# johnayoung/llm-consensus

Measured on AMD Instinct MI355X. Metric: consensus_aggregate_output_tokens_per_s, higher is better.
Workload: dtype bf16

## Files before the change

csrc/kernels/bindings.cpp:

```cpp
#include <hip/hip_runtime_api.h>
#include <pybind11/pybind11.h>

#include <pybind11/stl.h>

#include <stdexcept>
#include <string>
#include <vector>

namespace py = pybind11;
typedef uintptr_t ptr;

extern "C" {
int llmc_rmsnorm(const void*, const void*, void*, int, int, int, int, float, hipStream_t);
int llmc_embedding(const void*, const void*, void*, int, int, int, hipStream_t);
int llmc_lane_exchange_check(const void*, void*, int, hipStream_t);
int llmc_silu_mul_interleaved(const void*, void*, int, int, hipStream_t);
int llmc_gemv(int, const void*, int, const void*, float, const void*, void*, int, int, int, int, int, hipStream_t);
int llmc_gemv_p13(int, const void*, int, const void*, float, const void*, const void*, const void*, void*, int, int, int,
                  int, hipStream_t);
int llmc_gemv_qkv_rope_p13(int, const void*, int, const void*, float, const void*, const void*, const void*, int, int,
                           void*, int, void*, void*, const void*, const void*, const void*, const void*, int, int, int,
                           int, const void*, hipStream_t);
int llmc_wpack13(const void*, void*, void*, void*, int, int, hipStream_t);
int llmc_gemvm(int, const void*, int, const void*, float, const void*, void*, int, int, int, int, int, hipStream_t);
int llmc_moe_gemvm(int, const void*, int, const void*, float, const void*, const void*, int, int, void*, int, int, int,
                   int, hipStream_t);
int llmc_gemm(const void*, int, const void*, int, void*, int, int, int, int, int, hipStream_t);
int llmc_gemm_t128(const void*, int, const void*, int, void*, int, int, int, int, int, hipStream_t);
int llmc_gemm_narrow(const void*, int, const void*, int, void*, int, int, int, int, int, hipStream_t);
int llmc_gemm_kind(const void*, int, const void*, int, void*, int, int, int, int, int, int, hipStream_t);
int llmc_gemm_plan(int, int);
int llmc_rope_kv_write(const void*, int, void*, int, const void*, const void*, const void*, void*, void*, const void*,
                       int, int, int, int, int, const void*, hipStream_t);
int llmc_attn_decode_groups(int);
int llmc_qkv_attn_check(int, int, int, int);
int llmc_qkv_attn(const void*, const void*, float, const void*, int, void*, void*, void*, const void*, const void*,
                  const void*, const void*, const void*, int, const void*, void*, void*, void*, int, int, int, int, int,
                  int, int, int, float, void*, void*, void*, int, const void*, void*, int, const void* const*, void*,
                  int, int, size_t, hipStream_t);
int llmc_attn_oproj_check(int, int, int, int, int, int);
int llmc_attn_oproj_form(int, int, int, int, int, int, int, int);
int llmc_attn_oproj(const void*, const void*, const void*, const void*, int, const void*, const void*, void*, void*,
                    void*, void*, void*, void*, void*, int, int, int, int, int, int, int, int, float, int, void*,
                    int, const void* const*, void*, int, int, size_t, const void*, const void*, float, int, int,
                    void*, void*, void*, void*, hipStream_t);
int llmc_attn_decode(const void*, int, const void*, const void*, const void*, int, const void*, void*, void*, void*,
                     int, int, int, int, int, int, int, int, int, int, float, int, void*, int, hipStream_t);
int llmc_gemv_qkv_rope(int, const void*, int, const void*, float, const void*, int, int, void*, int, void*, void*,
                       const void*, const void*, const void*, const void*, int, int, int, int, int, const void*,
                       hipStream_t);
int llmc_attn_prefill(const void*, int, const void*, const void*, const void*, int, const void*, const void*,
                      const void*, void*, int, int, int, int, int, int, int, float, int, int, void*, void*, int,
                      int, int, hipStream_t);
int llmc_attn_prefill_form(int, int, int, int, int, int, int);
int llmc_attn_prefill_plan(int, int, int, int, int, int, int, int*);
int64_t llmc_attn_prefill_counters(int, int, int, int);
int llmc_sample(const void*, int64_t, int, int, const void*, const void*, const void*, const void*, const void*, void*,
                void*, void*, void*, void*, void*, const void*, int, int, void*, void*, int, int, hipStream_t);
int llmc_sample_parts();
int llmc_moe_route(const void*, int, int, int, void*, void*, hipStream_t);
int llmc_moe_down_combine(int, const void*, int, const void*, const void*, const void*, void*, int, int, int, int,
                          hipStream_t);
int llmc_moe_router(const void*, int, const void*, float, const void*, int, int, int, int, void*, void*, hipStream_t);
int llmc_moe_align(const void*, int, int, int, int, void*, void*, void*, void*, hipStream_t);
int llmc_moe_gemm(const void*, int, int, const void*, const void*, const void*, const void*, void*, int, int, int, int,
                  int, int, int, hipStream_t);
int llmc_moe_combine(const void*, const void*, const void*, void*, int, int, int, hipStream_t);
int llmc_moe_gemv(int, const void*, int, const void*, float, const void*, const void*, int, void*, int, int, int, int,
                  hipStream_t);
int llmc_moe_ep_localize(const void*, const void*, int, int, int, void*, void*, hipStream_t);
int llmc_moe_ep_dispatch(const void*, int, int, int, int, void*, void*, void*, void*, hipStream_t);
int llmc_gather_rows(const void*, int, const void*, int, int, int, void*, int, hipStream_t);
int llmc_moe_route_fused(const void*, int, const void*, int, int, int, int, void*, void*, hipStream_t);
int llmc_gemv_sweep(int, const void*, const void*, const void*, void*, int, int, hipStream_t);
size_t llmc_car_sig_bytes();
int llmc_car_alloc(size_t, void**);
int llmc_car_free(void*);
int llmc_ipc_handle(void*, void*);
int llmc_ipc_handle_size();
int llmc_ipc_open(const void*, void**);
int llmc_ipc_close(void*);
int llmc_car_timed_out(void*, int*);
int llmc_car_max_wait(void*, uint32_t*);
int llmc_car_host_alloc(void**, void**);
int llmc_car_host_free(void*);
int llmc_car_host_get(const void*, int);
void llmc_car_host_set(void*, int, int);
int llmc_car_host_word(int);
size_t llmc_car_timeout_off();
int llmc_car_reset(void*, size_t);
size_t llmc_car_oneshot_max(size_t);
int llmc_gemv_ar(int, const void*, int, const void*, void*, int, int, int, const void* const*, void*, int, int, size_t,
                 hipStream_t);
int llmc_stream_cu_mask(int, const uint32_t*, int, void**);
int llmc_can_access_peer(int, int, int*);
int llmc_car_twoshot(const void* const*, void*, int, int, size_t, int, const void*, void*, long, int, int, hipStream_t);
int llmc_car_allreduce(const void* const*, void*, int, int, size_t, void*, size_t, hipStream_t);
int llmc_car_allgather(const void* const*, void*, int, int, size_t, const void*, void*, size_t, hipStream_t);
}

static inline void check(int rc, const char* what) {
  if (rc != 0) {
    std::string msg = std::string("llmc HIP launch failed: ") + what + " rc=" + std::to_string(rc);
    if (rc > 0) msg += std::string(" (") + hipGetErrorString(static_cast<hipError_t>(rc)) + ")";
    throw std::runtime_error(msg);
  }
}
#define P(x) reinterpret_cast<void*>(x)
#define S(x) reinterpret_cast<hipStream_t>(x)

PYBIND11_MODULE(_llmc_hip, m) {
  m.doc() = "llm_consensus_amd gfx950 HIP kernels (raw-pointer launchers)";
  m.def("rmsnorm", [](ptr x, ptr w, ptr y, int T, int H, int xs, int ys, float eps, ptr s) {
    check(llmc_rmsnorm(P(x), P(w), P(y), T, H, xs, ys, eps, S(s)), "rmsnorm");
  });
  m.def("lane_exchange_check", [](ptr in, ptr out, int nb, ptr s) {
    check(llmc_lane_exchange_check(P(in), P(out), nb, S(s)), "lane_exchange_check");
  });
  m.def("embedding", [](ptr ids, ptr table, ptr out, int T, int H, int V, ptr s) {
    check(llmc_embedding(P(ids), P(table), P(out), T, H, V, S(s)), "embedding");
  });
  m.def("silu_mul_interleaved", [](ptr gu, ptr y, int T, int I, ptr s) {
    check(llmc_silu_mul_interleaved(P(gu), P(y), T, I, S(s)), "silu_mul");
  });
  m.def("gemv", [](int M, ptr x, int xs, ptr nw, float eps, ptr W, ptr out, int os, int N, int K, int epi, int mfma,
                   ptr s) {
    check(llmc_gemv(M, P(x), xs, P(nw), eps, P(W), P(out), os, N, K, epi, mfma, S(s)), "gemv");
  });
  m.def("gemv_p13", [](int M, ptr x, int xs, ptr nw, float eps, ptr W, ptr planes, ptr hdr, ptr out, int os, int N,
                       int K, int epi, ptr s) {
    check(llmc_gemv_p13(M, P(x), xs, P(nw), eps, P(W), P(planes), P(hdr), P(out), os, N, K, epi, S(s)), "gemv_p13");
  });
  m.def("gemv_qkv_rope_p13", [](int M, ptr x, int xs, ptr nw, float eps, ptr W, ptr planes, ptr hdr, int N, int K,
                                ptr qo, int qos, ptr kc, ptr vc, ptr pos, ptr slots, ptr cos_t, ptr sin_t, int nh,
                                int nkv, int D, int bs, ptr s, ptr bias) {
    check(llmc_gemv_qkv_rope_p13(M, P(x), xs, P(nw), eps, P(W), P(planes), P(hdr), N, K, P(qo), qos, P(kc), P(vc),
                                 P(pos), P(slots), P(cos_t), P(sin_t), nh, nkv, D, bs, P(bias), S(s)),
          "gemv_qkv_rope_p13");
  }, py::arg("M"), py::arg("x"), py::arg("x_stride"), py::arg("norm_w"), py::arg("eps"), py::arg("W"),
     py::arg("planes"), py::arg("hdr"), py::arg("N"), py::arg("K"), py::arg("q_out"), py::arg("q_stride"),
     py::arg("k_cache"), py::arg("v_cache"), py::arg("positions"), py::arg("slots"), py::arg("cos_t"),
     py::arg("sin_t"), py::arg("nh"), py::arg("nkv"), py::arg("D"), py::arg("bs"), py::arg("stream"),
     py::arg("bias") = 0);
  m.def("wpack13", [](ptr W, ptr planes, ptr hdr, ptr raw_count, int N, int K, ptr s) {
    check(llmc_wpack13(P(W), P(planes), P(hdr), P(raw_count), N, K, S(s)), "wpack13");
  });
  m.def("moe_gemvm", [](int P, ptr x, int xs, ptr nw, float eps, ptr W, ptr ids, int x_div, int E, ptr out, int os,
                        int N, int K, int epi, ptr s) {
    check(llmc_moe_gemvm(P, P(x), xs, P(nw), eps, P(W), P(ids), x_div, E, P(out), os, N, K, epi, S(s)), "moe_gemvm");
  });
  m.def("gemvm", [](int M, ptr x, int xs, ptr nw, float eps, ptr W, ptr out, int os, int N, int K, int epi, int form,
                    ptr s) {
    check(llmc_gemvm(M, P(x), xs, P(nw), eps, P(W), P(out), os, N, K, epi, form, S(s)), "gemvm");
  });
  m.def("gemm", [](ptr A, int lda, ptr W, int ldw, ptr C, int ldc, int M, int N, int K, int epi, ptr s) {
    check(llmc_gemm(P(A), lda, P(W), ldw, P(C), ldc, M, N, K, epi, S(s)), "gemm");
  });
  m.def("gemm_t128", [](ptr A, int lda, ptr W, int ldw, ptr C, int ldc, int M, int N, int K, int epi, ptr s) {
    check(llmc_gemm_t128(P(A), lda, P(W), ldw, P(C), ldc, M, N, K, epi, S(s)), "gemm_t128");
  });
  m.def("gemm_kind", [](ptr A, int lda, ptr W, int ldw, ptr C, int ldc, int M, int N, int K, int epi, int kind, ptr s) {
    check(llmc_gemm_kind(P(A), lda, P(W), ldw, P(C), ldc, M, N, K, epi, kind, S(s)), "gemm_kind");
  });
  m.def("gemm_plan", [](int M, int N) { return llmc_gemm_plan(M, N); });
  m.def("gemm_narrow", [](ptr A, int lda, ptr W, int ldw, ptr C, int ldc, int M, int N, int K, int epi, ptr s) {
    check(llmc_gemm_narrow(P(A), lda, P(W), ldw, P(C), ldc, M, N, K, epi, S(s)), "gemm_narrow");
  });
  m.def("rope_kv_write", [](ptr qkv, int qs, ptr qo, int qos, ptr pos, ptr cos_t, ptr sin_t, ptr kc, ptr vc,
                            ptr slots, int T, int nh, int nkv, int D, int bs, ptr s, ptr bias) {
    check(llmc_rope_kv_write(P(qkv), qs, P(qo), qos, P(pos), P(cos_t), P(sin_t), P(kc), P(vc), P(slots), T, nh, nkv, D,
                             bs, P(bias), S(s)),
          "rope_kv_write");
  }, py::arg("qkv"), py::arg("qkv_stride"), py::arg("q_out"), py::arg("q_stride"), py::arg("positions"),
     py::arg("cos_t"), py::arg("sin_t"), py::arg("k_cache"), py::arg("v_cache"), py::arg("slots"), py::arg("T"),
     py::arg("nh"), py::arg("nkv"), py::arg("D"), py::arg("bs"), py::arg("stream"),
     py::arg("bias") = 0);
  m.def("attn_decode_groups", [](int max_chunks) { return llmc_attn_decode_groups(max_chunks); });
  m.def("qkv_attn_check", [](int nh, int nkv, int D, int K) { return llmc_qkv_attn_check(nh, nkv, D, K); });
  m.def("qkv_attn", [](ptr x, ptr nw, float eps, ptr W, int K, ptr qo, ptr kc, ptr vc, ptr pos, ptr slots, ptr cos_t,
                       ptr sin_t, ptr bt, int bt_len, ptr sl, ptr part, ptr ctr, ptr out, int nh, int nkv, int D, int bs,
                       int nblocks, int chunk, int gc, int max_chunks, float scale, ptr fault, ptr gran, ptr hctr,
                       int o_mode, ptr w_o, ptr h, int o_n, const std::vector<ptr>& bases, ptr host, int rank, int world,
                       size_t cap, ptr s) {
    std::vector<const void*> b(bases.size());
    for (size_t i = 0; i < bases.size(); ++i) b[i] = P(bases[i]);
    check(llmc_qkv_attn(P(x), P(nw), eps, P(W), K, P(qo), P(kc), P(vc), P(pos), P(slots), P(cos_t), P(sin_t), P(bt),
                        bt_len, P(sl), P(part), P(ctr), P(out), nh, nkv, D, bs, nblocks, chunk, gc, max_chunks, scale,
                        P(fault), P(gran), P(hctr), o_mode, P(w_o), P(h), o_n, b.empty() ? nullptr : b.data(), P(host),
                        rank, world, cap, S(s)),
          "qkv_attn");
  });
  m.def("attn_oproj_check", [](int H, int nh, int nkv, int D, int nc, int K_o) {
    return llmc_attn_oproj_check(H, nh, nkv, D, nc, K_o);
  });
  m.def("attn_oproj_form", [](int H, int nh, int nkv, int D, int nc, int chunk, int mode, int world) {
    return llmc_attn_oproj_form(H, nh, nkv, D, nc, chunk, mode, world);
  });
  m.def("attn_oproj", [](ptr q, ptr kc, ptr vc, ptr bt, int bt_len, ptr sl, ptr w_o, ptr h, ptr attn_out, ptr part,
                         ptr handoff, ptr tile_part, ptr ctr, ptr fault, int H, int nh, int nkv, int D, int bs,
                         int nblocks, int chunk, int nc, float scale, int mode, ptr stamps, int add_resid,
                         const std::vector<ptr>& bases, ptr host, int rank, int world, size_t cap, ptr rt_norm,
                         ptr rt_wr, float rt_eps, int rt_E, int rt_k, ptr rt_w, ptr rt_ids, ptr rt_part,
                         ptr rt_epoch, ptr s) {
    std::vector<const void*> b(bases.size());
    for (size_t i = 0; i < bases.size(); ++i) b[i] = P(bases[i]);
    check(llmc_attn_oproj(P(q), P(kc), P(vc), P(bt), bt_len, P(sl), P(w_o), P(h), P(attn_out), P(part), P(handoff),
                          P(tile_part), P(ctr), P(fault), H, nh, nkv, D, bs, nblocks, chunk, nc, scale, mode, P(stamps),
                          add_resid, b.empty() ? nullptr : b.data(), P(host), rank, world, cap, P(rt_norm), P(rt_wr),
                          rt_eps, rt_E, rt_k, P(rt_w), P(rt_ids), P(rt_part), P(rt_epoch), S(s)),
          "attn_oproj");
  });
  m.def("attn_decode", [](ptr q, int qs, ptr kc, ptr vc, ptr bt, int bts, ptr sl, ptr part, ptr ctr, ptr out, int os,
                          int B, int nh, int nkv, int D, int bs, int nblocks, int chunk, int grid_chunks,
                          int max_chunks, float scale, int fused, ptr fault, ptr s, int window) {
    check(llmc_attn_decode(P(q), qs, P(kc), P(vc), P(bt), bts, P(sl), P(part), P(ctr), P(out), os, B, nh, nkv, D, bs,
                           nblocks, chunk, grid_chunks, max_chunks, scale, fused, P(fault), window, S(s)),
          "attn_decode");
  }, py::arg("q"), py::arg("q_stride"), py::arg("k_cache"), py::arg("v_cache"), py::arg("block_tables"),
     py::arg("bt_stride"), py::arg("seq_lens"), py::arg("part"), py::arg("counters"), py::arg("out"),
     py::arg("out_stride"), py::arg("B"), py::arg("nh"), py::arg("nkv"), py::arg("D"), py::arg("bs"),
     py::arg("nblocks"), py::arg("chunk"), py::arg("grid_chunks"), py::arg("max_chunks"), py::arg("scale"),
     py::arg("fused"), py::arg("fault"), py::arg("stream"), py::arg("window") = 0);
  m.def("gemv_qkv_rope", [](int M, ptr x, int xs, ptr nw, float eps, ptr W, int N, int K, ptr qo, int qos, ptr kc,
                            ptr vc, ptr pos, ptr slots, ptr cos_t, ptr sin_t, int nh, int nkv, int D, int bs,
                            int mfma, ptr s, ptr bias) {
    check(llmc_gemv_qkv_rope(M, P(x), xs, P(nw), eps, P(W), N, K, P(qo), qos, P(kc), P(vc), P(pos), P(slots),
                             P(cos_t), P(sin_t), nh, nkv, D, bs, mfma, P(bias), S(s)),
          "gemv_qkv_rope");
  }, py::arg("M"), py::arg("x"), py::arg("x_stride"), py::arg("norm_w"), py::arg("eps"), py::arg("W"), py::arg("N"),
     py::arg("K"), py::arg("q_out"), py::arg("q_stride"), py::arg("k_cache"), py::arg("v_cache"),
     py::arg("positions"), py::arg("slots"), py::arg("cos_t"), py::arg("sin_t"), py::arg("nh"), py::arg("nkv"),
     py::arg("D"), py::arg("bs"), py::arg("mfma"), py::arg("stream"),
     py::arg("bias") = 0);
  m.def("attn_prefill", [](ptr q, int qs, ptr kc, ptr vc, ptr bt, int bts, ptr qst, ptr ql, ptr cl, ptr out, int os,
                           int B, int max_qlen, int nh, int nkv, int D, int bs, float scale, int ksplit, int kmin,
                           ptr part, ptr counters, int T, int form, ptr s, int window) {
    check(llmc_attn_prefill(P(q), qs, P(kc), P(vc), P(bt), bts, P(qst), P(ql), P(cl), P(out), os, B, max_qlen, nh, nkv,
                            D, bs, scale, ksplit, kmin, P(part), P(counters), T, form, window, S(s)),
          "attn_prefill");
  }, py::arg("q"), py::arg("q_stride"), py::arg("k_cache"), py::arg("v_cache"), py::arg("block_tables"),
     py::arg("bt_stride"), py::arg("q_start"), py::arg("q_lens"), py::arg("ctx_lens"), py::arg("out"),
     py::arg("out_stride"), py::arg("B"), py::arg("max_qlen"), py::arg("nh"), py::arg("nkv"), py::arg("D"),
     py::arg("bs"), py::arg("scale"), py::arg("ksplit"), py::arg("kmin"), py::arg("part"), py::arg("counters"),
     py::arg("T"), py::arg("form"), py::arg("stream"), py::arg("window") = 0);
  m.def("attn_prefill_counters", [](int B, int max_qlen, int nh, int nkv) {
    return llmc_attn_prefill_counters(B, max_qlen, nh, nkv);
  });
  m.def("attn_prefill_form", [](int B, int T, int nh, int nkv, int ksplit, int D, int bs) {
    return llmc_attn_prefill_form(B, T, nh, nkv, ksplit, D, bs);
  });
  m.def("attn_prefill_plan", [](int B, int max_qlen, int max_ctx, int nh, int nkv, int D, int bs) {
    int kmin = 0;
    const int k = llmc_attn_prefill_plan(B, max_qlen, max_ctx, nh, nkv, D, bs, &kmin);
    return std::make_pair(k, kmin);
  });
  m.def("sample", [](ptr logits, int64_t rs, int B, int V, ptr it, ptr tk, ptr tp, ptr seeds, ptr pos, ptr wv, ptr wi,
                     ptr next, ptr tin, ptr sl, ptr slots, ptr bt, int bts, int bs, ptr ot, ptr oc, int cap,
                     int use_topkp, ptr s) {
    check(llmc_sample(P(logits), rs, B, V, P(it), P(tk), P(tp), P(seeds), P(pos), P(wv), P(wi), P(next), P(tin), P(sl),
                      P(slots), P(bt), bts, bs, P(ot), P(oc), cap, use_topkp, S(s)),
          "sample");
  });
  m.def("sample_parts", []() { return llmc_sample_parts(); });
  m.def("moe_route", [](ptr logits, int T, int E, int k, ptr w, ptr ids, ptr s) {
    check(llmc_moe_route(P(logits), T, E, k, P(w), P(ids), S(s)), "moe_route");
  });
  m.def("moe_down_combine", [](int T, ptr act, int as, ptr W, ptr ids, ptr w, ptr h, int hs, int N, int K, int k,
                               ptr s) {
    check(llmc_moe_down_combine(T, P(act), as, P(W), P(ids), P(w), P(h), hs, N, K, k, S(s)), "moe_down_combine");
  });
  m.def("moe_router", [](ptr x, int xs, ptr nw, float eps, ptr Wr, int T, int E, int H, int k, ptr w, ptr ids, ptr s) {
    check(llmc_moe_router(P(x), xs, P(nw), eps, P(Wr), T, E, H, k, P(w), P(ids), S(s)), "moe_router");
  });
  m.def("moe_align", [](ptr ids, int T, int k, int E, int tile, ptr sorted_rows, ptr tile_expert, ptr tile_count,
                        ptr counts, ptr s) {
    check(llmc_moe_align(P(ids), T, k, E, tile, P(sorted_rows), P(tile_expert), P(tile_count), P(counts), S(s)),
          "moe_align");
  });
  m.def("moe_gemm", [](ptr A, int lda, int a_rows, ptr W, ptr sorted_rows, ptr tile_expert, ptr tile_count, ptr C,
                       int ldc, int N, int K, int max_tiles, int a_row_div, int epi, int tile, ptr s) {
    check(llmc_moe_gemm(P(A), lda, a_rows, P(W), P(sorted_rows), P(tile_expert), P(tile_count), P(C), ldc, N, K,
                        max_tiles, a_row_div, epi, tile, S(s)),
          "moe_gemm");
  });
  m.def("moe_combine", [](ptr y, ptr w, ptr rows, ptr out, int T, int k, int H, ptr s) {
    check(llmc_moe_combine(P(y), P(w), P(rows), P(out), T, k, H, S(s)), "moe_combine");
  });
  m.def("moe_gemv", [](int npairs, ptr x, int xs, ptr nw, float eps, ptr W, ptr ids, int x_div, ptr out, int os,
                       int N, int K, int epi, ptr s) {
    check(llmc_moe_gemv(npairs, P(x), xs, P(nw), eps, P(W), P(ids), x_div, P(out), os, N, K, epi, S(s)), "moe_gemv");
  });
  m.def("moe_ep_dispatch", [](ptr ids, int npairs, int El, int n, int cap, ptr sp, ptr se, ptr slot, ptr cnt, ptr s) {
    check(llmc_moe_ep_dispatch(P(ids), npairs, El, n, cap, P(sp), P(se), P(slot), P(cnt), S(s)), "moe_ep_dispatch");
  });
  m.def("moe_route_fused", [](ptr x, int xs, ptr wr, int T, int E, int H, int k, ptr w, ptr ids, ptr s) {
    check(llmc_moe_route_fused(P(x), xs, P(wr), T, E, H, k, P(w), P(ids), S(s)), "moe_route_fused");
  });
  m.def("gather_rows", [](ptr x, int xs, ptr rows, int M, int div, int H, ptr out, int os, ptr s) {
    check(llmc_gather_rows(P(x), xs, P(rows), M, div, H, P(out), os, S(s)), "gather_rows");
  });
  m.def("moe_ep_localize", [](ptr ids, ptr w, int n, int e0, int nl, ptr lids, ptr lw, ptr s) {
    check(llmc_moe_ep_localize(P(ids), P(w), n, e0, nl, P(lids), P(lw), S(s)), "moe_ep_localize");
  });
  m.def("device_synchronize", []() { check(static_cast<int>(hipDeviceSynchronize()), "hipDeviceSynchronize"); });
  m.def("car_sig_bytes", []() { return llmc_car_sig_bytes(); });
  m.def("car_alloc", [](size_t cap) {
    void* p = nullptr;
    check(llmc_car_alloc(cap, &p), "car_alloc");
    return reinterpret_cast<ptr>(p);
  });
  m.def("car_free", [](ptr p) { check(llmc_car_free(P(p)), "car_free"); });
  m.def("ipc_handle", [](ptr p) {
    std::string h(static_cast<size_t>(llmc_ipc_handle_size()), '\0');
    check(llmc_ipc_handle(P(p), h.data()), "ipc_handle");
    return py::bytes(h);
  });
  m.def("ipc_open", [](py::bytes h) {
    std::string s = h;
    if (static_cast<int>(s.size()) != llmc_ipc_handle_size()) throw std::runtime_error("ipc_open: bad handle size");
    void* p = nullptr;
    check(llmc_ipc_open(s.data(), &p), "ipc_open");
    return reinterpret_cast<ptr>(p);
  });
  m.def("ipc_close", [](ptr p) { check(llmc_ipc_close(P(p)), "ipc_close"); });
  m.def("car_timed_out", [](ptr own) {
    int v = 0;
    check(llmc_car_timed_out(P(own), &v), "car_timed_out");
    return v;
  });
  m.def("car_timeout_off", []() { return llmc_car_timeout_off(); });
  m.def("car_max_wait", [](ptr own) {
    uint32_t v = 0;
    check(llmc_car_max_wait(P(own), &v), "car_max_wait");
    return v;
  });
  m.def("car_host_alloc", []() {
    void* h = nullptr;
    void* d = nullptr;
    check(llmc_car_host_alloc(&h, &d), "car_host_alloc");
    return py::make_tuple(reinterpret_cast<ptr>(h), reinterpret_cast<ptr>(d));
  });
  m.def("car_host_free", [](ptr h) { check(llmc_car_host_free(P(h)), "car_host_free"); });
  m.def("car_host_get", [](ptr h, int word) { return llmc_car_host_get(P(h), word); });
  m.def("car_host_set", [](ptr h, int word, int v) { llmc_car_host_set(P(h), word, v); });
  m.def("car_host_word", [](int which) { return llmc_car_host_word(which); });
  m.def("car_reset", [](ptr own, size_t cap) { check(llmc_car_reset(P(own), cap), "car_reset"); });
  m.def("car_oneshot_max", [](size_t cap) { return llmc_car_oneshot_max(cap); });
  m.def("gemv_ar", [](int M, ptr x, int xs, ptr W, ptr h, int hs, int N, int K, const std::vector<ptr>& bases,
                      ptr host, int rank, int world, size_t cap, ptr s) {
    std::vector<const void*> b(bases.size());
    for (size_t i = 0; i < bases.size(); ++i) b[i] = P(bases[i]);
    check(llmc_gemv_ar(M, P(x), xs, P(W), P(h), hs, N, K, b.data(), P(host), rank, world, cap, S(s)), "gemv_ar");
  });
  m.def("stream_cu_mask", [](int device, const std::vector<uint32_t>& mask) {
    void* st = nullptr;
    check(llmc_stream_cu_mask(device, mask.data(), static_cast<int>(mask.size()), &st), "stream_cu_mask");
    return reinterpret_cast<ptr>(st);
  });
  m.def("can_access_peer", [](int dev, int peer) {
    int v = 0;
    check(llmc_can_access_peer(dev, peer, &v), "can_access_peer");
    return v;
  });
  m.def("car_twoshot", [](const std::vector<ptr>& bases, ptr host, int rank, int world, size_t cap, int mode, ptr in,
                          ptr out, long seg_stride, int seg16, int nv, ptr s) {
    std::vector<const void*> b(bases.size());
    for (size_t i = 0; i < bases.size(); ++i) b[i] = P(bases[i]);
    check(llmc_car_twoshot(b.data(), P(host), rank, world, cap, mode, P(in), P(out), seg_stride, seg16, nv, S(s)),
          "car_twoshot");
  });
  m.def("car_allreduce", [](const std::vector<ptr>& bases, ptr host, int rank, int world, size_t cap, ptr x,
                            size_t nbytes, ptr s) {
    std::vector<const void*> b(bases.size());
    for (size_t i = 0; i < bases.size(); ++i) b[i] = P(bases[i]);
    check(llmc_car_allreduce(b.data(), P(host), rank, world, cap, P(x), nbytes, S(s)), "car_allreduce");
  });
  m.def("car_allgather", [](const std::vector<ptr>& bases, ptr host, int rank, int world, size_t cap, ptr x, ptr out,
                            size_t nbytes, ptr s) {
    std::vector<const void*> b(bases.size());
    for (size_t i = 0; i < bases.size(); ++i) b[i] = P(bases[i]);
    check(llmc_car_allgather(b.data(), P(host), rank, world, cap, P(x), P(out), nbytes, S(s)), "car_allgather");
  });
  m.def("gemv_sweep", [](int v, ptr x, ptr nw, ptr W, ptr out, int N, int K, ptr s) {
    check(llmc_gemv_sweep(v, P(x), P(nw), P(W), P(out), N, K, S(s)), "gemv_sweep");
  });
}
```

csrc/kernels/gemv.hip:

```cpp
#include <cstdlib>

#include "gemv_core.h"

namespace llmc {

template <int M, int NT, int RPW, int PRO, int EPI, int UNROLL>
static int launch_gemv_p13(const void* x, int x_stride, const void* nw, float eps, const void* W, const PackedW& pw,
                           void* out, int out_stride, int N, int K, const RopeEpi& rope, hipStream_t s) {
  if constexpr (M <= 2 && UNROLL % 4 == 0) {
    constexpr int WAVES = NT / kWave;
    auto kern = gemv_p13_kernel<M, NT, RPW, UNROLL, PRO, EPI>;
    const size_t lds = static_cast<size_t>(M) * K * sizeof(bf16_t) + 2 * M * WAVES * sizeof(float);
    if (lds > 160 * 1024) return -2;
    static bool attr_set = false;
    if (lds > 64 * 1024 && !attr_set) {
      (void)hipFuncSetAttribute(reinterpret_cast<const void*>(kern), hipFuncAttributeMaxDynamicSharedMemorySize,
                                160 * 1024);
      attr_set = true;
    }
    const int rows_per_block = WAVES * RPW;
    const int grid = (N + rows_per_block - 1) / rows_per_block;
    kern<<<grid, NT, lds, s>>>((const bf16_t*)x, x_stride, (const bf16_t*)nw, eps, (const bf16_t*)W, pw, out,
                               out_stride, N, K, rope);
    return static_cast<int>(hipGetLastError());
  } else {
    return -8;
  }
}

template <int M, int NT, int RPW, int PRO, int EPI, int UNROLL_OVERRIDE = 0>
static int launch_gemv_g(const void* x, int x_stride, const void* nw, float eps, const void* W, void* out,
                         int out_stride, int N, int K, const RopeEpi& rope, const PackedW& pw, hipStream_t s) {
  constexpr int UNROLL = UNROLL_OVERRIDE ? UNROLL_OVERRIDE : (RPW == 1 ? 4 : (RPW == 2 ? 4 : (M <= 2 ? 4 : 2)));
  constexpr int WAVES = NT / kWave;
  if (pw.planes != nullptr)
    return launch_gemv_p13<M, NT, RPW, PRO, EPI, UNROLL>(x, x_stride, nw, eps, W, pw, out, out_stride, N, K, rope, s);
  auto kern = gemv_kernel<M, NT, RPW, UNROLL, PRO, EPI, false>;
  const size_t lds = static_cast<size_t>(M) * K * sizeof(bf16_t) + 2 * M * WAVES * sizeof(float);
  if (lds > 160 * 1024) return -2;
  static bool attr_set = false;
  if (lds > 64 * 1024 && !attr_set) {
    (void)hipFuncSetAttribute(reinterpret_cast<const void*>(kern), hipFuncAttributeMaxDynamicSharedMemorySize,
                              160 * 1024);
    attr_set = true;
  }
  const int rows_per_block = WAVES * RPW;
  const int grid = (N + rows_per_block - 1) / rows_per_block;
  kern<<<grid, NT, lds, s>>>((const bf16_t*)x, x_stride, (const bf16_t*)nw, eps, (const bf16_t*)W, out, out_stride, N,
                             K, nullptr, 1, rope, CarArgs{});
  return static_cast<int>(hipGetLastError());
}

static int pick_waves(int N, bool paired) {
  if (N < 2048 && (!paired || N % 8 == 0)) return 4;
  static const bool no10 = std::getenv("LLMC_GEMV_NO_W10") != nullptr;
  static const bool no14 = std::getenv("LLMC_GEMV_NO_W14") != nullptr;
  int best = 16;
  double best_idle = 2.0;
  for (int w : {16, 14, 12, 10, 8}) {
    if ((w == 10 && no10) || (w == 14 && (no14 || !paired))) continue;
    if (paired && N % (2 * w) != 0) continue;
    const long blocks = (N + w - 1) / w;
    const long slots = (blocks + 255) / 256 * 256;
    const double idle = static_cast<double>(slots - blocks) / static_cast<double>(slots);
    if (idle < best_idle - 1e-9) {
      best_idle = idle;
      best = w;
    }
  }
  return best_idle > 1.0 ? 0 : best;
}

template <int M, int PRO, int EPI>
static int launch_gemv(const void* x, int x_stride, const void* nw, float eps, const void* W, void* out,
                       int out_stride, int N, int K, const RopeEpi& rope, const PackedW& pw, hipStream_t s) {
  constexpr bool paired = EPI == EPI_SILU || EPI == EPI_ROPE;
  const int w = pick_waves(N, paired);
  if constexpr (M <= 2) {
    static const bool rope_rpw1 = std::getenv("LLMC_GEMV_ROPE_RPW1") != nullptr;
    if (EPI == EPI_ROPE && w == 12 && N % (2 * 12 * 256) == 0 && !rope_rpw1)
      return launch_gemv_g<M, 768, 2, PRO, EPI, 4>(x, x_stride, nw, eps, W, out, out_stride, N, K, rope, pw, s);
    static const bool silu_rpw1 = std::getenv("LLMC_GEMV_SILU_RPW1") != nullptr;
    if (EPI == EPI_SILU && !silu_rpw1 && K < 8192) {
      if (N % (2 * 16 * 256) == 0)
        return launch_gemv_g<M, 1024, 2, PRO, EPI, 4>(x, x_stride, nw, eps, W, out, out_stride, N, K, rope, pw, s);
      if (N % (2 * 14 * 256) == 0)
        return launch_gemv_g<M, 896, 2, PRO, EPI, 4>(x, x_stride, nw, eps, W, out, out_stride, N, K, rope, pw, s);
    }
    if (w == 16 && K >= 8192 && N <= 4096)
      return launch_gemv_g<M, 1024, 1, PRO, EPI, 8>(x, x_stride, nw, eps, W, out, out_stride, N, K, rope, pw, s);
    if (w == 10 && K >= 8192)
      return launch_gemv_g<M, 640, 1, PRO, EPI, 8>(x, x_stride, nw, eps, W, out, out_stride, N, K, rope, pw, s);
  }
  switch (w) {
    case 16: return launch_gemv_g<M, 1024, 1, PRO, EPI>(x, x_stride, nw, eps, W, out, out_stride, N, K, rope, pw, s);
    case 14: return launch_gemv_g<M, 896, 1, PRO, EPI>(x, x_stride, nw, eps, W, out, out_stride, N, K, rope, pw, s);
    case 12: return launch_gemv_g<M, 768, 1, PRO, EPI>(x, x_stride, nw, eps, W, out, out_stride, N, K, rope, pw, s);
    case 10: return launch_gemv_g<M, 640, 1, PRO, EPI>(x, x_stride, nw, eps, W, out, out_stride, N, K, rope, pw, s);
    case 8: return launch_gemv_g<M, 512, 1, PRO, EPI>(x, x_stride, nw, eps, W, out, out_stride, N, K, rope, pw, s);
    case 4: return launch_gemv_g<M, 256, 1, PRO, EPI, 8>(x, x_stride, nw, eps, W, out, out_stride, N, K, rope, pw, s);
    default:
      return launch_gemv_g<M, 256, 2, PRO, EPI>(x, x_stride, nw, eps, W, out, out_stride, N, K, rope, pw, s);
  }
}

template <int PRO, int EPI>
static int dispatch_m(int M, const void* x, int x_stride, const void* nw, float eps, const void* W, void* out,
                      int out_stride, int N, int K, const RopeEpi& rope, const PackedW& pw, hipStream_t s) {
  switch (M) {
    case 1: return launch_gemv<1, PRO, EPI>(x, x_stride, nw, eps, W, out, out_stride, N, K, rope, pw, s);
    case 2: return launch_gemv<2, PRO, EPI>(x, x_stride, nw, eps, W, out, out_stride, N, K, rope, pw, s);
    case 3: return launch_gemv<3, PRO, EPI>(x, x_stride, nw, eps, W, out, out_stride, N, K, rope, pw, s);
    case 4: return launch_gemv<4, PRO, EPI>(x, x_stride, nw, eps, W, out, out_stride, N, K, rope, pw, s);
    default: return -3;
  }
}

static int gemv_dispatch(int M, const void* x, int x_stride, const void* norm_w, float eps, const void* W, void* out,
                         int out_stride, int N, int K, int epi, const RopeEpi& rope, const PackedW& pw, bool mfma,
                         hipStream_t s) {
  if (K % 8 != 0) return -1;
  if ((epi == EPI_SILU || epi == EPI_ROPE) && (N % 2 != 0)) return -1;
  if ((M > kGemvMaxM || mfma) && K % 128 == 0 && x_stride % 8 == 0)
    return gemvm_dispatch(M, x, x_stride, norm_w, eps, W, out, out_stride, N, K, epi, rope, s);
  const bool norm = norm_w != nullptr;
#define LLMC_GEMV_CASE(E)                                                                                   \
  case E:                                                                                                   \
    return norm ? dispatch_m<PRO_NORM, E>(M, x, x_stride, norm_w, eps, W, out, out_stride, N, K, rope, pw, s)   \
                : dispatch_m<PRO_NONE, E>(M, x, x_stride, norm_w, eps, W, out, out_stride, N, K, rope, pw, s);
  switch (epi) {
    LLMC_GEMV_CASE(EPI_BF16)
    LLMC_GEMV_CASE(EPI_F32)
    LLMC_GEMV_CASE(EPI_RESADD)
    LLMC_GEMV_CASE(EPI_SILU)
    case EPI_ROPE:
      if (!norm) return -5;
      return dispatch_m<PRO_NORM, EPI_ROPE>(M, x, x_stride, norm_w, eps, W, out, out_stride, N, K, rope, pw, s);
    default: return -4;
  }
#undef LLMC_GEMV_CASE
}

}

using namespace llmc;

extern "C" int llmc_gemv(int M, const void* x, int x_stride, const void* norm_w, float eps, const void* W, void* out,
                         int out_stride, int N, int K, int epi, int mfma, hipStream_t s) {
  if (epi == EPI_ROPE) return -5;
  RopeEpi rope{};
  return gemv_dispatch(M, x, x_stride, norm_w, eps, W, out, out_stride, N, K, epi, rope, PackedW{}, mfma != 0, s);
}

extern "C" int llmc_gemv_p13(int M, const void* x, int x_stride, const void* norm_w, float eps, const void* W,
                             const void* planes, const void* hdr, void* out, int out_stride, int N, int K, int epi,
                             hipStream_t s) {
  if (epi == EPI_ROPE) return -5;
  if (M < 1 || M > kGemvMaxM || K % kP13UnitElems != 0 || planes == nullptr || hdr == nullptr) return -1;
  RopeEpi rope{};
  const PackedW pw{static_cast<const uint8_t*>(planes), static_cast<const uint8_t*>(hdr)};
  return gemv_dispatch(M, x, x_stride, norm_w, eps, W, out, out_stride, N, K, epi, rope, pw, false, s);
}

extern "C" int llmc_gemv_qkv_rope(int M, const void* x, int x_stride, const void* norm_w, float eps, const void* W,
                                  int N, int K, void* q_out, int q_stride, void* k_cache, void* v_cache,
                                  const void* positions, const void* slots, const void* cos_t, const void* sin_t,
                                  int nh, int nkv, int D, int bs, int mfma, const void* bias, hipStream_t s) {
  if (N != (nh + 2 * nkv) * D || D % 2 != 0 || reinterpret_cast<uintptr_t>(bias) % 4 != 0) return -1;
  RopeEpi rope{(bf16_t*)q_out, q_stride, (bf16_t*)k_cache, (bf16_t*)v_cache, (const int32_t*)positions,
               (const int32_t*)slots, (const float*)cos_t, (const float*)sin_t, nh, nkv, D, bs};
  rope.bias = static_cast<const bf16_t*>(bias);
  return gemv_dispatch(M, x, x_stride, norm_w, eps, W, nullptr, 0, N, K, EPI_ROPE, rope, PackedW{}, mfma != 0, s);
}

extern "C" int llmc_gemv_qkv_rope_p13(int M, const void* x, int x_stride, const void* norm_w, float eps,
                                      const void* W, const void* planes, const void* hdr, int N, int K, void* q_out,
                                      int q_stride, void* k_cache, void* v_cache, const void* positions,
                                      const void* slots, const void* cos_t, const void* sin_t, int nh, int nkv, int D,
                                      int bs, const void* bias, hipStream_t s) {
  if (N != (nh + 2 * nkv) * D || D % 2 != 0 || reinterpret_cast<uintptr_t>(bias) % 4 != 0) return -1;
  if (M < 1 || M > kGemvMaxM || K % kP13UnitElems != 0 || planes == nullptr || hdr == nullptr) return -1;
  RopeEpi rope{(bf16_t*)q_out, q_stride, (bf16_t*)k_cache, (bf16_t*)v_cache, (const int32_t*)positions,
               (const int32_t*)slots, (const float*)cos_t, (const float*)sin_t, nh, nkv, D, bs};
  rope.bias = static_cast<const bf16_t*>(bias);
  const PackedW pw{static_cast<const uint8_t*>(planes), static_cast<const uint8_t*>(hdr)};
  return gemv_dispatch(M, x, x_stride, norm_w, eps, W, nullptr, 0, N, K, EPI_ROPE, rope, pw, false, s);
}

namespace llmc {
template <int M, int NT, int UNROLL>
static int launch_gemv_ar(const void* x, int x_stride, const void* W, void* h, int h_stride, int N, int K,
                          const CarArgs& ar, hipStream_t s) {
  constexpr int WAVES = NT / kWave;
  auto kern = gemv_kernel<M, NT, 1, UNROLL, PRO_NONE, EPI_AR, false>;
  const size_t lds = static_cast<size_t>(M) * K * sizeof(bf16_t) + 2 * M * WAVES * sizeof(float);
  if (lds > 160 * 1024) return -2;
  static bool attr_set = false;
  if (lds > 64 * 1024 && !attr_set) {
    (void)hipFuncSetAttribute(reinterpret_cast<const void*>(kern), hipFuncAttributeMaxDynamicSharedMemorySize,
                              160 * 1024);
    attr_set = true;
  }
  const int grid = (N + WAVES - 1) / WAVES;
  if (grid > kMaxBlocks || static_cast<size_t>(grid) * kArGranulesPerBlock * 8 > static_cast<size_t>(ar.cap) / kMaxRanks)
    return -6;
  kern<<<grid, NT, lds, s>>>((const bf16_t*)x, x_stride, nullptr, 0.f, (const bf16_t*)W, h, h_stride, N, K, nullptr, 1,
                             RopeEpi{}, ar);
  return static_cast<int>(hipGetLastError());
}

template <int M>
static int gemv_ar_geom(const void* x, int x_stride, const void* W, void* h, int h_stride, int N, int K,
                        const CarArgs& ar, hipStream_t s) {
  const int w = pick_waves(N, false);
  if (w == 16 && K >= 8192 && N <= 4096) return launch_gemv_ar<M, 1024, 8>(x, x_stride, W, h, h_stride, N, K, ar, s);
  if (w == 10 && K >= 8192) return launch_gemv_ar<M, 640, 8>(x, x_stride, W, h, h_stride, N, K, ar, s);
  switch (w) {
    case 16: return launch_gemv_ar<M, 1024, 4>(x, x_stride, W, h, h_stride, N, K, ar, s);
    case 12: return launch_gemv_ar<M, 768, 4>(x, x_stride, W, h, h_stride, N, K, ar, s);
    case 10: return launch_gemv_ar<M, 640, 4>(x, x_stride, W, h, h_stride, N, K, ar, s);
    case 8: return launch_gemv_ar<M, 512, 4>(x, x_stride, W, h, h_stride, N, K, ar, s);
    case 4: return launch_gemv_ar<M, 256, 8>(x, x_stride, W, h, h_stride, N, K, ar, s);
    default: return -7;
  }
}
}

extern "C" int llmc_gemv_ar(int M, const void* x, int x_stride, const void* W, void* h, int h_stride, int N, int K,
                            const void* const* bases, void* host, int rank, int world, size_t cap, hipStream_t s) {
  if (K % 8 != 0 || N % 2 != 0 || world < 1 || world > kMaxRanks || rank < 0 || rank >= world) return -1;
  CarArgs ar{};
  for (int r = 0; r < kMaxRanks; ++r)
    ar.P.base[r] = r < world ? static_cast<char*>(const_cast<void*>(bases[r])) : nullptr;
  ar.P.host = static_cast<uint32_t*>(host);
  ar.rank = rank;
  ar.world = world;
  ar.cap = static_cast<long>(cap);
  switch (M) {
    case 1: return gemv_ar_geom<1>(x, x_stride, W, h, h_stride, N, K, ar, s);
    case 2: return gemv_ar_geom<2>(x, x_stride, W, h, h_stride, N, K, ar, s);
    default: return -3;
  }
}

namespace llmc {
template <int NT, int RPW, int EPI, int PRO>
static int launch_moe_gemv(int npairs, const void* x, int x_stride, const void* nw, float eps, const void* W,
                           const void* ids, int x_div, void* out, int out_stride, int N, int K, hipStream_t s) {
  constexpr int WAVES = NT / kWave;
  const size_t lds = static_cast<size_t>(K) * sizeof(bf16_t) + 2 * WAVES * sizeof(float);
  if (lds > 64 * 1024) return -2;
  dim3 grid((N + WAVES * RPW - 1) / (WAVES * RPW), npairs);
  gemv_kernel<1, NT, RPW, 4, PRO, EPI, true><<<grid, NT, lds, s>>>(
      (const bf16_t*)x, x_stride, (const bf16_t*)nw, eps, (const bf16_t*)W, out, out_stride, N, K,
      (const int32_t*)ids, x_div, RopeEpi{}, CarArgs{});
  return static_cast<int>(hipGetLastError());
}

template <int EPI, int PRO>
static int moe_gemv_geom(int npairs, const void* x, int x_stride, const void* nw, float eps, const void* W,
                         const void* ids, int x_div, void* out, int out_stride, int N, int K, hipStream_t s) {
  static const bool silu_rpw1 = std::getenv("LLMC_GEMV_SILU_RPW1") != nullptr;
  if (EPI == EPI_SILU && !silu_rpw1 && K < 8192) {
    if (N % (2 * 16 * 256) == 0)
      return launch_moe_gemv<1024, 2, EPI, PRO>(npairs, x, x_stride, nw, eps, W, ids, x_div, out, out_stride, N, K, s);
    if (N % (2 * 14 * 256) == 0)
      return launch_moe_gemv<896, 2, EPI, PRO>(npairs, x, x_stride, nw, eps, W, ids, x_div, out, out_stride, N, K, s);
  }
  switch (pick_waves(N, EPI == EPI_SILU)) {
    case 16: return launch_moe_gemv<1024, 1, EPI, PRO>(npairs, x, x_stride, nw, eps, W, ids, x_div, out, out_stride, N, K, s);
    case 14: return launch_moe_gemv<896, 1, EPI, PRO>(npairs, x, x_stride, nw, eps, W, ids, x_div, out, out_stride, N, K, s);
    case 12: return launch_moe_gemv<768, 1, EPI, PRO>(npairs, x, x_stride, nw, eps, W, ids, x_div, out, out_stride, N, K, s);
    case 10: return launch_moe_gemv<640, 1, EPI, PRO>(npairs, x, x_stride, nw, eps, W, ids, x_div, out, out_stride, N, K, s);
    case 8: return launch_moe_gemv<512, 1, EPI, PRO>(npairs, x, x_stride, nw, eps, W, ids, x_div, out, out_stride, N, K, s);
    case 4: return launch_moe_gemv<256, 1, EPI, PRO>(npairs, x, x_stride, nw, eps, W, ids, x_div, out, out_stride, N, K, s);
    default: return launch_moe_gemv<256, 2, EPI, PRO>(npairs, x, x_stride, nw, eps, W, ids, x_div, out, out_stride, N, K, s);
  }
}
}

extern "C" int llmc_moe_down_combine(int T, const void* act, int act_stride, const void* W, const void* ids,
                                     const void* w, void* h, int h_stride, int N, int K, int k, hipStream_t s) {
  if (k != 2 || K % 8 != 0) return -1;
  constexpr int NT = 1024, WAVES = NT / kWave;
  auto kern = gemv_kernel<2, NT, 2, 4, PRO_NONE, EPI_COMBINE, true>;
  const size_t lds = static_cast<size_t>(2) * K * sizeof(bf16_t) + 2 * 2 * WAVES * sizeof(float);
  if (lds > 160 * 1024) return -2;
  static bool attr_set = false;
  if (lds > 64 * 1024 && !attr_set) {
    (void)hipFuncSetAttribute(reinterpret_cast<const void*>(kern), hipFuncAttributeMaxDynamicSharedMemorySize,
                              160 * 1024);
    attr_set = true;
  }
  RopeEpi wts{};
  wts.cos_t = static_cast<const float*>(w);
  dim3 grid((N + WAVES - 1) / WAVES, T);
  kern<<<grid, NT, lds, s>>>((const bf16_t*)act, act_stride, nullptr, 0.f, (const bf16_t*)W, h, h_stride, N, K,
                             (const int32_t*)ids, 1, wts, CarArgs{});
  return static_cast<int>(hipGetLastError());
}

extern "C" int llmc_moe_gemv(int npairs, const void* x, int x_stride, const void* norm_w, float eps, const void* W,
                             const void* ids, int x_div, void* out, int out_stride, int N, int K, int epi,
                             hipStream_t s) {
  if (K % 8 != 0) return -1;
  const void* nw = norm_w;
  switch (epi) {
    case EPI_BF16:
      return nw ? moe_gemv_geom<EPI_BF16, PRO_NORM>(npairs, x, x_stride, nw, eps, W, ids, x_div, out, out_stride, N, K, s)
                : moe_gemv_geom<EPI_BF16, PRO_NONE>(npairs, x, x_stride, nw, eps, W, ids, x_div, out, out_stride, N, K, s);
    case EPI_SILU:
      return nw ? moe_gemv_geom<EPI_SILU, PRO_NORM>(npairs, x, x_stride, nw, eps, W, ids, x_div, out, out_stride, N, K, s)
                : moe_gemv_geom<EPI_SILU, PRO_NONE>(npairs, x, x_stride, nw, eps, W, ids, x_div, out, out_stride, N, K, s);
    default: return -4;
  }
}

namespace llmc {
template <int NT, int RPW, int UNROLL>
static int launch_sweep(const void* x, const void* nw, const void* W, void* out, int N, int K, hipStream_t s) {
  constexpr int WAVES = NT / kWave;
  const size_t lds = static_cast<size_t>(K) * sizeof(bf16_t) + WAVES * sizeof(float);
  const int grid = (N + WAVES * RPW - 1) / (WAVES * RPW);
  gemv_kernel<1, NT, RPW, UNROLL, PRO_NORM, EPI_BF16, false><<<grid, NT, lds, s>>>(
      (const bf16_t*)x, K, (const bf16_t*)nw, 1e-5f, (const bf16_t*)W, out, N, N, K, nullptr, 1, RopeEpi{}, CarArgs{});
  return static_cast<int>(hipGetLastError());
}
}

extern "C" int llmc_gemv_sweep(int variant, const void* x, const void* nw, const void* W, void* out, int N, int K,
                               hipStream_t s) {
  if (K % 8 != 0 || K * 2 > 64 * 1024) return -1;
  switch (variant) {
    case 0: return launch_sweep<256, 1, 8>(x, nw, W, out, N, K, s);
    case 1: return launch_sweep<256, 2, 4>(x, nw, W, out, N, K, s);
    case 2: return launch_sweep<256, 4, 4>(x, nw, W, out, N, K, s);
    case 3: return launch_sweep<512, 1, 8>(x, nw, W, out, N, K, s);
    case 4: return launch_sweep<512, 2, 4>(x, nw, W, out, N, K, s);
    case 5: return launch_sweep<128, 1, 8>(x, nw, W, out, N, K, s);
    case 6: return launch_sweep<64, 1, 8>(x, nw, W, out, N, K, s);
    case 7: return launch_sweep<1024, 1, 4>(x, nw, W, out, N, K, s);
    case 8: return launch_sweep<256, 1, 4>(x, nw, W, out, N, K, s);
    case 9: return launch_sweep<256, 2, 8>(x, nw, W, out, N, K, s);
    case 10: return launch_sweep<512, 4, 2>(x, nw, W, out, N, K, s);
    case 11: return launch_sweep<128, 2, 4>(x, nw, W, out, N, K, s);
    case 12: return launch_sweep<1024, 1, 8>(x, nw, W, out, N, K, s);
    case 13: return launch_sweep<1024, 2, 4>(x, nw, W, out, N, K, s);
    case 14: return launch_sweep<1024, 2, 2>(x, nw, W, out, N, K, s);
    case 15: return launch_sweep<1024, 1, 2>(x, nw, W, out, N, K, s);
    case 16: return launch_sweep<768, 1, 4>(x, nw, W, out, N, K, s);
    case 17: return launch_sweep<1024, 4, 2>(x, nw, W, out, N, K, s);
    case 18: return launch_sweep<1024, 1, 6>(x, nw, W, out, N, K, s);
    case 19: return launch_sweep<768, 2, 4>(x, nw, W, out, N, K, s);
    case 20: return launch_sweep<640, 1, 8>(x, nw, W, out, N, K, s);
    case 21: return launch_sweep<896, 1, 4>(x, nw, W, out, N, K, s);
    case 22: return launch_sweep<768, 2, 2>(x, nw, W, out, N, K, s);
    case 23: return launch_sweep<1024, 2, 2>(x, nw, W, out, N, K, s);
    default: return -2;
  }
}
```

csrc/kernels/gemv_core.h:

```cpp
#pragma once
#include <type_traits>

#include "car_proto.h"
#include "common.h"

namespace llmc {

enum { PRO_NONE = 0, PRO_NORM = 1 };
enum { EPI_BF16 = 0, EPI_F32 = 1, EPI_RESADD = 2, EPI_SILU = 3, EPI_ROPE = 4, EPI_COMBINE = 5, EPI_AR = 6 };


struct RopeEpi {
  bf16_t* q_out;
  int q_stride;
  bf16_t* k_cache;
  bf16_t* v_cache;
  const int32_t* positions;
  const int32_t* slots;
  const float* cos_t;
  const float* sin_t;
  int nh, nkv, D, bs;
  uint64_t* granules;
  uint32_t gtag;
  const bf16_t* bias;
};

enum { WF_BF16 = 0, WF_P13 = 1 };
constexpr int kP13UnitElems = 2048, kP13UnitBytes = 3328, kP13Raw = 0xff;
struct PackedW {
  const uint8_t* planes;
  const uint8_t* hdr;
};
struct P13Unit {
  u32x4 l0, l1, n;
  uint32_t s;
};
template <int C>
__device__ __forceinline__ u32x4 p13_chunk(const P13Unit& p, uint32_t base4) {
  const uint32_t n = p.n[C];
  const uint32_t e0 = (n & 0x0f0f0f0fu) + base4, e1 = ((n >> 4) & 0x0f0f0f0fu) + base4;
  const u32x4& L = C < 2 ? p.l0 : p.l1;
  const uint32_t lw0 = L[(2 * C) & 3], lw1 = L[(2 * C + 1) & 3];
  const uint32_t h0 = ((p.s << (7 - 2 * C)) & 0x80808080u) | e0;
  const uint32_t h1 = ((p.s << (6 - 2 * C)) & 0x80808080u) | e1;
  u32x4 w;
  w[0] = __builtin_amdgcn_perm(h0, lw0, 0x05010400u);
  w[1] = __builtin_amdgcn_perm(h0, lw0, 0x07030602u);
  w[2] = __builtin_amdgcn_perm(h1, lw1, 0x05010400u);
  w[3] = __builtin_amdgcn_perm(h1, lw1, 0x07030602u);
  return w;
}

constexpr int kGemvMaxM = 2, kGemvmMaxM = 32, kMoeGemvmMaxTokens = 16;
int gemvm_dispatch(int M, const void* x, int x_stride, const void* norm_w, float eps, const void* W, void* out,
                   int out_stride, int N, int K, int epi, const RopeEpi& rope, hipStream_t st, int form = 0);

template <int M, int NT, int RPW, int UNROLL, int PRO, int EPI, bool EXPERT = false, int WF = WF_BF16>
__device__ __forceinline__ void gemv_block(const int bx, const int by, char* smem, const bf16_t* __restrict__ x,
                                           int x_stride, const bf16_t* __restrict__ norm_w, float eps,
                                           const bf16_t* __restrict__ W, void* __restrict__ out, int out_stride, int N,
                                           int K, const int32_t* __restrict__ expert_ids, int x_div, const RopeEpi& rope,
                                           const CarArgs& ar, const PackedW& pw = PackedW{}) {
  constexpr int WAVES = NT / kWave;
  constexpr bool P13 = WF == WF_P13;
  static_assert(!P13 || (!EXPERT && EPI != EPI_AR && EPI != EPI_COMBINE && UNROLL % 4 == 0 && M <= 2),
                "packed weights: the dense one- and two-row decode forms");
  constexpr bool PAIR_LDS = (EPI == EPI_SILU || EPI == EPI_ROPE) && RPW == 1;
  constexpr bool ROPE_PRE = EPI == EPI_ROPE && (PAIR_LDS || RPW == 2);
  constexpr bool COMBINE = EPI == EPI_COMBINE;
  static_assert(!COMBINE || (EXPERT && M == RPW), "combine: one x row per expert slot");
  if constexpr (EXPERT && !COMBINE) {
    const int pair = by;
    if (expert_ids[pair] < 0) return;
    W += static_cast<int64_t>(expert_ids[pair]) * N * K;
    x += static_cast<int64_t>(pair / x_div) * x_stride;
    out = reinterpret_cast<char*>(out) + static_cast<int64_t>(pair) * out_stride * (EPI == EPI_F32 ? 4 : 2);
  }
  if constexpr (COMBINE) {
    const int t = by;
    x += static_cast<int64_t>(t) * RPW * x_stride;
    out = reinterpret_cast<char*>(out) + static_cast<int64_t>(t) * out_stride * 2;
  }
  bf16_t* xs = reinterpret_cast<bf16_t*>(smem);
  const int tid = threadIdx.x;
  const int nchunk = K / 8;
  const int wave = tid / kWave, lane = tid % kWave;
  const int row0 = COMBINE ? bx * WAVES + wave : (bx * WAVES + wave) * RPW;

  const u32x4* wrow[RPW];
#pragma unroll
  for (int r = 0; r < RPW; ++r) {
    if constexpr (COMBINE) {
      const int e = expert_ids[by * RPW + r];
      wrow[r] = reinterpret_cast<const u32x4*>(W + (static_cast<int64_t>(e) * N + min(row0, N - 1)) * K);
    } else {
      const int n = min(row0 + r, N - 1);
      wrow[r] = reinterpret_cast<const u32x4*>(W + static_cast<int64_t>(n) * K);
    }
  }
  constexpr int STEP = kWave * UNROLL;
  const int iters = (nchunk + STEP - 1) / STEP;
  u32x4 cur[RPW][UNROLL];
  auto issue = [&](u32x4 (&dst)[RPW][UNROLL], int cbase) {
#pragma unroll
    for (int u = 0; u < UNROLL; ++u) {
      const int c = min(cbase + u * kWave, nchunk - 1);
#pragma unroll
      for (int r = 0; r < RPW; ++r) dst[r][u] = load16<true>(wrow[r] + c);
    }
  };
  constexpr bool kXRegs = (PRO == PRO_NORM || PRO == PRO_NONE);
  const bool x_fast = nchunk <= 2 * NT;
  u32x4 xr[2][M], gr[2];
  if constexpr (kXRegs) {
    if (x_fast) {
#pragma unroll
      for (int j = 0; j < 2; ++j) {
        const int c = tid + j * NT;
        if (c < nchunk) {
          if constexpr (PRO == PRO_NORM) gr[j] = reinterpret_cast<const u32x4*>(norm_w)[c];
#pragma unroll
          for (int m = 0; m < M; ++m) xr[j][m] = reinterpret_cast<const u32x4*>(x + static_cast<int64_t>(m) * x_stride)[c];
        }
      }
    }
  }
  constexpr int UB = P13 ? UNROLL / 4 : 1;
  const int units = K / kP13UnitElems;
  P13Unit cur13[P13 ? RPW : 1][UB];
  const uint8_t* prow[RPW];
  uint32_t hdr_w[RPW];
  auto issue13 = [&](P13Unit (&dst)[P13 ? RPW : 1][UB], int ubase) {
#pragma unroll
    for (int j = 0; j < UB; ++j) {
      const int u = min(ubase + j, units - 1);
#pragma unroll
      for (int r = 0; r < (P13 ? RPW : 1); ++r) {
        const uint8_t* p = prow[r] + static_cast<int64_t>(u) * kP13UnitBytes + lane * 16;
        dst[r][j].l0 = load16<true>(p);
        dst[r][j].l1 = load16<true>(p + 1024);
        dst[r][j].n = load16<true>(p + 2048);
        dst[r][j].s = __builtin_nontemporal_load(reinterpret_cast<const uint32_t*>(p + 3072 - lane * 12));
      }
    }
  };
  __builtin_amdgcn_sched_barrier(0);
  if constexpr (P13) {
    const int w_u = __builtin_amdgcn_readfirstlane(wave);
#pragma unroll
    for (int r = 0; r < RPW; ++r) {
      const int n_u = min((bx * WAVES + w_u) * RPW + r, N - 1);
      hdr_w[r] = ld_scalar(reinterpret_cast<const uint32_t*>(pw.hdr + (n_u & ~3))) >> ((n_u & 3) * 8) & 0xffu;
      prow[r] = pw.planes + static_cast<int64_t>(n_u) * units * kP13UnitBytes;
    }
    issue13(cur13, 0);
  } else {
    issue(cur, lane);
  }
  __builtin_amdgcn_sched_barrier(0);


  uint32_t ar_epoch = 0;
  float ar_resid[M];
  if constexpr (EPI == EPI_AR) {
    static_assert(RPW == 1 && M <= 2 && M * WAVES / 2 <= kArGranulesPerBlock, "EPI_AR geometry");
    if (tid == 0)
      ar_epoch = __hip_atomic_load(car_ctr(ar.P.base[ar.rank]) + bx, __ATOMIC_RELAXED,
                                   __HIP_MEMORY_SCOPE_SYSTEM) + 1;
#pragma unroll
    for (int m = 0; m < M; ++m)
      ar_resid[m] = ar.rank == 0 && row0 < N
                        ? bf16_to_f32(reinterpret_cast<const bf16_t*>(out)[static_cast<int64_t>(m) * out_stride + row0])
                        : 0.f;
  }

  int pre_pos[M], pre_slot[M];
  float pre_c[M], pre_s[M];
  uint32_t pre_b = 0;
  if constexpr (ROPE_PRE) {
#pragma unroll
    for (int m = 0; m < M; ++m) {
      pre_slot[m] = ld_scalar(rope.slots + m);
      pre_pos[m] = ld_scalar(rope.positions + m);
    }
    if (rope.bias != nullptr) {
      const int w_u = __builtin_amdgcn_readfirstlane(wave);
      const int r_u = min(((bx * WAVES + w_u) * RPW) & ~1, N - 2);
      pre_b = ld_scalar(reinterpret_cast<const uint32_t*>(rope.bias + r_u));
    }
  }

  if constexpr (PRO == PRO_NORM) {
    float(*red)[WAVES] = reinterpret_cast<float(*)[WAVES]>(smem + static_cast<size_t>(M) * K * sizeof(bf16_t));
    float ss[M];
#pragma unroll
    for (int m = 0; m < M; ++m) ss[m] = 0.f;
    if (x_fast) {
#pragma unroll
      for (int j = 0; j < 2; ++j) {
        if (tid + j * NT < nchunk) {
#pragma unroll
          for (int m = 0; m < M; ++m) {
            float f[8];
            unpack8(xr[j][m], f);
#pragma unroll
            for (int e = 0; e < 8; ++e) ss[m] += f[e] * f[e];
          }
        }
      }
#pragma unroll
      for (int m = 0; m < M; ++m) {
        const float sm = wave_sum(ss[m]);
        if ((tid & 63) == 0) red[m][tid / 64] = sm;
      }
      __syncthreads();
      float inv[M];
#pragma unroll
      for (int m = 0; m < M; ++m) {
        float t = 0.f;
#pragma unroll
        for (int w = 0; w < WAVES; ++w) t += red[m][w];
        inv[m] = rsqrtf(t / K + eps);
      }
#pragma unroll
      for (int j = 0; j < 2; ++j) {
        const int c = tid + j * NT;
        if (c < nchunk) {
          float g[8];
          unpack8(gr[j], g);
#pragma unroll
          for (int m = 0; m < M; ++m) {
            float f[8];
            unpack8(xr[j][m], f);
#pragma unroll
            for (int e = 0; e < 8; ++e) f[e] = f[e] * inv[m] * g[e];
            reinterpret_cast<u32x4*>(xs + m * K)[c] = pack8(f);
          }
        }
      }
    } else {
      for (int c = tid; c < nchunk; c += NT) {
#pragma unroll
        for (int m = 0; m < M; ++m) {
          float f[8];
          unpack8(reinterpret_cast<const u32x4*>(x + static_cast<int64_t>(m) * x_stride)[c], f);
#pragma unroll
          for (int j = 0; j < 8; ++j) ss[m] += f[j] * f[j];
        }
      }
#pragma unroll
      for (int m = 0; m < M; ++m) {
        const float sm = wave_sum(ss[m]);
        if ((tid & 63) == 0) red[m][tid / 64] = sm;
      }
      __syncthreads();
      float inv[M];
#pragma unroll
      for (int m = 0; m < M; ++m) {
        float t = 0.f;
#pragma unroll
        for (int w = 0; w < WAVES; ++w) t += red[m][w];
        inv[m] = rsqrtf(t / K + eps);
      }
      for (int c = tid; c < nchunk; c += NT) {
        float g[8];
        unpack8(reinterpret_cast<const u32x4*>(norm_w)[c], g);
#pragma unroll
        for (int m = 0; m < M; ++m) {
          float f[8];
          unpack8(reinterpret_cast<const u32x4*>(x + static_cast<int64_t>(m) * x_stride)[c], f);
#pragma unroll
          for (int j = 0; j < 8; ++j) f[j] = f[j] * inv[m] * g[j];
          reinterpret_cast<u32x4*>(xs + m * K)[c] = pack8(f);
        }
      }
    }
  } else if (x_fast) {
#pragma unroll
    for (int j = 0; j < 2; ++j) {
      const int c = tid + j * NT;
      if (c < nchunk) {
#pragma unroll
        for (int m = 0; m < M; ++m) reinterpret_cast<u32x4*>(xs + m * K)[c] = xr[j][m];
      }
    }
  } else {
    for (int c = tid; c < nchunk; c += NT) {
#pragma unroll
      for (int m = 0; m < M; ++m)
        reinterpret_cast<u32x4*>(xs + m * K)[c] =
            reinterpret_cast<const u32x4*>(x + static_cast<int64_t>(m) * x_stride)[c];
    }
  }
  __syncthreads();
  if (!PAIR_LDS && EPI != EPI_AR && row0 >= N) return;
  if constexpr (ROPE_PRE) {
    const int w_u = __builtin_amdgcn_readfirstlane(wave);
    const int r_u = (bx * WAVES + w_u) * RPW;
    const int D = rope.D, half = D / 2;
    const bool qk = r_u / D < rope.nh + rope.nkv;
    const int i = (r_u % D) / 2;
#pragma unroll
    for (int m = 0; m < M; ++m) {
      pre_c[m] = 1.f;
      pre_s[m] = 0.f;
      if (qk) {
        const int64_t t = static_cast<int64_t>(pre_pos[m]) * half + i;
        pre_c[m] = ld_scalar(rope.cos_t + t);
        pre_s[m] = ld_scalar(rope.sin_t + t);
      }
    }
  }

  float acc[RPW][M];
#pragma unroll
  for (int r = 0; r < RPW; ++r)
#pragma unroll
    for (int m = 0; m < M; ++m) acc[r][m] = 0.f;

  const u32x4* xv = reinterpret_cast<const u32x4*>(xs);
  auto consume = [&](const u32x4 (&wv)[RPW][UNROLL], int cbase, auto masked) {
#pragma unroll
    for (int u = 0; u < UNROLL; ++u) {
      const int c = cbase + u * kWave;
      if (!decltype(masked)::value || c < nchunk) {
#pragma unroll
        for (int m = 0; m < M; ++m) {
          const u32x4 xx = xv[m * nchunk + c];
#pragma unroll
          for (int r = 0; r < RPW; ++r)
            if (!COMBINE || r == m) acc[r][m] = dot8_bf16(wv[r][u], xx, acc[r][m]);
        }
      }
    }
  };
  using Full = std::integral_constant<bool, false>;
  using Masked = std::integral_constant<bool, true>;
  auto stream_bf16 = [&]() {
    const int full = nchunk / STEP;
    int c0 = lane;
    for (int it = 0; it + 1 < iters; ++it, c0 += STEP) {
      u32x4 nxt[RPW][UNROLL];
      issue(nxt, c0 + STEP);
      consume(cur, c0, Full{});
#pragma unroll
      for (int u = 0; u < UNROLL; ++u)
#pragma unroll
        for (int r = 0; r < RPW; ++r) cur[r][u] = nxt[r][u];
    }
    if (full == iters) {
      consume(cur, c0, Full{});
    } else {
      consume(cur, c0, Masked{});
    }
  };
  if constexpr (P13) {
    bool raw = false;
    uint32_t base4[RPW];
#pragma unroll
    for (int r = 0; r < RPW; ++r) {
      raw |= hdr_w[r] == kP13Raw;
      base4[r] = hdr_w[r] * 0x01010101u;
    }
    if (raw) {
      issue(cur, lane);
      stream_bf16();
    } else {
      auto consume13 = [&](const P13Unit (&wv)[RPW][UB], int ubase, auto masked) {
#pragma unroll
        for (int j = 0; j < UB; ++j) {
          if (!decltype(masked)::value || ubase + j < units) {
            const int cb = lane + kWave * 4 * (ubase + j);
            auto chunk = [&](auto cc) {
              constexpr int C = decltype(cc)::value;
              u32x4 w[RPW];
#pragma unroll
              for (int r = 0; r < RPW; ++r) w[r] = p13_chunk<C>(wv[r][j], base4[r]);
#pragma unroll
              for (int m = 0; m < M; ++m) {
                const u32x4 xx = xv[m * nchunk + cb + C * kWave];
#pragma unroll
                for (int r = 0; r < RPW; ++r) acc[r][m] = dot8_bf16(w[r], xx, acc[r][m]);
              }
            };
            chunk(std::integral_constant<int, 0>{});
            chunk(std::integral_constant<int, 1>{});
            chunk(std::integral_constant<int, 2>{});
            chunk(std::integral_constant<int, 3>{});
          }
        }
      };
      const int it13 = (units + UB - 1) / UB;
      int u0 = 0;
      for (int it = 0; it + 1 < it13; ++it, u0 += UB) {
        P13Unit nxt[RPW][UB];
        issue13(nxt, u0 + UB);
        consume13(cur13, u0, Full{});
#pragma unroll
        for (int j = 0; j < UB; ++j)
#pragma unroll
          for (int r = 0; r < RPW; ++r) cur13[r][j] = nxt[r][j];
      }
      if (units % UB == 0) {
        consume13(cur13, u0, Full{});
      } else {
        consume13(cur13, u0, Masked{});
      }
    }
  } else {
    stream_bf16();
  }

#pragma unroll
  for (int r = 0; r < RPW; ++r)
#pragma unroll
    for (int m = 0; m < M; ++m)
      if (!COMBINE || r == m) acc[r][m] = wave_sum(acc[r][m]);

  auto rope_ops = [&](int n, int m, float& c, float& sn, int& slot, uint32_t& b2) {
    const int D = rope.D, half = D / 2;
    slot = rope.slots[m];
    b2 = rope.bias != nullptr ? *reinterpret_cast<const uint32_t*>(rope.bias + n) : 0u;
    c = 1.f;
    sn = 0.f;
    if (n / D < rope.nh + rope.nkv) {
      const int i = (n % D) / 2;
      const int pos = rope.positions[m];
      c = rope.cos_t[static_cast<int64_t>(pos) * half + i];
      sn = rope.sin_t[static_cast<int64_t>(pos) * half + i];
    }
  };
  auto pair_epi = [&](int n, int m, float v, float x2, float c, float sn, int slot, uint32_t b2) {
    if constexpr (EPI == EPI_ROPE) {
      if (rope.bias != nullptr) {
        v += bf16_lo(b2);
        x2 += bf16_hi(b2);
      }
    }
    if constexpr (EPI == EPI_SILU) {
      reinterpret_cast<bf16_t*>(out)[static_cast<int64_t>(m) * out_stride + n / 2] = f32_to_bf16(silu(v) * x2);
    } else if constexpr (EPI == EPI_ROPE) {
      const int D = rope.D, half = D / 2;
      const int head = n / D;
      const int64_t page = slot >= 0 ? slot / rope.bs : 0;
      const int off = slot >= 0 ? slot % rope.bs : 0;
      if (head < rope.nh + rope.nkv) {
        const int i = (n % D) / 2;
        const float o1 = v * c - x2 * sn, o2 = x2 * c + v * sn;
        if (head < rope.nh) {
          bf16_t* qo = rope.q_out + static_cast<int64_t>(m) * rope.q_stride + head * D;
          qo[i] = f32_to_bf16(o1);
          qo[i + half] = f32_to_bf16(o2);
        } else if (slot >= 0) {
          bf16_t* ko = rope.k_cache + ((page * rope.nkv + (head - rope.nh)) * rope.bs + off) * D;
          ko[i] = f32_to_bf16(o1);
          ko[i + half] = f32_to_bf16(o2);
        }
        if (rope.granules != nullptr)
          __hip_atomic_store(rope.granules + head * half + i,
                             static_cast<uint64_t>(pack_bf16x2(o1, o2)) | (static_cast<uint64_t>(rope.gtag) << 32),
                             __ATOMIC_RELAXED, __HIP_MEMORY_SCOPE_AGENT);
      } else {
        const int vh = head - rope.nh - rope.nkv, d = n % D;
        if (slot >= 0) {
          bf16_t* vv = rope.v_cache + ((page * rope.nkv + vh) * rope.bs + off) * D;
          vv[d] = f32_to_bf16(v);
          vv[d + 1] = f32_to_bf16(x2);
        }
        if (rope.granules != nullptr)
          __hip_atomic_store(rope.granules + head * half + d / 2,
                             static_cast<uint64_t>(pack_bf16x2(v, x2)) | (static_cast<uint64_t>(rope.gtag) << 32),
                             __ATOMIC_RELAXED, __HIP_MEMORY_SCOPE_AGENT);
      }
    }
  };
  if constexpr (PAIR_LDS) {
    float* pairx = reinterpret_cast<float*>(smem + static_cast<size_t>(M) * K * sizeof(bf16_t)) + M * WAVES;
    if ((wave & 1) && lane < M) {
#pragma unroll
      for (int m = 0; m < M; ++m)
        if (lane == m) pairx[(wave >> 1) * M + m] = acc[0][m];
    }
    __syncthreads();
    if (!(wave & 1)) {
#pragma unroll
      for (int m = 0; m < M; ++m)
        if (lane == m && row0 < N) {
          if constexpr (EPI == EPI_ROPE) {
            pair_epi(row0, m, acc[0][m], pairx[(wave >> 1) * M + m], pre_c[m], pre_s[m], pre_slot[m], pre_b);
          } else {
            pair_epi(row0, m, acc[0][m], pairx[(wave >> 1) * M + m], 1.f, 0.f, -1, 0u);
          }
        }
    }
    return;
  }
  if constexpr (EPI == EPI_AR) {
    constexpr int HP = WAVES / 2, NG = M * HP;
    float* rowv = reinterpret_cast<float*>(smem + static_cast<size_t>(M) * K * sizeof(bf16_t)) + M * WAVES;
#pragma unroll
    for (int m = 0; m < M; ++m)
      if (lane == m) rowv[m * WAVES + wave] = acc[0][m] + ar_resid[m];
    __syncthreads();
    if (wave != 0) return;
    const uint32_t epoch = __shfl(ar_epoch, 0, 64);
    const int rb = bx * WAVES;
    const int pairs = max(0, min(WAVES, N - rb)) / 2;
    const long gbase = static_cast<long>(bx) * kArGranulesPerBlock;
    auto payload = [&](int gi) {
      const int m = gi / HP, j = gi % HP;
      return pack_bf16x2(rowv[m * WAVES + 2 * j], rowv[m * WAVES + 2 * j + 1]);
    };
    for (int idx = lane; idx < ar.world * NG; idx += kWave) {
      const int p = idx / NG, gi = idx % NG;
      if (p != ar.rank && gi % HP < pairs)
        car_put(ar.P.base[p] + car_granule_off(epoch, ar.cap, ar.rank, gbase + gi), payload(gi), epoch);
    }
    if (lane < NG && lane % HP < pairs) {
      const long g[1] = {gbase + lane};
      uint32_t in[kMaxRanks][1];
      car_collect<1>(ar.P, ar.rank, ar.world, ar.cap, epoch, g, in);
      in[ar.rank][0] = payload(lane);
      float lo = 0.f, hi = 0.f;
#pragma unroll
      for (int r = 0; r < kMaxRanks; ++r) {
        if (r < ar.world) {
          lo += bf16_lo(in[r][0]);
          hi += bf16_hi(in[r][0]);
        }
      }
      const int m = lane / HP, j = lane % HP;
      *reinterpret_cast<uint32_t*>(reinterpret_cast<bf16_t*>(out) + static_cast<int64_t>(m) * out_stride + rb + 2 * j) =
          pack_bf16x2(lo, hi);
    }
    if (lane == 0)
      __hip_atomic_store(car_ctr(ar.P.base[ar.rank]) + bx, epoch, __ATOMIC_RELAXED, __HIP_MEMORY_SCOPE_SYSTEM);
    return;
  }
  if constexpr (COMBINE) {
    if (lane == 0 && row0 < N) {
      const float* wt = rope.cos_t + by * RPW;
      bf16_t* h = reinterpret_cast<bf16_t*>(out) + row0;
      float v = bf16_to_f32(*h);
#pragma unroll
      for (int r = 0; r < RPW; ++r) v += wt[r] * acc[r][r];
      *h = f32_to_bf16(v);
    }
    return;
  }
#pragma unroll
  for (int r = 0; r < RPW; ++r) {
#pragma unroll
    for (int m = 0; m < M; ++m) {
      const int n = row0 + r;
      if (lane != r * M + m || n >= N) continue;
      const float v = acc[r][m];
      if constexpr (EPI == EPI_BF16) {
        reinterpret_cast<bf16_t*>(out)[static_cast<int64_t>(m) * out_stride + n] = f32_to_bf16(v);
      } else if constexpr (EPI == EPI_F32) {
        reinterpret_cast<float*>(out)[static_cast<int64_t>(m) * out_stride + n] = v;
      } else if constexpr (EPI == EPI_RESADD) {
        bf16_t* h = reinterpret_cast<bf16_t*>(out) + static_cast<int64_t>(m) * out_stride + n;
        *h = f32_to_bf16(bf16_to_f32(*h) + v);
      } else {
        if constexpr (RPW >= 2) {
          if ((r & 1) == 0) {
            float c = 1.f, sn = 0.f;
            int slot = -1;
            uint32_t b2 = 0;
            if constexpr (EPI == EPI_ROPE && RPW == 2) {
              c = pre_c[m];
              sn = pre_s[m];
              slot = pre_slot[m];
              b2 = pre_b;
            } else if constexpr (EPI == EPI_ROPE) {
              rope_ops(n, m, c, sn, slot, b2);
            }
            pair_epi(n, m, v, acc[r + 1][m], c, sn, slot, b2);
          }
        }
      }
    }
  }
}

template <int M, int NT, int RPW, int UNROLL, int PRO, int EPI, bool EXPERT = false>
__global__ __launch_bounds__(NT) void gemv_kernel(const bf16_t* __restrict__ x, int x_stride,
                                                  const bf16_t* __restrict__ norm_w, float eps,
                                                  const bf16_t* __restrict__ W, void* __restrict__ out,
                                                  int out_stride, int N, int K, const int32_t* __restrict__ expert_ids,
                                                  int x_div, RopeEpi rope, CarArgs ar) {
  extern __shared__ __attribute__((aligned(16))) char smem[];
  gemv_block<M, NT, RPW, UNROLL, PRO, EPI, EXPERT>(blockIdx.x, blockIdx.y, smem, x, x_stride, norm_w, eps, W, out,
                                                   out_stride, N, K, expert_ids, x_div, rope, ar);
}


template <int M, int NT, int RPW, int UNROLL, int PRO, int EPI>
__global__ __launch_bounds__(NT) void gemv_p13_kernel(const bf16_t* __restrict__ x, int x_stride,
                                                      const bf16_t* __restrict__ norm_w, float eps,
                                                      const bf16_t* __restrict__ W, PackedW pw,
                                                      void* __restrict__ out, int out_stride, int N, int K,
                                                      RopeEpi rope) {
  extern __shared__ __attribute__((aligned(16))) char smem[];
  gemv_block<M, NT, RPW, UNROLL, PRO, EPI, false, WF_P13>(blockIdx.x, blockIdx.y, smem, x, x_stride, norm_w, eps, W,
                                                          out, out_stride, N, K, nullptr, 1, rope, CarArgs{}, pw);
}

}
```

csrc/kernels/wpack.hip:

```cpp
#include "gemv_core.h"

namespace llmc {

__global__ __launch_bounds__(256) void wpack_header_kernel(const bf16_t* __restrict__ W, uint8_t* __restrict__ hdr,
                                                           int32_t* __restrict__ raw_count, int N, int K) {
  const int lane = threadIdx.x % kWave;
  const int row = blockIdx.x * (blockDim.x / kWave) + threadIdx.x / kWave;
  if (row >= N) return;
  const u32x4* w = reinterpret_cast<const u32x4*>(W + static_cast<int64_t>(row) * K);
  int hi = 0, lo = 127;
  for (int c = lane; c < K / 8; c += kWave) {
    const u32x4 v = w[c];
#pragma unroll
    for (int i = 0; i < 4; ++i) {
      const int a = (v[i] >> 8) & 0x7f, b = (v[i] >> 24) & 0x7f;
      hi = max(hi, max(a, b));
      lo = min(lo, min(a, b));
    }
  }
  for (int o = 32; o; o >>= 1) {
    hi = max(hi, __shfl_xor(hi, o, kWave));
    lo = min(lo, __shfl_xor(lo, o, kWave));
  }
  if (lane == 0) {
    const int base = max(hi - 15, 0);
    const bool raw = lo < base;
    hdr[row] = raw ? kP13Raw : static_cast<uint8_t>(base);
    if (raw) atomicAdd(raw_count, 1);
  }
}

__global__ __launch_bounds__(256) void wpack_planes_kernel(const bf16_t* __restrict__ W,
                                                           const uint8_t* __restrict__ hdr, uint8_t* __restrict__ P,
                                                           int N, int K) {
  const int units = K / kP13UnitElems;
  const int64_t gid = static_cast<int64_t>(blockIdx.x) * blockDim.x + threadIdx.x;
  if (gid >= static_cast<int64_t>(N) * units * kWave) return;
  const int lane = static_cast<int>(gid % kWave);
  const int u = static_cast<int>((gid / kWave) % units);
  const int64_t row = gid / kWave / units;
  const u32x4* w = reinterpret_cast<const u32x4*>(W + row * K);
  const uint32_t hb = hdr[row];
  const uint32_t base = hb == kP13Raw ? 0u : hb;
  uint32_t lowb[8], nib[4], S = 0;
#pragma unroll
  for (int c = 0; c < 4; ++c) {
    const u32x4 v = w[lane + kWave * (4 * u + c)];
    uint32_t code[2];
#pragma unroll
    for (int h = 0; h < 2; ++h) {
      const int g = 2 * c + h;
      uint32_t lb = 0, cd = 0;
#pragma unroll
      for (int j = 0; j < 4; ++j) {
        const uint32_t b = (v[2 * h + j / 2] >> (16 * (j & 1))) & 0xffffu;
        lb |= (b & 0xffu) << (8 * j);
        cd |= ((((b >> 8) & 0x7fu) - base) & 0xfu) << (8 * j);
        S |= (b >> 15) << (8 * j + g);
      }
      lowb[g] = lb;
      code[h] = cd;
    }
    nib[c] = code[0] | (code[1] << 4);
  }
  uint8_t* p = P + (row * units + u) * kP13UnitBytes;
  u32x4 o;
  o = u32x4{lowb[0], lowb[1], lowb[2], lowb[3]};
  *reinterpret_cast<u32x4*>(p + lane * 16) = o;
  o = u32x4{lowb[4], lowb[5], lowb[6], lowb[7]};
  *reinterpret_cast<u32x4*>(p + 1024 + lane * 16) = o;
  o = u32x4{nib[0], nib[1], nib[2], nib[3]};
  *reinterpret_cast<u32x4*>(p + 2048 + lane * 16) = o;
  *reinterpret_cast<uint32_t*>(p + 3072 + lane * 4) = S;
}

}

using namespace llmc;

extern "C" int llmc_wpack13(const void* W, void* planes, void* hdr, void* raw_count, int N, int K, hipStream_t s) {
  if (N <= 0 || K <= 0 || K % kP13UnitElems != 0) return -1;
  wpack_header_kernel<<<(N + 3) / 4, 256, 0, s>>>((const bf16_t*)W, (uint8_t*)hdr, (int32_t*)raw_count, N, K);
  const int64_t threads = static_cast<int64_t>(N) * (K / kP13UnitElems) * kWave;
  wpack_planes_kernel<<<static_cast<unsigned>((threads + 255) / 256), 256, 0, s>>>(
      (const bf16_t*)W, (const uint8_t*)hdr, (uint8_t*)planes, N, K);
  return static_cast<int>(hipGetLastError());
}
```

llm_consensus_amd/engine/engine.py:

```python

from __future__ import annotations

import dataclasses
import logging
import math
import os
import time
from typing import Callable, Dict, List, Optional, Sequence as Seq

import torch

from .. import ops
from ..context import Context, ContextError
from ..models.config import ModelConfig, rope_inv_freq
from ..models.transformer import TransformerWeights
from ..ops import EPI_BF16, EPI_F32, EPI_RESADD, EPI_SILU, oracle
from ..parallel.comm import TPGroup
from ..parallel.placement import packed_weights_mode
from ..utils import trace
from ..utils.native import runtime


@dataclasses.dataclass
class EngineConfig:
    device: str = "cuda:0"
    max_context: int = 8192
    max_batch: int = 1
    max_seqs: int = 0
    block_size: int = 64
    kv_blocks: int = 0
    seed: int = 0
    steps_per_graph: int = 8
    use_graphs: bool = True
    prefill_chunk: int = 8192
    init_scale: float = 1.0
    stream_priority: int = 0
    cu_mask: str = dataclasses.field(default_factory=lambda: os.environ.get("LLMC_CU_MASK", ""))
    sequence_parallel: bool = True
    sp_min_tokens: int = 256
    expert_parallel: bool = False
    attn_oproj: bool = dataclasses.field(default_factory=lambda: os.environ.get("LLMC_ATTN_OPROJ", "1") != "0")
    tp_attn_oproj: bool = dataclasses.field(default_factory=lambda: os.environ.get("LLMC_TP_ATTN_OPROJ", "0") == "1")
    attn_oproj_min_chunk: int = dataclasses.field(default_factory=ops.attn_oproj_min_chunk)
    qkv_attn: str = dataclasses.field(default_factory=lambda: os.environ.get("LLMC_QKV_ATTN", "1"))
    qkv_attn_o: bool = dataclasses.field(default_factory=lambda: os.environ.get("LLMC_QKV_ATTN_O", "0") == "1")
    ao_router: bool = dataclasses.field(default_factory=lambda: os.environ.get("LLMC_AO_ROUTER", "1") != "0")
    fused_ar: bool = True
    packed_weights: str = dataclasses.field(default_factory=packed_weights_mode)


FUSED_CHUNK_SMALL, FUSED_CHUNK_LARGE = 128, 256
PACKED_MARGIN_BYTES = 4 << 30
log = logging.getLogger(__name__)
QKV_ATTN_MAX_ROWS = 2048
BATCHING_MIN_KEYS, BATCHING_MIN_KEYS_FEW = 2048, 512


def attn_buckets(ctxmax: int, blocks_per_head: int = 32, fused_max: int = 4096, group: int = 4,
                 nkv: int = 8, rows: int = 1) -> List[tuple]:
    out, cap = [], 1024
    if rows >= 3:
        mk = BATCHING_MIN_KEYS if rows * nkv >= 32 else BATCHING_MIN_KEYS_FEW
        while True:
            c = min(cap, ctxmax)
            gc = min(32, (c + mk - 1) // mk)
            if out and out[-1][2] == gc:
                out[-1] = (c, mk, gc, False)
            else:
                out.append((c, mk, gc, False))
            if cap >= ctxmax:
                return out
            cap *= 2
    while True:
        c = min(cap, ctxmax)
        if fused_max > 0 and c <= fused_max:
            ch = FUSED_CHUNK_SMALL if c <= (2048 if group >= 2 else 1024) else FUSED_CHUNK_LARGE
            out.append((c, ch, (c + ch - 1) // ch, True))
        elif fused_max > 0 and (c + 127) // 128 * nkv <= 256:
            out.append((c, 128, (c + 127) // 128, True))
        elif fused_max > 0 and (c + 255) // 256 * nkv <= 256:
            out.append((c, 256, (c + 255) // 256, True))
        else:
            gc = min((c + 127) // 128, blocks_per_head)
            if out and not out[-1][3] and out[-1][2] == gc:
                out[-1] = (c, 128, gc, False)
            else:
                out.append((c, 128, gc, False))
        if cap >= ctxmax:
            return out
        cap *= 2


def qkv_attn_plan(buckets: List[tuple], ao_chunks: List[int], mode: str, qkv_rows: int, bs: int):
    plan: List[Optional[tuple]] = [None] * len(buckets)
    if mode in ("0", "False", "") or (mode != "all" and qkv_rows >= QKV_ATTN_MAX_ROWS):
        return plan, list(ao_chunks)
    qa_all = mode == "all"
    for i, (cap, ch, gc, fused) in enumerate(buckets):
        if fused and ch in (128, 256) and bs % (ch // 4) == 0 and (qa_all or not ao_chunks[i]):
            plan[i] = (ch, gc)
        elif qa_all and not fused and bs % 64 == 0:
            plan[i] = (256, (cap + 255) // 256)
    ao = [0 if q else a for q, a in zip(plan, ao_chunks)] if qa_all else list(ao_chunks)
    return plan, ao


def split_blocks_per_head(nh: int, nkv: int) -> int:
    blocks = 512 if nh == nkv else 256
    return max(1, min(blocks // nkv, 256))


@dataclasses.dataclass
class SamplingParams:
    max_tokens: int = 256
    temperature: float = 1.0
    top_p: float = 1.0
    top_k: int = 0
    seed: int = 0
    stop_on_eos: bool = True


class Sequence:

    def __init__(self, sid: int):
        self.sid = sid
        self.row = -1
        self.blocks: List[int] = []
        self.length = 0
        self.has_logits = False
        self.logits: Optional[torch.Tensor] = None


class EngineError(Exception):
    pass


class InjectedEngineFault(EngineError):
    """Raised by the ``Engine.fault_at`` test hook."""


class _TPBroken(EngineError):
    """The TP group of this engine can no longer agree (see Engine._tp_broken)."""


class Engine:
    def __init__(self, cfg: ModelConfig, ecfg: Optional[EngineConfig] = None, tp: Optional[TPGroup] = None,
                 name: str = "", weights: Optional[TransformerWeights] = None):
        self.cfg = cfg
        self.ecfg = ecfg or EngineConfig()
        rows_max = ops.MOE_GEMVM_MAX_TOKENS if cfg.is_moe else ops.GEMV_MAX_M
        if not 1 <= self.ecfg.max_batch <= rows_max:
            raise EngineError(f"{cfg.name}: max_batch {self.ecfg.max_batch} outside 1..{rows_max} decode rows")
        self.tp = tp or TPGroup.single()
        self.name = name or cfg.name
        self.device = torch.device(self.ecfg.device)
        self.on_gpu = self.device.type == "cuda"
        self.mfma_decode = self.on_gpu and self.ecfg.max_batch >= 3
        if self.on_gpu:
            torch.cuda.set_device(self.device)
            if self.ecfg.cu_mask:
                lo, hi = (int(v) for v in self.ecfg.cu_mask.split("-"))
                words = [0] * max(8, hi // 32 + 1)
                for cu in range(lo, hi + 1):
                    words[cu // 32] |= 1 << (cu % 32)
                from ..utils.native import kernels

                ptr = kernels().stream_cu_mask(self.device.index or 0, words)
                self.stream = torch.cuda.ExternalStream(ptr, device=self.device)
            else:
                self.stream = torch.cuda.Stream(self.device, priority=self.ecfg.stream_priority)
        else:
            self.stream = None
        e = self.ecfg
        with self._on_stream():
            with trace.span("weights_init", engine=self.name):
                if weights is not None:
                    self.w = weights.to(self.device)
                else:
                    self.w = TransformerWeights(cfg, self.tp, self.device, e.seed, e.init_scale,
                                                expert_parallel=e.expert_parallel)
        self.nh, self.nkv, self.D = self.w.nh, self.w.nkv, cfg.head_dim
        self.scale = 1.0 / math.sqrt(self.D)
        self.bs = e.block_size
        self.max_blocks_per_seq = (e.max_context + self.bs - 1) // self.bs + 1
        nb = e.kv_blocks or max(e.max_seqs, e.max_batch) * self.max_blocks_per_seq + 2
        self.alloc = runtime().BlockAllocator(nb, self.bs)
        dev = self.device
        L = cfg.n_layers
        self.k_cache = torch.zeros(L, nb, self.nkv, self.bs, self.D, dtype=torch.bfloat16, device=dev)
        self.v_cache = torch.zeros_like(self.k_cache)
        cos_t, sin_t = oracle.rope_tables(rope_inv_freq(cfg), e.max_context + e.steps_per_graph + 2)
        self.cos_t, self.sin_t = cos_t.to(dev), sin_t.to(dev)
        self._alloc_decode_buffers()
        with self._on_stream():
            self._build_packed_weights()
        self._graphs: Dict[int, "torch.cuda.CUDAGraph"] = {}
        self._next_sid = 0

    def _on_stream(self):
        if self.stream is not None:
            return torch.cuda.stream(self.stream)
        import contextlib

        return contextlib.nullcontext()

    def _build_packed_weights(self) -> None:
        mode = str(self.ecfg.packed_weights).lower()
        self.packed = False
        if mode not in ("auto", "on", "off"):
            raise EngineError(f"packed_weights: auto, on or off, got {self.ecfg.packed_weights!r}")
        why = None
        if mode == "off":
            why = "switched off"
        elif not self.on_gpu:
            why = "not on a GPU"
        elif self.cfg.is_moe or self.tp.size != 1:
            why = "dense models at TP = 1 only"
        elif self.ecfg.max_batch > ops.GEMV_PACKED_MAX_M:
            why = f"max_batch {self.ecfg.max_batch} decodes on the MFMA form"
        if why is None and self.w.p_lm_head is None and not any(L.p_qkv or L.p_gu or L.p_down for L in self.w.layers):
            with_o = not (self.ecfg.max_batch == 1 and all(self.ao_chunks))
            need = self.w.packed_demand(with_o)
            free = torch.cuda.mem_get_info(self.device)[0]
            if need == 0:
                why = "no weight with K a multiple of 2048"
            elif mode == "auto" and need + PACKED_MARGIN_BYTES > free:
                why = f"the twin ({need / 2**30:.2f} GiB) does not fit in {free / 2**30:.2f} GiB free"
            else:
                st = self.w.pack_decode_weights(with_o)
                log.info("%s: packed weights on: %d of %d tensors, %.2f GiB beside %.2f GiB bf16, raw rows <= %.3f %%",
                         self.name, st["packed"], st["tensors"], st["bytes"] / 2**30, self.w.nbytes() / 2**30,
                         100 * st["raw_share"])
        if why is not None:
            log.info("%s: packed weights off: %s", self.name, why)
            return
        self.packed = True

    def _alloc_decode_buffers(self) -> None:
        B, dev, c = self.ecfg.max_batch, self.device, self.cfg
        i32 = dict(dtype=torch.int32, device=dev)
        self.tokens_in = torch.zeros(B, **i32)
        self.positions = torch.zeros(B, **i32)
        self.seq_lens = torch.ones(B, **i32)
        self.slots = torch.zeros(B, **i32)
        self.block_tables = torch.zeros(B, self.max_blocks_per_seq, **i32)
        self.cap = self.ecfg.max_context + self.ecfg.steps_per_graph + 1
        self.out_tokens = torch.zeros(B, self.cap, **i32)
        self.out_count = torch.zeros(B, **i32)
        self.next_tok = torch.zeros(B, **i32)
        self.inv_temp = torch.ones(B, dtype=torch.float32, device=dev)
        self.top_k = torch.zeros(B, **i32)
        self.top_p = torch.ones(B, dtype=torch.float32, device=dev)
        self.seeds = torch.zeros(B, dtype=torch.int64, device=dev)
        bf = dict(dtype=torch.bfloat16, device=dev)
        self.h = torch.zeros(B, c.hidden, **bf)
        self.q = torch.zeros(B, self.w.q_size, **bf)
        self.attn = torch.zeros(B, self.w.q_size, **bf)
        self.act = torch.zeros(B, self.w.inter, **bf)
        self.logits_local = torch.zeros(B, self.w.vocab_local, dtype=torch.float32, device=dev)
        self.logits = (self.logits_local if self.tp.size == 1
                       else torch.zeros(B, c.vocab, dtype=torch.float32, device=dev))
        self._gather_buf = (None if self.tp.size == 1 else
                            torch.zeros(self.tp.size, B, self.w.vocab_local, dtype=torch.float32, device=dev))
        ctxmax = self.ecfg.max_context + self.ecfg.steps_per_graph + 2
        self.attn_buckets = attn_buckets(ctxmax, split_blocks_per_head(self.nh, self.nkv),
                                         ops.FUSED_ATTN_MAX_KEYS if self.bs % 32 == 0 else 0, self.nh // self.nkv,
                                         self.nkv, rows=self.ecfg.max_batch)
        self.ao_chunks: List[int] = [0] * len(self.attn_buckets)
        self.ao_nc = 0
        self.window = int(c.sliding_window) if 0 < c.sliding_window < ctxmax else 0
        if (self.on_gpu and self.ecfg.attn_oproj and B == 1 and self.bs % 32 == 0 and not self.window
                and (self.tp.size == 1 or self.ecfg.tp_attn_oproj)):
            self.ao_nc = ops.attn_oproj_grid(c.hidden, self.nh, self.nkv, self.D)
            if self.ao_nc:
                lo = self.ecfg.attn_oproj_min_chunk
                self.ao_chunks = [ch if ch >= lo and (ch <= 256 or self.bs % 64 == 0) else 0
                                  for ch in (ops.attn_oproj_chunk(cap, self.ao_nc) for cap, _, _, _ in self.attn_buckets)]
                self.ao_ws = ops.attn_oproj_workspace(c.hidden, self.nh, self.nkv, self.D, self.ao_nc, dev)
        self.qa_plan: List[Optional[tuple]] = [None] * len(self.attn_buckets)
        if (self.on_gpu and B == 1 and not self.window and not c.qkv_bias
                and ops.qkv_attn_supported(self.nh, self.nkv, self.D, c.hidden)):
            self.qa_plan, self.ao_chunks = qkv_attn_plan(self.attn_buckets, self.ao_chunks, str(self.ecfg.qkv_attn),
                                                         (self.nh + 2 * self.nkv) * self.D, self.bs)
            if any(self.qa_plan):
                self.qa_ws = ops.qkv_attn_workspace(self.nh, self.nkv, self.D, dev)
        self.qa_buckets = [p is not None for p in self.qa_plan]
        self.ao_router = [False] * len(self.attn_buckets)
        if (self.ao_nc and c.is_moe and self.tp.size == 1 and not self.w.ep and self.ecfg.ao_router
                and c.n_experts <= 8 and not self.mfma_decode):
            self.ao_router = [bool(ch) and ops.attn_oproj_form(c.hidden, self.nh, self.nkv, self.D, self.ao_nc, ch) == 2
                              for ch in self.ao_chunks]
            if any(self.ao_router):
                self.ao_rws = ops.attn_oproj_router_workspace(self.nkv, self.ao_nc, dev)
        self.qa_o = (any(self.qa_plan) and self.ecfg.qkv_attn_o
                     and ops.qkv_attn_o_supported(self.nh, self.D, c.hidden))
        max_chunks = max([gc for _, _, gc, _ in self.attn_buckets] + [p[1] for p in self.qa_plan if p])
        self.attn_part, self.attn_counters = ops.decode_attn_workspace(B, self.nh, self.nkv, self.D, max_chunks, dev)
        self.attn_fault = torch.zeros(1, dtype=torch.int32, device=dev) if self.on_gpu else None
        if self.on_gpu:
            P = ops.sample_parts()
            self.ws_v = torch.zeros(B, P, dtype=torch.float32, device=dev)
            self.ws_i = torch.zeros(B, P, dtype=torch.int32, device=dev)
        else:
            self.ws_v = self.ws_i = None
        if c.is_moe:
            k = c.top_k_experts
            self.xn = torch.zeros(B, c.hidden, **bf)
            self.router_logits = torch.zeros(B, c.n_experts, dtype=torch.float32, device=dev)
            self.moe_w = torch.zeros(B, k, dtype=torch.float32, device=dev)
            self.moe_ids = torch.zeros(B, k, **i32)
            self.moe_act = torch.zeros(B * k, self.w.inter, **bf)
            self.moe_y = torch.zeros(B * k, c.hidden, **bf)
            self.moe_lw = torch.zeros(B, k, dtype=torch.float32, device=dev)
            self.moe_lids = torch.zeros(B, k, **i32)
        if self.on_gpu:
            self.host_tokens = torch.zeros(B, self.cap, dtype=torch.int32, pin_memory=True)
            self.host_count = torch.zeros(B, dtype=torch.int32, pin_memory=True)

    def new_sequence(self) -> Sequence:
        self._next_sid += 1
        return Sequence(self._next_sid)

    def free_sequence(self, seq: Sequence) -> None:
        if seq.blocks:
            self.alloc.free(seq.blocks)
            seq.blocks = []
        seq.length = 0
        seq.logits = None
        seq.has_logits = False

    def truncate(self, seq: Sequence, length: int) -> None:
        if not 0 <= length <= seq.length:
            raise EngineError(f"truncate to {length} of a {seq.length}-token sequence")
        seq.length = length
        seq.logits = None
        seq.has_logits = False

    def _reserve(self, seq: Sequence, total_tokens: int) -> None:
        need = self.alloc.blocks_for(total_tokens) - len(seq.blocks)
        if total_tokens > self.max_blocks_per_seq * self.bs:
            raise EngineError(f"context {total_tokens} exceeds engine max_context {self.ecfg.max_context}")
        if need > 0:
            got = self.alloc.allocate(need)
            if not got:
                raise EngineError(f"KV cache exhausted ({self.alloc.num_free} blocks free, need {need})")
            seq.blocks.extend(got)

    def _block_table(self, seqs: List[Sequence]) -> torch.Tensor:
        bt = torch.zeros(len(seqs), self.max_blocks_per_seq, dtype=torch.int32)
        for i, s in enumerate(seqs):
            bt[i, : len(s.blocks)] = torch.tensor(s.blocks, dtype=torch.int32)
        return bt.to(self.device, non_blocking=True) if self.on_gpu else bt

    @torch.no_grad()
    def prefill(self, seqs: List[Sequence], token_lists: List[List[int]], want_logits: bool = True) -> None:
        self._check_usable()
        with self._on_stream(), trace.span("prefill", engine=self.name, tokens=sum(len(t) for t in token_lists)):
            pending = [(s, list(t)) for s, t in zip(seqs, token_lists) if t]
            chunk = self.ecfg.prefill_chunk
            while pending:
                batch, rest, budget, finals = [], [], chunk, set()
                for s, t in pending:
                    if budget <= 0:
                        rest.append((s, t))
                        continue
                    take = t[:budget]
                    batch.append((s, take))
                    budget -= len(take)
                    if len(take) < len(t):
                        rest.append((s, t[len(take):]))
                    else:
                        finals.add(s)
                self._prefill_chunk(batch, want_logits, finals)
                pending = rest

    def _prefill_chunk(self, batch, want_logits: bool, finals) -> None:
        dev, c = self.device, self.cfg
        ids, pos, slots, q_start, q_lens, ctx_lens = [], [], [], [], [], []
        for s, toks in batch:
            self._reserve(s, s.length + len(toks))
            q_start.append(len(ids))
            q_lens.append(len(toks))
            for i, t in enumerate(toks):
                p = s.length + i
                ids.append(t)
                pos.append(p)
                slots.append(s.blocks[p // self.bs] * self.bs + p % self.bs)
            s.length += len(toks)
            ctx_lens.append(s.length)
        T = len(ids)
        i32 = dict(dtype=torch.int32)
        ids_d = torch.tensor(ids, **i32).to(dev, non_blocking=True)
        pos_d = torch.tensor(pos, **i32).to(dev, non_blocking=True)
        slots_d = torch.tensor(slots, **i32).to(dev, non_blocking=True)
        qs_d = torch.tensor(q_start, **i32).to(dev, non_blocking=True)
        ql_d = torch.tensor(q_lens, **i32).to(dev, non_blocking=True)
        cl_d = torch.tensor(ctx_lens, **i32).to(dev, non_blocking=True)
        bt = self._block_table([s for s, _ in batch])
        max_qlen = max(q_lens)
        max_ctx = max(ctx_lens)
        ksplit, kmin = (ops.attn_prefill_plan(len(batch), max_qlen, max_ctx, self.nh, self.nkv, D=self.D, bs=self.bs,
                                              window=self.window)
                        if ids_d.is_cuda else (1, 1))
        pws = (ops.attn_prefill_workspace(ksplit, T, self.nh, self.D, dev, len(batch), self.nkv, max_qlen)
               if ksplit > 1 else None)

        h = ops.embedding(ids_d, self.w.embed)
        attn = torch.empty(T, self.w.q_size, dtype=torch.bfloat16, device=dev)
        qbuf = torch.empty(T, self.w.q_size, dtype=torch.bfloat16, device=dev)
        sp = self._sp_plan(T)
        if sp is not None:
            Ts, gbuf, pbuf = sp
            r0 = self.tp.rank * Ts
            hs = torch.zeros(Ts, c.hidden, dtype=torch.bfloat16, device=dev)
            mine = max(0, min(T, r0 + Ts) - r0)
            if mine:
                hs[:mine].copy_(h[r0:r0 + mine])
            del h
        for li, Lw in enumerate(self.w.layers):
            if sp is not None:
                xn = self._sp_gather(ops.rmsnorm(hs, Lw.ln1, c.rms_eps), gbuf, T)
            else:
                xn = ops.rmsnorm(h, Lw.ln1, c.rms_eps)
            qkv = ops.linear(xn, Lw.w_qkv, EPI_BF16)
            ops.rope_kv_write(qkv, pos_d, self.cos_t, self.sin_t, self.k_cache[li], self.v_cache[li], slots_d,
                              self.nh, self.nkv, self.D, self.bs, qbuf, bias=Lw.b_qkv)
            ops.attn_prefill(qbuf, self.k_cache[li], self.v_cache[li], bt, qs_d, ql_d, cl_d, attn, max_qlen,
                             self.nh, self.nkv, self.D, self.bs, self.scale, max_ctx=max_ctx, ksplit=ksplit, kmin=kmin,
                             ws=pws, window=self.window)
            if sp is not None:
                self._sp_row_parallel(lambda out: ops.linear(attn, Lw.w_o, EPI_RESADD, out=out), hs, pbuf, T)
                if c.is_moe and self.w.ep:
                    self._moe_ep_a2a(ops.rmsnorm(hs, Lw.ln2, c.rms_eps), Lw, hs)
                    continue
                xn = self._sp_gather(ops.rmsnorm(hs, Lw.ln2, c.rms_eps), gbuf, T)
                if c.is_moe:
                    self._sp_row_parallel(lambda out: self._moe(xn, Lw, out, reduce=False), hs, pbuf, T)
                else:
                    act = ops.linear(xn, Lw.w_gu, EPI_SILU)
                    self._sp_row_parallel(lambda out: ops.linear(act, Lw.w_down, EPI_RESADD, out=out), hs, pbuf, T)
                continue
            self._row_parallel(attn, Lw.w_o, h)
            xn = ops.rmsnorm(h, Lw.ln2, c.rms_eps)
            if c.is_moe:
                self._moe(xn, Lw, h)
            else:
                act = ops.linear(xn, Lw.w_gu, EPI_SILU)
                self._row_parallel(act, Lw.w_down, h)
        if sp is not None:
            h = self._sp_gather(hs, sp[1], T)
        sel = [i for i, (s, _) in enumerate(batch) if want_logits and s in finals]
        for i0 in range(0, len(sel), ops.GEMV_MAX_M):
            part = sel[i0:i0 + ops.GEMV_MAX_M]
            last_d = torch.tensor([q_start[i] + q_lens[i] - 1 for i in part], dtype=torch.int32).to(dev)
            hl = ops.gather_rows(h, last_d, 1)
            lg = torch.empty(len(part), self.w.vocab_local, dtype=torch.float32, device=dev)
            ops.linear(hl, self.w.lm_head, EPI_F32, out=lg, norm_w=self.w.final_norm, eps=c.rms_eps,
                       mfma=self.mfma_decode)
            for j, i in enumerate(part):
                s = batch[i][0]
                s.logits = lg[j]
                s.has_logits = True

    def _sp_plan(self, T: int):
        n = self.tp.size
        if n == 1 or not self.ecfg.sequence_parallel or T < max(self.ecfg.sp_min_tokens, n):
            return None
        Ts = (T + n - 1) // n
        H = self.cfg.hidden
        gbuf = torch.empty(n * Ts, H, dtype=torch.bfloat16, device=self.device)
        pbuf = torch.empty(n * Ts, H, dtype=torch.bfloat16, device=self.device)
        return Ts, gbuf, pbuf

    def _sp_gather(self, xs: torch.Tensor, gbuf: torch.Tensor, T: int) -> torch.Tensor:
        self.tp.all_gather_rows(xs, gbuf.view(self.tp.size, xs.shape[0], xs.shape[1]))
        return gbuf[:T]

    def _sp_row_parallel(self, accumulate, hs: torch.Tensor, pbuf: torch.Tensor, T: int) -> None:
        Ts = hs.shape[0]
        r0 = self.tp.rank * Ts
        pbuf.zero_()
        pbuf[r0:r0 + Ts].copy_(hs)
        accumulate(pbuf[:T])
        self.tp.reduce_scatter_rows(pbuf, hs)

    def _row_parallel(self, x: torch.Tensor, W: torch.Tensor, h: torch.Tensor, Wp=None) -> None:
        car = self.tp.custom_fused if self.ecfg.fused_ar else None
        if car is not None and h.is_cuda and x.shape[0] <= 2 and not self.mfma_decode and h.is_contiguous():
            car.gemv_allreduce(x, W, h)
            return
        ops.linear(x, W, EPI_RESADD if self.tp.rank == 0 else EPI_BF16, out=h, mfma=self.mfma_decode, Wp=Wp)
        self.tp.all_reduce_(h)

    def _expert_ffn(self, A: torch.Tensor, ids: torch.Tensor, Lw) -> torch.Tensor:
        c = self.cfg
        n, k = ids.shape
        E_l, I_l, H = Lw.w_gu.shape[0], self.w.inter, c.hidden
        y = torch.empty(n * k, H, dtype=torch.bfloat16, device=A.device)
        if n == 0:
            return y
        if not A.is_cuda:
            for p in range(n * k):
                e = int(ids.view(-1)[p])
                if e < 0:
                    y[p].zero_()
                    continue
                gu = (A[p // k:p // k + 1].float() @ Lw.w_gu[e].float().t()).to(torch.bfloat16)
                y[p] = (oracle.silu_mul_interleaved(gu).float() @ Lw.w_down[e].float().t()).to(torch.bfloat16)[0]
            return y
        if n <= ops.MOE_GEMV_MAX_M:
            act = torch.empty(n * k, I_l, dtype=torch.bfloat16, device=A.device)
            ops.moe_gemv(A, Lw.w_gu, ids, k, act, 2 * I_l, H, EPI_SILU)
            ops.moe_gemv(act, Lw.w_down, ids, 1, y, H, I_l, EPI_BF16)
            return y
        tile = ops.moe_tile(n * k, E_l)
        mt = ops.moe_max_tiles(n * k, E_l, tile)
        sr = torch.empty(mt * tile, dtype=torch.int32, device=A.device)
        te = torch.empty(mt, dtype=torch.int32, device=A.device)
        tc = torch.empty(1, dtype=torch.int32, device=A.device)
        ops.moe_align(ids, E_l, sr, te, tc, tile=tile)
        act = torch.empty(n * k, I_l, dtype=torch.bfloat16, device=A.device)
        ops.moe_gemm(A, Lw.w_gu, sr, te, tc, act, 2 * I_l, H, mt, k, epi=EPI_SILU, tile=tile)
        ops.moe_gemm(act, Lw.w_down, sr, te, tc, y, H, I_l, mt, 1, tile=tile)
        return y

    def _route(self, xn: torch.Tensor, Lw):
        c = self.cfg
        T, k = xn.shape[0], c.top_k_experts
        w = torch.empty(T, k, dtype=torch.float32, device=xn.device)
        ids = torch.empty(T, k, dtype=torch.int32, device=xn.device)
        if xn.is_cuda and xn.is_contiguous() and ops.moe_route_fused_supported(c.n_experts, c.hidden):
            ops.moe_route_fused(xn, Lw.w_router, k, w, ids)
            return w, ids
        rl = ops.linear(xn, Lw.w_router, EPI_F32)
        ops.moe_route(rl, k, w, ids)
# ... 566 lines not shown
```

llm_consensus_amd/models/transformer.py:

```python

from __future__ import annotations

import math
import zlib
from typing import List, Optional

import torch

from ..parallel.comm import TPGroup, shard_range
from .config import ModelConfig


class LayerWeights:
    TENSORS = ("ln1", "ln2", "w_qkv", "w_o", "w_gu", "w_down", "w_router", "b_qkv")
    PACKED = ("p_qkv", "p_o", "p_gu", "p_down")
    __slots__ = TENSORS + PACKED

    def __init__(self):
        for s in self.__slots__:
            setattr(self, s, None)


class TransformerWeights:
    def __init__(self, cfg: ModelConfig, tp: TPGroup, device: torch.device, seed: int,
                 init_scale: float = 1.0, source=None, expert_parallel: bool = False):
        if source is None and cfg.checkpoint:
            from .checkpoint import HFCheckpoint

            source = HFCheckpoint(cfg.checkpoint, cfg)
        self.source = source
        self.cfg = cfg
        self.tp = tp
        self.device = device
        self.seed = seed
        self.init_scale = init_scale
        if cfg.n_heads % tp.size or cfg.n_kv_heads % tp.size or cfg.intermediate % tp.size or cfg.vocab % tp.size:
            raise ValueError(f"{cfg.name}: not shardable with tp={tp.size}")
        self.ep = bool(expert_parallel and cfg.is_moe and tp.size > 1)
        if self.ep and cfg.n_experts % tp.size:
            raise ValueError(f"{cfg.name}: {cfg.n_experts} experts not shardable over ep={tp.size}")
        self.n_local_experts = cfg.n_experts // tp.size if self.ep else cfg.n_experts
        self.e0 = tp.rank * self.n_local_experts if self.ep else 0
        self.nh = cfg.n_heads // tp.size
        self.nkv = cfg.n_kv_heads // tp.size
        self.inter = cfg.intermediate if self.ep else cfg.intermediate // tp.size
        self.vocab_local = cfg.vocab // tp.size
        self.q_size = self.nh * cfg.head_dim
        self.kv_size = self.nkv * cfg.head_dim
        self.qkv_size = self.q_size + 2 * self.kv_size
        self.layers: List[LayerWeights] = []
        self.p_lm_head = None
        self._build()
        self.source = None

    def _gen(self, name: str, shape, std: float, mean: float = 0.0) -> torch.Tensor:
        s = (zlib.crc32(name.encode()) ^ (self.seed * 0x9E3779B1)) & 0x7FFFFFFFFFFF
        g = torch.Generator(device=self.device)
        g.manual_seed(s)
        t = torch.randn(*shape, generator=g, device=self.device, dtype=torch.float32)
        if std != 1.0:
            t.mul_(std)
        if mean != 0.0:
            t.add_(mean)
        return t.to(torch.bfloat16)

    def _full(self, name: str, shape, kind: str = "linear") -> torch.Tensor:
        if self.source is not None:
            t = self.source.get(name)
            if tuple(t.shape) != tuple(shape):
                raise ValueError(f"checkpoint tensor {name}: shape {tuple(t.shape)} != expected {tuple(shape)}")
            return t.to(device=self.device, dtype=torch.bfloat16)
        if kind == "embed":
            return self._gen(name, shape, 1.0)
        if kind == "norm":
            return self._gen(name, shape, 0.02, 1.0)
        return self._gen(name, shape, self.init_scale / math.sqrt(shape[1]))

    def _linear(self, name: str, n_out: int, n_in: int) -> torch.Tensor:
        return self._full(name, (n_out, n_in))

    def _build(self) -> None:
        c, r, n = self.cfg, self.tp.rank, self.tp.size
        D = c.head_dim
        with torch.no_grad():
            self.embed = self._full("embed", (c.vocab, c.hidden), "embed")
            self.final_norm = self._full("final_norm", (c.hidden,), "norm")
            lm = self._linear("lm_head", c.vocab, c.hidden)
            v0, v1 = shard_range(c.vocab, r, n)
            self.lm_head = lm[v0:v1].contiguous()
            del lm
            for i in range(c.n_layers):
                L = LayerWeights()
                p = f"layers.{i}."
                L.ln1 = self._full(p + "ln1", (c.hidden,), "norm")
                L.ln2 = self._full(p + "ln2", (c.hidden,), "norm")
                qkv = self._linear(p + "w_qkv", c.qkv_size, c.hidden)
                q0, q1 = shard_range(c.n_heads, r, n)
                k0, k1 = shard_range(c.n_kv_heads, r, n)
                qs = qkv[q0 * D:q1 * D]
                ks = qkv[c.q_size + k0 * D:c.q_size + k1 * D]
                vs = qkv[c.q_size + c.kv_size + k0 * D:c.q_size + c.kv_size + k1 * D]
                L.w_qkv = torch.cat([pair_interleave_heads(qs, D), pair_interleave_heads(ks, D), vs], 0).contiguous()
                del qkv
                if c.qkv_bias:
                    if self.source is not None:
                        b = self._full(p + "b_qkv", (c.qkv_size,))
                    else:
                        b = self._gen(p + "b_qkv", (c.qkv_size,), 1.0)
                    b = b.view(-1, 1)
                    bq, bk = b[q0 * D:q1 * D], b[c.q_size + k0 * D:c.q_size + k1 * D]
                    bv = b[c.q_size + c.kv_size + k0 * D:c.q_size + c.kv_size + k1 * D]
                    L.b_qkv = torch.cat([pair_interleave_heads(bq, D), pair_interleave_heads(bk, D), bv],
                                        0).reshape(-1).contiguous()
                wo = self._linear(p + "w_o", c.hidden, c.q_size)
                L.w_o = wo[:, q0 * D:q1 * D].contiguous()
                del wo
                i0, i1 = shard_range(c.intermediate, r, n)
                if c.is_moe:
                    L.w_router = self._linear(p + "w_router", c.n_experts, c.hidden)
                    gus, downs = [], []
                    for e in range(self.e0, self.e0 + self.n_local_experts):
                        gu = self._linear(p + f"experts.{e}.w_gu", 2 * c.intermediate, c.hidden)
                        dn = self._linear(p + f"experts.{e}.w_down", c.hidden, c.intermediate)
                        if self.ep:
                            gus.append(gu)
                            downs.append(dn)
                        else:
                            gus.append(gu[2 * i0:2 * i1])
                            downs.append(dn[:, i0:i1])
                    L.w_gu = torch.stack(gus).contiguous()
                    L.w_down = torch.stack(downs).contiguous()
                    del gus, downs
                else:
                    gu = self._linear(p + "w_gu", 2 * c.intermediate, c.hidden)
                    L.w_gu = gu[2 * i0:2 * i1].contiguous()
                    del gu
                    dn = self._linear(p + "w_down", c.hidden, c.intermediate)
                    L.w_down = dn[:, i0:i1].contiguous()
                    del dn
                self.layers.append(L)

    def to(self, device) -> "TransformerWeights":
        device = torch.device(device)
        self.device = device
        self.embed = self.embed.to(device)
        self.final_norm = self.final_norm.to(device)
        self.lm_head = self.lm_head.to(device)
        for L in self.layers:
            for s in LayerWeights.TENSORS:
                t = getattr(L, s)
                if t is not None:
                    setattr(L, s, t.to(device))
        return self

    def packed_demand(self, with_o: bool = True) -> int:
        from ..ops import wpack

        ts = [self.lm_head]
        for L in self.layers:
            ts += [L.w_qkv, L.w_gu, L.w_down] + ([L.w_o] if with_o else [])
        return sum(wpack.packed_nbytes(*t.shape) for t in ts if t.dim() == 2 and wpack.packable_shape(*t.shape))

    def pack_decode_weights(self, with_o: bool = True) -> dict:
        from ..ops import wpack

        if self.cfg.is_moe:
            raise ValueError("packed weights: dense models only")
        st = {"tensors": 0, "packed": 0, "bytes": 0, "raw_share": 0.0}

        def twin(W):
            st["tensors"] += 1
            pw, share = wpack.pack_if_worthwhile(W)
            st["raw_share"] = max(st["raw_share"], share)
            if pw is not None:
                st["packed"] += 1
                st["bytes"] += pw.nbytes()
            return pw

        self.p_lm_head = twin(self.lm_head)
        for L in self.layers:
            L.p_qkv, L.p_gu, L.p_down = twin(L.w_qkv), twin(L.w_gu), twin(L.w_down)
            L.p_o = twin(L.w_o) if with_o else None
        return st

    def packed_nbytes(self) -> int:
        tot = self.p_lm_head.nbytes() if self.p_lm_head is not None else 0
        for L in self.layers:
            tot += sum(getattr(L, s).nbytes() for s in LayerWeights.PACKED if getattr(L, s) is not None)
        return tot

    def nbytes(self) -> int:
        tot = self.embed.numel() + self.final_norm.numel() + self.lm_head.numel()
        for L in self.layers:
            for s in LayerWeights.TENSORS:
                t = getattr(L, s)
                if t is not None:
                    tot += t.numel()
        return tot * 2


def pair_interleave_heads(rows: torch.Tensor, D: int) -> torch.Tensor:
    n = rows.shape[0] // D
    half = D // 2
    r = rows.view(n, 2, half, -1).transpose(1, 2)
    return r.reshape(n * D, -1)


def full_reference_weights(cfg: ModelConfig, seed: int, device="cpu", init_scale: float = 1.0) -> TransformerWeights:
    return TransformerWeights(cfg, TPGroup.single(), torch.device(device), seed, init_scale)


def split_for_rank(full: Optional[TransformerWeights], cfg: ModelConfig, tp: TPGroup, device, seed: int,
                   init_scale: float = 1.0) -> TransformerWeights:
    return TransformerWeights(cfg, tp, torch.device(device), seed, init_scale)
```

llm_consensus_amd/ops/__init__.py:

```python

from __future__ import annotations

import os
from typing import Optional

import torch

from ..utils.native import kernels
from . import oracle, wpack

EPI_BF16, EPI_F32, EPI_RESADD, EPI_SILU, EPI_ROPE = 0, 1, 2, 3, 4
GEMV_MAX_M = 32
GEMV_PACKED_MAX_M = 2
MOE_GEMVM_MAX_TOKENS = 16
MOE_GEMV_MAX_M = 4


def _p(t: Optional[torch.Tensor]) -> int:
    return 0 if t is None else t.data_ptr()


def _s(t: torch.Tensor) -> int:
    return torch.cuda.current_stream(t.device).cuda_stream


def _bf16(t: torch.Tensor, name: str) -> None:
    if t.dtype != torch.bfloat16:
        raise TypeError(f"{name}: expected bfloat16, got {t.dtype}")


def lane_exchange_check(x: torch.Tensor) -> torch.Tensor:
    if not x.is_cuda:
        raise RuntimeError("lane_exchange_check: GPU only")
    x = x.contiguous().float()
    nb = x.numel() // 64
    out = torch.empty(nb * 64, 10, 2, dtype=torch.float32, device=x.device)
    kernels().lane_exchange_check(_p(x), _p(out), nb, _s(x))
    return out


def rmsnorm(x: torch.Tensor, w: torch.Tensor, eps: float, out: Optional[torch.Tensor] = None) -> torch.Tensor:
    if not x.is_cuda:
        r = oracle.rmsnorm(x, w, eps)
        return out.copy_(r) if out is not None else r
    _bf16(x, "rmsnorm.x")
    H = x.shape[-1]
    x2 = x.reshape(-1, H)
    if out is None:
        out = torch.empty_like(x)
    kernels().rmsnorm(_p(x2), _p(w), _p(out), x2.shape[0], H, x2.stride(0), out.reshape(-1, H).stride(0), float(eps), _s(x))
    return out


def embedding(ids: torch.Tensor, table: torch.Tensor, out: Optional[torch.Tensor] = None) -> torch.Tensor:
    if not table.is_cuda:
        r = oracle.embedding(ids, table)
        return out.copy_(r) if out is not None else r
    T = ids.numel()
    if out is None:
        out = torch.empty(T, table.shape[1], dtype=table.dtype, device=table.device)
    kernels().embedding(_p(ids), _p(table), _p(out), T, table.shape[1], table.shape[0], _s(table))
    return out


def silu_mul_interleaved(gu: torch.Tensor, out: Optional[torch.Tensor] = None) -> torch.Tensor:
    if not gu.is_cuda:
        r = oracle.silu_mul_interleaved(gu)
        return out.copy_(r) if out is not None else r
    T, I2 = gu.shape
    if out is None:
        out = torch.empty(T, I2 // 2, dtype=gu.dtype, device=gu.device)
    kernels().silu_mul_interleaved(_p(gu), _p(out), T, I2 // 2, _s(gu))
    return out


def _use_packed(Wp, M: int, N: int, K: int, mfma: bool) -> bool:
    return Wp is not None and M <= GEMV_PACKED_MAX_M and not mfma and Wp.N == N and Wp.K == K


def linear(x: torch.Tensor, W: torch.Tensor, epi: int = EPI_BF16, out: Optional[torch.Tensor] = None,
           norm_w: Optional[torch.Tensor] = None, eps: float = 1e-5, mfma: bool = False,
           Wp: Optional["wpack.PackedWeight"] = None) -> torch.Tensor:
    if not x.is_cuda:
        return oracle.linear(x, W, epi, out, norm_w, eps)
    _bf16(x, "linear.x")
    _bf16(W, "linear.W")
    M, K = x.shape
    N = W.shape[0]
    if W.shape[1] != K:
        raise ValueError(f"linear: x[{M},{K}] vs W{tuple(W.shape)}")
    if out is None:
        if epi == EPI_RESADD:
            raise ValueError("EPI_RESADD needs out")
        n_out = N // 2 if epi == EPI_SILU else N
        out = torch.empty(M, n_out, dtype=torch.float32 if epi == EPI_F32 else torch.bfloat16, device=x.device)
    if _use_packed(Wp, M, N, K, mfma):
        kernels().gemv_p13(M, _p(x), x.stride(0), _p(norm_w), float(eps), _p(W), _p(Wp.planes), _p(Wp.hdr), _p(out),
                           out.stride(0), N, K, epi, _s(x))
        return out
    if M <= 4 or (M <= GEMV_MAX_M and K % 128 == 0 and x.stride(0) % 8 == 0):
        kernels().gemv(M, _p(x), x.stride(0), _p(norm_w), float(eps), _p(W), _p(out), out.stride(0), N, K, epi,
                       int(mfma), _s(x))
        return out
    if norm_w is not None:
        x = rmsnorm(x, norm_w, eps)
    kernels().gemm(_p(x), x.stride(0), _p(W), W.stride(0), _p(out), out.stride(0), M, N, K, epi, _s(x))
    return out


def gemm(x: torch.Tensor, W: torch.Tensor, epi: int = EPI_BF16, out: Optional[torch.Tensor] = None) -> torch.Tensor:
    if not x.is_cuda:
        return oracle.linear(x, W, epi, out)
    M, K = x.shape
    N = W.shape[0]
    if out is None:
        n_out = N // 2 if epi == EPI_SILU else N
        out = torch.empty(M, n_out, dtype=torch.float32 if epi == EPI_F32 else torch.bfloat16, device=x.device)
    kernels().gemm(_p(x), x.stride(0), _p(W), W.stride(0), _p(out), out.stride(0), M, N, K, epi, _s(x))
    return out


def gemm128(x: torch.Tensor, W: torch.Tensor, epi: int = EPI_BF16, out: Optional[torch.Tensor] = None) -> torch.Tensor:
    if not x.is_cuda:
        return oracle.linear(x, W, epi, out)
    M, K = x.shape
    N = W.shape[0]
    if out is None:
        n_out = N // 2 if epi == EPI_SILU else N
        out = torch.empty(M, n_out, dtype=torch.float32 if epi == EPI_F32 else torch.bfloat16, device=x.device)
    kernels().gemm_t128(_p(x), x.stride(0), _p(W), W.stride(0), _p(out), out.stride(0), M, N, K, epi, _s(x))
    return out


def _gemm_kind(x, W, epi, out, kind):
    if not x.is_cuda:
        return oracle.linear(x, W, epi, out)
    M, K = x.shape
    N = W.shape[0]
    if out is None:
        n_out = N // 2 if epi == EPI_SILU else N
        out = torch.empty(M, n_out, dtype=torch.float32 if epi == EPI_F32 else torch.bfloat16, device=x.device)
    kernels().gemm_kind(_p(x), x.stride(0), _p(W), W.stride(0), _p(out), out.stride(0), M, N, K, epi, kind, _s(x))
    return out


def gemm256(x: torch.Tensor, W: torch.Tensor, epi: int = EPI_BF16, out: Optional[torch.Tensor] = None) -> torch.Tensor:
    return _gemm_kind(x, W, epi, out, 0)


def gemm_narrow(x: torch.Tensor, W: torch.Tensor, epi: int = EPI_BF16, out: Optional[torch.Tensor] = None) -> torch.Tensor:
    return _gemm_kind(x, W, epi, out, 1)


def gemm_plan(M: int, N: int) -> str:
    return ("256x256", "128x192")[kernels().gemm_plan(int(M), int(N))]


def gemv(x: torch.Tensor, W: torch.Tensor, epi: int = EPI_BF16, out: Optional[torch.Tensor] = None,
         norm_w: Optional[torch.Tensor] = None, eps: float = 1e-5, mfma: bool = False) -> torch.Tensor:
    if not x.is_cuda:
        return oracle.linear(x, W, epi, out, norm_w, eps)
    M, K = x.shape
    N = W.shape[0]
    if out is None:
        n_out = N // 2 if epi == EPI_SILU else N
        out = torch.empty(M, n_out, dtype=torch.float32 if epi == EPI_F32 else torch.bfloat16, device=x.device)
    kernels().gemv(M, _p(x), x.stride(0), _p(norm_w), float(eps), _p(W), _p(out), out.stride(0), N, K, epi, int(mfma),
                   _s(x))
    return out


def gemvm(x: torch.Tensor, W: torch.Tensor, epi: int = EPI_BF16, out: Optional[torch.Tensor] = None,
          norm_w: Optional[torch.Tensor] = None, eps: float = 1e-5, form: int = 0) -> torch.Tensor:
    if not x.is_cuda:
        return oracle.linear(x, W, epi, out, norm_w, eps)
    M, K = x.shape
    N = W.shape[0]
    if out is None:
        n_out = N // 2 if epi == EPI_SILU else N
        out = torch.empty(M, n_out, dtype=torch.float32 if epi == EPI_F32 else torch.bfloat16, device=x.device)
    kernels().gemvm(M, _p(x), x.stride(0), _p(norm_w), float(eps), _p(W), _p(out), out.stride(0), N, K, epi, form,
                    _s(x))
    return out


def _qkv_bias(bias, n: int, name: str):
    if bias is None:
        return None
    _bf16(bias, name + ".bias")
    if not bias.is_cuda or bias.dim() != 1 or bias.numel() != n or not bias.is_contiguous():
        raise ValueError(f"{name}: bias must be a contiguous GPU tensor of {n} elements, got {tuple(bias.shape)}")
    return bias


def rope_kv_write(qkv, positions, cos_t, sin_t, k_cache, v_cache, slots, nh, nkv, D, bs, q_out, bias=None) -> None:
    if not qkv.is_cuda:
        oracle.rope_kv_write(qkv, positions, cos_t, sin_t, k_cache, v_cache, slots, nh, nkv, D, bs, q_out, bias)
        return
    T = qkv.shape[0]
    bias = _qkv_bias(bias, (nh + 2 * nkv) * D, "rope_kv_write")
    kernels().rope_kv_write(_p(qkv), qkv.stride(0), _p(q_out), q_out.stride(0), _p(positions), _p(cos_t), _p(sin_t),
                            _p(k_cache), _p(v_cache), _p(slots), T, nh, nkv, D, bs, _s(qkv), _p(bias))


def qkv_rope(x, W, norm_w, eps, q_out, k_cache, v_cache, positions, slots, cos_t, sin_t, nh, nkv, D, bs,
             mfma: bool = False, Wp: Optional["wpack.PackedWeight"] = None, bias=None) -> None:
    if not x.is_cuda:
        qkv = oracle.linear(x, W, EPI_BF16, None, norm_w, eps)
        oracle.rope_kv_write(qkv, positions, cos_t, sin_t, k_cache, v_cache, slots, nh, nkv, D, bs, q_out, bias)
        return
    M, K = x.shape
    bias = _qkv_bias(bias, W.shape[0], "qkv_rope")
    if _use_packed(Wp, M, W.shape[0], K, mfma):
        kernels().gemv_qkv_rope_p13(M, _p(x), x.stride(0), _p(norm_w), float(eps), _p(W), _p(Wp.planes), _p(Wp.hdr),
                                    W.shape[0], K, _p(q_out), q_out.stride(0), _p(k_cache), _p(v_cache),
                                    _p(positions), _p(slots), _p(cos_t), _p(sin_t), nh, nkv, D, bs, _s(x), _p(bias))
        return
    if M > 4 and (K % 128 != 0 or x.stride(0) % 8 != 0):
        qkv = linear(x, W, EPI_BF16, norm_w=norm_w, eps=eps)
        rope_kv_write(qkv, positions, cos_t, sin_t, k_cache, v_cache, slots, nh, nkv, D, bs, q_out, bias)
        return
    kernels().gemv_qkv_rope(M, _p(x), x.stride(0), _p(norm_w), float(eps), _p(W), W.shape[0], K, _p(q_out),
                            q_out.stride(0), _p(k_cache), _p(v_cache), _p(positions), _p(slots), _p(cos_t), _p(sin_t),
                            nh, nkv, D, bs, int(mfma), _s(x), _p(bias))


FUSED_ATTN_MAX_KEYS = 4096
FUSED_CHUNK = 128


ATTN_CTR_PITCH = 32


def decode_attn_workspace(B, nh, nkv, D, max_chunks, device, fused: bool = False):
    G = nh // nkv
    dev = torch.device(device)
    groups = kernels().attn_decode_groups(max_chunks) if dev.type == "cuda" else 0
    part = torch.zeros(B, nkv, max_chunks + groups, G, D + 4, dtype=torch.float32, device=dev)
    counters = torch.zeros(B, nkv, 2 + groups, ATTN_CTR_PITCH, dtype=torch.int32, device=dev)
    return part, counters


def attn_decode(q, k_cache, v_cache, block_tables, seq_lens, out, part, counters, nh, nkv, D, bs, chunk, scale,
                grid_chunks: Optional[int] = None, fused: bool = False, fault: Optional[torch.Tensor] = None,
                window: int = 0):
    window = int(window)
    if window < 0:
        raise ValueError("attn_decode: window must be >= 0")
    if not q.is_cuda:
        out.copy_(oracle.attn_decode(q, k_cache, v_cache, block_tables, seq_lens, nh, nkv, D, bs, scale, window))
        return out
    B = q.shape[0]
    groups = counters.shape[-2] - 2
    max_chunks = part.shape[2] - groups
    gc = max_chunks if grid_chunks is None else min(grid_chunks, max_chunks)
    if (part.shape[-1] != D + 4 or counters.shape[0] < B or groups < 0 or counters.shape[-1] != ATTN_CTR_PITCH
            or kernels().attn_decode_groups(max_chunks) != groups):
        raise ValueError("attn_decode: workspace does not match (use decode_attn_workspace)")
    kernels().attn_decode(_p(q), q.stride(0), _p(k_cache), _p(v_cache), _p(block_tables), block_tables.stride(0),
                          _p(seq_lens), _p(part), _p(counters), _p(out), out.stride(0), B, nh, nkv, D, bs,
                          k_cache.shape[0], chunk, gc, max_chunks, float(scale), 1 if fused else 0, _p(fault), _s(q),
                          window)
    return out


def qkv_attn_supported(nh: int, nkv: int, D: int, K: int) -> bool:
    return kernels().qkv_attn_check(nh, nkv, D, K) == 0


def qkv_attn_workspace(nh: int, nkv: int, D: int, device):
    dev = torch.device(device)
    return (torch.zeros((nh + 2 * nkv) * D // 2, dtype=torch.int64, device=dev),
            torch.zeros(3 * ATTN_CTR_PITCH, dtype=torch.int32, device=dev))


QKV_ATTN_O_MAX_K = 2048


def qkv_attn_o_supported(nh: int, D: int, H: int) -> bool:
    k_o = nh * D
    return k_o % 512 == 0 and k_o <= QKV_ATTN_O_MAX_K and H % 2 == 0


def qkv_attn(x, W, norm_w, eps, q_out, k_cache, v_cache, positions, slots, cos_t, sin_t, block_table, seq_len, out,
             part, counters, ws, nh, nkv, D, bs, chunk, grid_chunks, scale, fault: Optional[torch.Tensor] = None,
             w_o: Optional[torch.Tensor] = None, h: Optional[torch.Tensor] = None, add_resid: bool = True, car=None):
    if not x.is_cuda:
        qkv_rope(x[:1], W, norm_w, eps, q_out[:1], k_cache, v_cache, positions[:1], slots[:1], cos_t, sin_t, nh, nkv,
                 D, bs)
        out[:1].copy_(oracle.attn_decode(q_out[:1], k_cache, v_cache, block_table[:1], seq_len[:1], nh, nkv, D, bs,
                                         scale))
        if w_o is not None:
            if car is not None:
                raise ValueError("qkv_attn: the fused all-reduce runs on GPU ranks only")
            oracle.linear(out[:1], w_o, EPI_RESADD if add_resid else EPI_BF16, h[:1])
        return
    groups = counters.shape[-2] - 2
    max_chunks = part.shape[2] - groups
    if part.shape[-1] != D + 4 or counters.shape[-1] != ATTN_CTR_PITCH or grid_chunks > max_chunks:
        raise ValueError("qkv_attn: workspace does not match (decode_attn_workspace / qkv_attn_workspace)")
    gran, hctr = ws
    o_mode = 0 if w_o is None else (3 if car is not None else (1 if add_resid else 2))
    if o_mode and hctr.numel() < 3 * ATTN_CTR_PITCH:
        raise ValueError("qkv_attn: the o-role needs the 3-line counter workspace (qkv_attn_workspace)")
    bases, host, rank, world, cap = (([], 0, 0, 1, 0) if car is None else
                                     (car.bases, car.host_dev, car.rank, car.world, car.cap))
    kernels().qkv_attn(_p(x), _p(norm_w), float(eps), _p(W), x.shape[-1], _p(q_out), _p(k_cache), _p(v_cache),
                       _p(positions), _p(slots), _p(cos_t), _p(sin_t), _p(block_table), block_table.shape[-1],
                       _p(seq_len), _p(part), _p(counters), _p(out), nh, nkv, D, bs, k_cache.shape[0], chunk,
                       grid_chunks, max_chunks, float(scale), _p(fault), _p(gran), _p(hctr), o_mode, _p(w_o), _p(h),
                       0 if h is None else h.shape[-1], bases, host, rank, world, cap, _s(x))


ATTN_OPROJ_MAX_CHUNK = 512
ATTN_OPROJ_MODE = int(os.environ.get("LLMC_ATTN_OPROJ_MODE", "7"))
ATTN_OPROJ_MIN_CHUNK = 256


def attn_oproj_min_chunk(alone: bool = False) -> int:
    if os.environ.get("LLMC_ATTN_OPROJ") == "all" or alone:
        return 32
    return ATTN_OPROJ_MIN_CHUNK


def attn_oproj_grid(H: int, nh: int, nkv: int, D: int) -> int:
    top = max(1, 256 // max(1, nkv))
    for nc in sorted({top} | {n for n in (H // 128, H // 64, H // 32) if 0 < n <= top}, reverse=True):
        if kernels().attn_oproj_check(H, nh, nkv, D, nc, nh * D) == 0:
            return nc
    return 0


def attn_oproj_chunk(ctx_cap: int, nc: int) -> int:
    per = -(-ctx_cap // nc)
    ch = max(32, (per + 31) // 32 * 32)
    if ch > 256:
        ch = (per + 63) // 64 * 64
    return ch if ch <= ATTN_OPROJ_MAX_CHUNK else 0


def attn_oproj_workspace(H: int, nh: int, nkv: int, D: int, nc: int, device):
    G = nh // nkv
    dev = torch.device(device)
    part = torch.zeros(2 * nkv, nc, G, D // 4 + 1, 4, dtype=torch.float32, device=dev)
    handoff = torch.zeros(nkv, G * D // 4, 4, dtype=torch.int32, device=dev)
    tile_part = torch.zeros(nc, nkv, H // nc, dtype=torch.int64, device=dev)
    counters = torch.zeros((nkv + nc + 2) * 16, dtype=torch.int32, device=dev)
    return part, handoff, tile_part, counters


def attn_oproj_form(H: int, nh: int, nkv: int, D: int, nc: int, chunk: int, mode: int = -1, world: int = 1) -> int:
    return int(kernels().attn_oproj_form(H, nh, nkv, D, nc, chunk, ATTN_OPROJ_MODE if mode < 0 else mode, world))


def attn_oproj_router_workspace(nkv: int, nc: int, device):
    if nkv * nc > 256:
        raise ValueError("attn_oproj router: at most 256 blocks")
    dev = torch.device(device)
    return (torch.zeros(9, 256, dtype=torch.int64, device=dev), torch.zeros(16, dtype=torch.int32, device=dev))


def attn_oproj(q, k_cache, v_cache, block_table, seq_len, w_o, h, attn_out, ws, nh, nkv, D, bs, chunk, nc, scale,
               fault: Optional[torch.Tensor] = None, stamps: Optional[torch.Tensor] = None, mode: int = -1,
               add_resid: bool = True, car=None, router=None) -> None:
    H = h.shape[-1]
    if not q.is_cuda:
        if car is not None:
            raise ValueError("attn_oproj: the fused all-reduce runs on GPU ranks only")
        a = oracle.attn_decode(q[:1], k_cache, v_cache, block_table[:1], seq_len[:1], nh, nkv, D, bs, scale)
        attn_out[:1].copy_(a)
        oracle.linear(attn_out[:1], w_o, EPI_RESADD if add_resid else EPI_BF16, h[:1])
        if router is not None:
            raise ValueError("attn_oproj: the router partials are a GPU form")
        return
    if chunk <= 0 or chunk * nc < 1 or nc != ws[0].shape[1]:
        raise ValueError("attn_oproj: chunk / workspace do not match (attn_oproj_chunk, attn_oproj_workspace)")
    part, handoff, tile_part, counters = ws
    bases, host, rank, world, cap = (([], 0, 0, 1, 0) if car is None else
                                     (car.bases, car.host_dev, car.rank, car.world, car.cap))
    rt = (None, None, 0.0, 0, 0, None, None, None, None)
    if router is not None:
        if car is not None:
            raise ValueError("attn_oproj: the fused router runs on one-GPU engines only")
        norm_w, W_r, eps, k, w_out, ids_out, (rpart, repoch) = router
        if tuple(rpart.shape) != (9, 256) or W_r.shape[1] != H:
            raise ValueError("attn_oproj: router workspace / weights do not match")
        rt = (norm_w, W_r, float(eps), W_r.shape[0], int(k), w_out, ids_out, rpart, repoch)
    kernels().attn_oproj(_p(q), _p(k_cache), _p(v_cache), _p(block_table), block_table.shape[-1], _p(seq_len), _p(w_o),
                         _p(h), _p(attn_out), _p(part), _p(handoff), _p(tile_part), _p(counters), _p(fault), H, nh, nkv,
                         D, bs, k_cache.shape[0], chunk, nc, float(scale),
                         ATTN_OPROJ_MODE if mode < 0 else mode, _p(stamps), int(bool(add_resid)), bases, host, rank,
                         world, cap, _p(rt[0]), _p(rt[1]), rt[2], rt[3], rt[4], _p(rt[5]), _p(rt[6]), _p(rt[7]),
                         _p(rt[8]), _s(h))


PREFILL_KSPLIT = int(os.environ.get("LLMC_PREFILL_KSPLIT", "-1"))
PREFILL_KMIN = int(os.environ.get("LLMC_PREFILL_KMIN", "8"))


def attn_prefill_plan(B, max_qlen, max_ctx, nh, nkv, ksplit=None, kmin=None, D=128, bs=64, window=0):
    k = PREFILL_KSPLIT if ksplit is None else int(ksplit)
    if window > 0 and (ksplit is None or k < 0):
        return 1, int(PREFILL_KMIN if kmin is None else kmin)
    if k < 0:
        return tuple(kernels().attn_prefill_plan(B, int(max_qlen), int(max_ctx), nh, nkv, int(D), int(bs)))
    return max(1, min(k, 4)), int(PREFILL_KMIN if kmin is None else kmin)


def attn_prefill_counters(B, max_qlen, nh, nkv) -> int:
    return int(kernels().attn_prefill_counters(int(B), int(max_qlen), int(nh), int(nkv)))


def attn_prefill_workspace(ksplit, T, nh, D, device, B=1, nkv=1, max_qlen=None):
    return (torch.empty(ksplit * T * nh * (D + 2), dtype=torch.float32, device=device),
            torch.zeros(max(1, attn_prefill_counters(B, max_qlen or T, nh, nkv)), dtype=torch.int32, device=device))


def attn_prefill(q, k_cache, v_cache, block_tables, q_start, q_lens, ctx_lens, out, max_qlen, nh, nkv, D, bs, scale,
                 max_ctx=None, ksplit=None, kmin=None, ws=None, form=None, window: int = 0):
    window = int(window)
    if window < 0:
        raise ValueError("attn_prefill: window must be >= 0")
    if max_ctx is not None and window >= max_ctx:
        window = 0
    if not q.is_cuda:
        return oracle.attn_prefill(q, k_cache, v_cache, block_tables, q_start, q_lens, ctx_lens, nh, nkv, D, bs,
                                   scale, out, window)
    B = q_lens.shape[0]
    T = q.shape[0]
    k, km = attn_prefill_plan(B, max_qlen, max_qlen if max_ctx is None else max_ctx, nh, nkv, ksplit, kmin, D, bs,
                               window)
    part = ctr = 0
    if k > 1:
        need_c = attn_prefill_counters(B, max_qlen, nh, nkv)
        if ws is None or ws[0].numel() < k * T * nh * (D + 2) or ws[1].numel() < need_c:
            ws = attn_prefill_workspace(k, T, nh, D, q.device, B, nkv, max_qlen)
        part, ctr = _p(ws[0]), _p(ws[1])
    try:
        kernels().attn_prefill(_p(q), q.stride(0), _p(k_cache), _p(v_cache), _p(block_tables), block_tables.stride(0),
                               _p(q_start), _p(q_lens), _p(ctx_lens), _p(out), out.stride(0), B, int(max_qlen), nh,
                               nkv, D, bs, float(scale), k, km, part, ctr, T, -1 if form is None else int(form), _s(q),
                               window)
    except Exception:
        if k > 1:
            ws[1].zero_()
        raise
    return out


def sample_parts() -> int:
    return kernels().sample_parts()


def sample(logits, inv_temp, top_k, top_p, seeds, positions, next_tok, workspace_v=None, workspace_i=None,
           tokens_in=None, seq_lens=None, slots=None, block_tables=None, bs=0, out_tokens=None, out_count=None,
           use_topkp: bool = False):
    if not logits.is_cuda:
        tok = oracle.sample(logits, inv_temp, top_k, top_p, seeds, positions)
        next_tok.copy_(tok)
        _advance_cpu(tok, tokens_in, positions, seq_lens, slots, block_tables, bs, out_tokens, out_count)
        return next_tok
    B, V = logits.shape
    cap = out_tokens.shape[1] if out_tokens is not None else 0
    kernels().sample(_p(logits), logits.stride(0), B, V, _p(inv_temp), _p(top_k), _p(top_p), _p(seeds), _p(positions),
                     _p(workspace_v), _p(workspace_i), _p(next_tok), _p(tokens_in), _p(seq_lens), _p(slots),
                     _p(block_tables), block_tables.stride(0) if block_tables is not None else 0, bs, _p(out_tokens),
                     _p(out_count), cap, 1 if use_topkp else 0, _s(logits))
    return next_tok


def _advance_cpu(tok, tokens_in, positions, seq_lens, slots, block_tables, bs, out_tokens, out_count):
    if tokens_in is None:
        return
    B = tok.shape[0]
    for b in range(B):
        t = int(tok[b])
        if out_tokens is not None:
            c = int(out_count[b])
            if c < out_tokens.shape[1]:
                out_tokens[b, c] = t
            out_count[b] = c + 1
        if tokens_in is not None:
            tokens_in[b] = t
        if positions is not None:
            p = int(positions[b]) + 1
            positions[b] = p
            if seq_lens is not None:
                seq_lens[b] = p + 1
            if slots is not None and block_tables is not None:
                slots[b] = int(block_tables[b, p // bs]) * bs + p % bs


MOE_TILE = 128
MOE_TILE_LARGE = 256


def moe_tile(npairs: int, E: int) -> int:
    return MOE_TILE_LARGE if npairs >= MOE_TILE_LARGE * E else MOE_TILE


def moe_route(logits: torch.Tensor, k: int, w_out: torch.Tensor, ids_out: torch.Tensor):
    if not logits.is_cuda:
        w, ids = oracle.moe_route(logits, k)
        w_out.copy_(w)
        ids_out.copy_(ids)
        return w_out, ids_out
    T, E = logits.shape
    kernels().moe_route(_p(logits), T, E, k, _p(w_out), _p(ids_out), _s(logits))
    return w_out, ids_out


def moe_route_fused(x: torch.Tensor, W_router: torch.Tensor, k: int, w_out: torch.Tensor, ids_out: torch.Tensor):
    if not x.is_cuda:
        return moe_route(oracle.linear(x, W_router, EPI_F32), k, w_out, ids_out)
    T, H = x.shape
    kernels().moe_route_fused(_p(x), x.stride(0), _p(W_router), T, W_router.shape[0], H, k, _p(w_out), _p(ids_out),
                              _s(x))
    return w_out, ids_out

# ... 108 lines not shown
```

llm_consensus_amd/ops/wpack.py:

```python

from __future__ import annotations

from typing import Optional, Tuple

import torch

UNIT_ELEMS = 2048
UNIT_BYTES = 3328
RAW = 0xFF
MAX_RAW_SHARE = 0.01


class PackedWeight:

    __slots__ = ("planes", "hdr", "raw_rows", "N", "K")

    def __init__(self, planes: torch.Tensor, hdr: torch.Tensor, raw_rows: int, N: int, K: int):
        self.planes, self.hdr, self.raw_rows, self.N, self.K = planes, hdr, int(raw_rows), N, K

    @property
    def raw_share(self) -> float:
        return self.raw_rows / max(1, self.N)

    def nbytes(self) -> int:
        return self.planes.numel() + self.hdr.numel()


def packable_shape(N: int, K: int) -> bool:
    return N > 0 and K > 0 and K % UNIT_ELEMS == 0


def packed_nbytes(N: int, K: int) -> int:
    return N * (K // UNIT_ELEMS) * UNIT_BYTES + (N + 3) // 4 * 4


def _bits(W: torch.Tensor) -> torch.Tensor:
    if W.dtype != torch.bfloat16 or W.dim() != 2:
        raise TypeError("wpack: a bf16 [N, K] tensor")
    return W.contiguous().view(torch.int16).to(torch.int32) & 0xFFFF


def row_headers(W: torch.Tensor) -> torch.Tensor:
    hi7 = (_bits(W) >> 8) & 0x7F
    base = (hi7.max(dim=1).values - 15).clamp(min=0)
    raw = hi7.min(dim=1).values < base
    return torch.where(raw, torch.full_like(base, RAW), base).to(torch.uint8)


def _lane_order(t: torch.Tensor, U: int) -> torch.Tensor:
    N = t.shape[0]
    return t.view(N, U, 4, 64, 8).permute(0, 1, 3, 2, 4).reshape(N, U, 64, 32)


def pack_reference(W: torch.Tensor) -> PackedWeight:
    N, K = W.shape
    if not packable_shape(N, K):
        raise ValueError(f"wpack: K = {K} is not a multiple of {UNIT_ELEMS}")
    U = K // UNIT_ELEMS
    bits = _bits(W)
    hdr = row_headers(W)
    base = torch.where(hdr == RAW, torch.zeros_like(hdr), hdr).to(torch.int32)
    b = _lane_order(bits, U)
    low = (b & 0xFF).to(torch.uint8)
    code = (((b >> 8) & 0x7F) - base.view(N, 1, 1, 1)) & 0xF
    code = code.view(N, U, 64, 4, 2, 4)
    nib = (code[..., 0, :] | (code[..., 1, :] << 4)).to(torch.uint8)
    sign = (b >> 15).view(N, U, 64, 8, 4)
    sbyte = (sign << torch.arange(8, device=W.device).view(1, 1, 1, 8, 1)).sum(dim=3).to(torch.uint8)
    planes = torch.cat([low[..., :16].reshape(N, U, 1024), low[..., 16:].reshape(N, U, 1024),
                        nib.reshape(N, U, 1024), sbyte.reshape(N, U, 256)], dim=2).contiguous()
    hdr_pad = torch.zeros((N + 3) // 4 * 4, dtype=torch.uint8, device=W.device)
    hdr_pad[:N] = hdr
    return PackedWeight(planes, hdr_pad, int((hdr == RAW).sum()), N, K)


def unpack_reference(pw: PackedWeight, W: Optional[torch.Tensor] = None) -> torch.Tensor:
    N, K = pw.N, pw.K
    U = K // UNIT_ELEMS
    p = pw.planes.view(N, U, UNIT_BYTES).to(torch.int32)
    hdr = pw.hdr[:N].to(torch.int32)
    base = torch.where(hdr == RAW, torch.zeros_like(hdr), hdr).view(N, 1, 1, 1)
    low = torch.cat([p[..., :1024].reshape(N, U, 64, 16), p[..., 1024:2048].reshape(N, U, 64, 16)], dim=3)
    nib = p[..., 2048:3072].reshape(N, U, 64, 4, 4)
    code = torch.stack([nib & 0xF, nib >> 4], dim=4).reshape(N, U, 64, 32)
    sb = p[..., 3072:].reshape(N, U, 64, 1, 4)
    sign = ((sb >> torch.arange(8, device=p.device).view(1, 1, 1, 8, 1)) & 1).reshape(N, U, 64, 32)
    b = (sign << 15) | ((code + base) << 8) | low
    bits = b.view(N, U, 64, 4, 8).permute(0, 1, 3, 2, 4).reshape(N, K)
    out = (bits - ((bits & 0x8000) << 1)).to(torch.int16).view(torch.bfloat16)
    if W is not None:
        rows = hdr == RAW
        out[rows] = W[rows].to(out.device)
    return out


def pack(W: torch.Tensor) -> PackedWeight:
    if not W.is_cuda:
        return pack_reference(W)
    from ..utils.native import kernels

    N, K = W.shape
    if W.dtype != torch.bfloat16 or not packable_shape(N, K):
        raise ValueError(f"wpack: bf16 [N, K] with K a multiple of {UNIT_ELEMS}, got {W.dtype} {tuple(W.shape)}")
    W = W.contiguous()
    planes = torch.empty(N, K // UNIT_ELEMS, UNIT_BYTES, dtype=torch.uint8, device=W.device)
    hdr = torch.zeros((N + 3) // 4 * 4, dtype=torch.uint8, device=W.device)
    raw = torch.zeros(1, dtype=torch.int32, device=W.device)
    kernels().wpack13(W.data_ptr(), planes.data_ptr(), hdr.data_ptr(), raw.data_ptr(), N, K,
                      torch.cuda.current_stream(W.device).cuda_stream)
    return PackedWeight(planes, hdr, int(raw.item()), N, K)


def pack_if_worthwhile(W: torch.Tensor) -> Tuple[Optional[PackedWeight], float]:
    if W.dim() != 2 or not packable_shape(*W.shape):
        return None, 0.0
    pw = pack(W)
    return (pw if pw.raw_share <= MAX_RAW_SHARE else None), pw.raw_share
```

llm_consensus_amd/parallel/placement.py:

```python

from __future__ import annotations

import dataclasses
import os
from typing import Dict, List, Optional, Sequence

HBM_BYTES = 288 * 10**9
USABLE_FRACTION = 0.92


def packed_weights_mode() -> str:
    v = os.environ.get("LLMC_PACKED_WEIGHTS", "auto").strip().lower()
    return {"1": "on", "true": "on", "0": "off", "false": "off"}.get(v, v if v in ("auto", "on", "off") else "auto")


@dataclasses.dataclass
class ModelDemand:
    name: str
    weight_bytes: int
    kv_bytes: int
    tp: int = 1
    is_judge: bool = False


@dataclasses.dataclass
class Placement:
    gpus: Dict[str, List[int]]

    def models_on(self, gpu: int) -> List[str]:
        return [m for m, g in self.gpus.items() if gpu in g]

    def used_gpus(self) -> List[int]:
        return sorted({g for gs in self.gpus.values() for g in gs})


class PlacementError(Exception):
    pass


def decodes_alone(gpus: Dict[str, List[int]], name: str, concurrent: Sequence[str]) -> bool:
    mine = set(gpus[name])
    return not any(mine & set(gpus[o]) for o in concurrent if o != name and o in gpus)


def fused_ar_allowed(gpus: Dict[str, List[int]], name: str, concurrent: Sequence[str]) -> bool:
    if len(gpus[name]) <= 1:
        return True
    return decodes_alone(gpus, name, concurrent)


def _concurrent(gpus: Dict[str, List[int]], m: str, judge: Optional[str], concurrency: int,
                responders: Optional[Sequence[str]] = None) -> List[str]:
    if concurrency > 1:
        return [o for o in gpus if o != m]
    resp = set(responders) if responders is not None else {o for o in gpus if o != judge}
    if m not in resp:
        return []
    return [o for o in gpus if o != m and o in resp]


def fused_ar_plan(gpus: Dict[str, List[int]], judge: Optional[str], concurrency: int = 1,
                  responders: Optional[Sequence[str]] = None) -> Dict[str, bool]:
    return {m: fused_ar_allowed(gpus, m, _concurrent(gpus, m, judge, concurrency, responders)) for m in gpus}


def alone_plan(gpus: Dict[str, List[int]], judge: Optional[str], concurrency: int = 1,
               responders: Optional[Sequence[str]] = None) -> Dict[str, bool]:
    return {m: decodes_alone(gpus, m, _concurrent(gpus, m, judge, concurrency, responders)) for m in gpus}


def parse_pins(spec: str) -> Dict[str, List[int]]:
    pins: Dict[str, List[int]] = {}
    for item in filter(None, (x.strip() for x in (spec or "").split(","))):
        name, sep, gs = item.rpartition("=")
        if not sep or not name.strip():
            raise PlacementError(f"bad placement entry {item!r} (want model=gpu[+gpu...])")
        try:
            ids = [int(x) for x in gs.split("+")]
        except ValueError:
            raise PlacementError(f"bad GPU list in placement entry {item!r}") from None
        if len(set(ids)) != len(ids):
            raise PlacementError(f"duplicate GPU in placement entry {item!r}")
        pins[name.strip()] = ids
    return pins


def solve(demands: Sequence[ModelDemand], gpu_ids: Sequence[int], hbm_bytes: int = HBM_BYTES,
          pins: Optional[Dict[str, List[int]]] = None) -> Placement:
    gpu_ids = list(gpu_ids)
    if not gpu_ids:
        raise PlacementError("no GPUs available")
    cap = hbm_bytes * USABLE_FRACTION
    used = {g: 0.0 for g in gpu_ids}
    count = {g: 0 for g in gpu_ids}
    out: Dict[str, List[int]] = {}
    pins = dict(pins or {})
    unknown = sorted(set(pins) - {d.name for d in demands})
    if unknown:
        raise PlacementError(f"placement names models not in the run: {unknown}")

    def fits(g: int, b: float) -> bool:
        return used[g] + b <= cap

    def take(name: str, gs: List[int], per_gpu: float) -> None:
        for g in gs:
            used[g] += per_gpu
            count[g] += 1
        out[name] = gs

    for d in demands:
        gs = pins.get(d.name)
        if gs is None:
            continue
        bad = [g for g in gs if g not in used]
        if bad:
            raise PlacementError(f"{d.name}: placement GPU(s) {bad} not available (have {gpu_ids})")
        per = (d.weight_bytes + d.kv_bytes) / len(gs)
        if not all(fits(g, per) for g in gs):
            raise PlacementError(f"{d.name}: {per / 1e9:.1f} GB per GPU does not fit on {gs}")
        take(d.name, list(gs), per)
    demands = [dataclasses.replace(d) for d in demands if d.name not in pins]
    for d in sorted((d for d in demands if d.tp > 1), key=lambda d: -d.tp):
        if d.tp > len(gpu_ids):
            raise PlacementError(f"{d.name}: tp={d.tp} needs {d.tp} GPUs, only {len(gpu_ids)} available")
        per = (d.weight_bytes + d.kv_bytes) / d.tp
        groups = [gpu_ids[i:i + d.tp] for i in range(0, len(gpu_ids) - d.tp + 1, d.tp)]
        groups = [g for g in groups if all(fits(x, per) for x in g)]
        if not groups:
            raise PlacementError(f"{d.name}: no GPU group with {per / 1e9:.1f} GB free per GPU")
        best = min(groups, key=lambda g: (sum(count[x] for x in g), g[0]))
        take(d.name, best, per)
    singles = [d for d in demands if d.tp == 1 and not d.is_judge] + [d for d in demands if d.tp == 1 and d.is_judge]
    for d in singles:
        per = d.weight_bytes + d.kv_bytes
        cands = [g for g in gpu_ids if fits(g, per)]
        if not cands:
            raise PlacementError(f"{d.name}: needs {per / 1e9:.1f} GB, no GPU has that free")
        best = min(cands, key=lambda g: (count[g], used[g], g))
        take(d.name, [best], per)
    return Placement(out)


def describe(p: Placement) -> str:
    return "; ".join(f"{m}->{','.join(map(str, g))}" for m, g in sorted(p.gpus.items()))


_KFD_NODES = "/sys/class/kfd/kfd/topology/nodes"


def visible_gpu_count() -> int:
    try:
        nodes = sorted(os.listdir(_KFD_NODES), key=lambda d: int(d) if d.isdigit() else 1 << 30)
    except OSError:
        return -1
    n = 0
    for d in nodes:
        try:
            with open(os.path.join(_KFD_NODES, d, "gpu_id")) as f:
                if int(f.read().strip() or "0") == 0:
                    continue
            minor = None
            with open(os.path.join(_KFD_NODES, d, "properties")) as f:
                for line in f:
                    k, _, v = line.partition(" ")
                    if k == "drm_render_minor":
                        minor = int(v)
            if minor is None:
                continue
            fd = os.open(f"/dev/dri/renderD{minor}", os.O_RDWR | os.O_CLOEXEC)
            os.close(fd)
            n += 1
        except (OSError, ValueError):
            continue
    for var in ("ROCR_VISIBLE_DEVICES", "HIP_VISIBLE_DEVICES", "CUDA_VISIBLE_DEVICES"):
        v = os.environ.get(var)
        if v is None:
            continue
        kept = 0
        for x in (t.strip() for t in v.split(",")):
            if x == "":
                continue
            if not x.lstrip("-").isdigit():
                return -1
            if not 0 <= int(x) < n:
                break
            kept += 1
        n = min(n, kept)
    return n


def default_gpus(requested: Optional[List[int]] = None) -> List[int]:
    if requested:
        return list(requested)
    n = visible_gpu_count()
    if n <= 0:
        try:
            import torch

            n = torch.cuda.device_count()
        except Exception:
            n = 0
    return list(range(n))
```

Before: 483.6.

## Add 12-bit packed bf16 weight format with per-row exception records

Adds a lossless 12-bit weight packing: each bf16 keeps its low byte, sign, and a 3-bit exponent offset from a per-row base. Up to 16 outliers per row are stored in a record list and patched in during decode. The packed GEMV and fused QKV+RoPE kernels read 3072 bytes per 2048-element unit instead of 3328, which reduces weight bandwidth during memory-bound decode. In exchange the inner loop gains a scalar exception-scan branch, and an optional prefetch-depth-2 template path is added. The new format is the default through LLMC_PACKED_FORMAT=12, and rows with too many exceptions fall back to the 13-bit or raw format.

```diff
diff --git a/csrc/kernels/bindings.cpp b/csrc/kernels/bindings.cpp
--- a/csrc/kernels/bindings.cpp
+++ b/csrc/kernels/bindings.cpp
@@ -22,6 +22,12 @@
                            void*, int, void*, void*, const void*, const void*, const void*, const void*, int, int, int,
                            int, const void*, hipStream_t);
 int llmc_wpack13(const void*, void*, void*, void*, int, int, hipStream_t);
+int llmc_gemv_p12(int, const void*, int, const void*, float, const void*, const void*, const void*, void*, int, int, int,
+                  int, hipStream_t);
+int llmc_gemv_qkv_rope_p12(int, const void*, int, const void*, float, const void*, const void*, const void*, int, int,
+                           void*, int, void*, void*, const void*, const void*, const void*, const void*, int, int, int,
+                           int, const void*, hipStream_t);
+int llmc_wpack12(const void*, void*, void*, void*, int, int, hipStream_t);
 int llmc_gemvm(int, const void*, int, const void*, float, const void*, void*, int, int, int, int, int, hipStream_t);
 int llmc_moe_gemvm(int, const void*, int, const void*, float, const void*, const void*, int, int, void*, int, int, int,
                    int, hipStream_t);
@@ -145,6 +151,24 @@
   m.def("wpack13", [](ptr W, ptr planes, ptr hdr, ptr raw_count, int N, int K, ptr s) {
     check(llmc_wpack13(P(W), P(planes), P(hdr), P(raw_count), N, K, S(s)), "wpack13");
   });
+  m.def("gemv_p12", [](int M, ptr x, int xs, ptr nw, float eps, ptr W, ptr planes, ptr recs, ptr out, int os, int N,
+                       int K, int epi, ptr s) {
+    check(llmc_gemv_p12(M, P(x), xs, P(nw), eps, P(W), P(planes), P(recs), P(out), os, N, K, epi, S(s)), "gemv_p12");
+  });
+  m.def("gemv_qkv_rope_p12", [](int M, ptr x, int xs, ptr nw, float eps, ptr W, ptr planes, ptr recs, int N, int K,
+                                ptr qo, int qos, ptr kc, ptr vc, ptr pos, ptr slots, ptr cos_t, ptr sin_t, int nh,
+                                int nkv, int D, int bs, ptr s, ptr bias) {
+    check(llmc_gemv_qkv_rope_p12(M, P(x), xs, P(nw), eps, P(W), P(planes), P(recs), N, K, P(qo), qos, P(kc), P(vc),
+                                 P(pos), P(slots), P(cos_t), P(sin_t), nh, nkv, D, bs, P(bias), S(s)),
+          "gemv_qkv_rope_p12");
+  }, py::arg("M"), py::arg("x"), py::arg("x_stride"), py::arg("norm_w"), py::arg("eps"), py::arg("W"),
+     py::arg("planes"), py::arg("recs"), py::arg("N"), py::arg("K"), py::arg("q_out"), py::arg("q_stride"),
+     py::arg("k_cache"), py::arg("v_cache"), py::arg("positions"), py::arg("slots"), py::arg("cos_t"),
+     py::arg("sin_t"), py::arg("nh"), py::arg("nkv"), py::arg("D"), py::arg("bs"), py::arg("stream"),
+     py::arg("bias") = 0);
+  m.def("wpack12", [](ptr W, ptr planes, ptr recs, ptr counts, int N, int K, ptr s) {
+    check(llmc_wpack12(P(W), P(planes), P(recs), P(counts), N, K, S(s)), "wpack12");
+  });
   m.def("moe_gemvm", [](int P, ptr x, int xs, ptr nw, float eps, ptr W, ptr ids, int x_div, int E, ptr out, int os,
                         int N, int K, int epi, ptr s) {
     check(llmc_moe_gemvm(P, P(x), xs, P(nw), eps, P(W), P(ids), x_div, E, P(out), os, N, K, epi, S(s)), "moe_gemvm");
diff --git a/csrc/kernels/gemv.hip b/csrc/kernels/gemv.hip
--- a/csrc/kernels/gemv.hip
+++ b/csrc/kernels/gemv.hip
@@ -33,6 +33,8 @@
                          int out_stride, int N, int K, const RopeEpi& rope, const PackedW& pw, hipStream_t s) {
   constexpr int UNROLL = UNROLL_OVERRIDE ? UNROLL_OVERRIDE : (RPW == 1 ? 4 : (RPW == 2 ? 4 : (M <= 2 ? 4 : 2)));
   constexpr int WAVES = NT / kWave;
+  if (pw.planes != nullptr && pw.wf == WF_P12)
+    return launch_gemv_p12(M, NT, RPW, UNROLL, PRO, EPI, x, x_stride, nw, eps, W, pw, out, out_stride, N, K, rope, s);
   if (pw.planes != nullptr)
     return launch_gemv_p13<M, NT, RPW, PRO, EPI, UNROLL>(x, x_stride, nw, eps, W, pw, out, out_stride, N, K, rope, s);
   auto kern = gemv_kernel<M, NT, RPW, UNROLL, PRO, EPI, false>;
@@ -162,6 +164,18 @@
   return gemv_dispatch(M, x, x_stride, norm_w, eps, W, out, out_stride, N, K, epi, rope, pw, false, s);
 }
 
+extern "C" int llmc_gemv_p12(int M, const void* x, int x_stride, const void* norm_w, float eps, const void* W,
+                             const void* planes, const void* recs, void* out, int out_stride, int N, int K, int epi,
+                             hipStream_t s) {
+  if (epi == EPI_ROPE) return -5;
+  if (M < 1 || M > kGemvMaxM || K % kP13UnitElems != 0 || K > kP12MaxK || planes == nullptr || recs == nullptr ||
+      reinterpret_cast<uintptr_t>(recs) % 4 != 0)
+    return -1;
+  RopeEpi rope{};
+  const PackedW pw{static_cast<const uint8_t*>(planes), static_cast<const uint8_t*>(recs), WF_P12};
+  return gemv_dispatch(M, x, x_stride, norm_w, eps, W, out, out_stride, N, K, epi, rope, pw, false, s);
+}
+
 extern "C" int llmc_gemv_qkv_rope(int M, const void* x, int x_stride, const void* norm_w, float eps, const void* W,
                                   int N, int K, void* q_out, int q_stride, void* k_cache, void* v_cache,
                                   const void* positions, const void* slots, const void* cos_t, const void* sin_t,
@@ -184,6 +198,22 @@
                (const int32_t*)slots, (const float*)cos_t, (const float*)sin_t, nh, nkv, D, bs};
   rope.bias = static_cast<const bf16_t*>(bias);
   const PackedW pw{static_cast<const uint8_t*>(planes), static_cast<const uint8_t*>(hdr)};
+  return gemv_dispatch(M, x, x_stride, norm_w, eps, W, nullptr, 0, N, K, EPI_ROPE, rope, pw, false, s);
+}
+
+extern "C" int llmc_gemv_qkv_rope_p12(int M, const void* x, int x_stride, const void* norm_w, float eps,
+                                      const void* W, const void* planes, const void* recs, int N, int K, void* q_out,
+                                      int q_stride, void* k_cache, void* v_cache, const void* positions,
+                                      const void* slots, const void* cos_t, const void* sin_t, int nh, int nkv, int D,
+                                      int bs, const void* bias, hipStream_t s) {
+  if (N != (nh + 2 * nkv) * D || D % 2 != 0 || reinterpret_cast<uintptr_t>(bias) % 4 != 0) return -1;
+  if (M < 1 || M > kGemvMaxM || K % kP13UnitElems != 0 || K > kP12MaxK || planes == nullptr || recs == nullptr ||
+      reinterpret_cast<uintptr_t>(recs) % 4 != 0)
+    return -1;
+  RopeEpi rope{(bf16_t*)q_out, q_stride, (bf16_t*)k_cache, (bf16_t*)v_cache, (const int32_t*)positions,
+               (const int32_t*)slots, (const float*)cos_t, (const float*)sin_t, nh, nkv, D, bs};
+  rope.bias = static_cast<const bf16_t*>(bias);
+  const PackedW pw{static_cast<const uint8_t*>(planes), static_cast<const uint8_t*>(recs), WF_P12};
   return gemv_dispatch(M, x, x_stride, norm_w, eps, W, nullptr, 0, N, K, EPI_ROPE, rope, pw, false, s);
 }
 
diff --git a/csrc/kernels/gemv_core.h b/csrc/kernels/gemv_core.h
--- a/csrc/kernels/gemv_core.h
+++ b/csrc/kernels/gemv_core.h
@@ -25,11 +25,15 @@
   const bf16_t* bias;
 };
 
-enum { WF_BF16 = 0, WF_P13 = 1 };
+enum { WF_BF16 = 0, WF_P13 = 1, WF_P12 = 2 };
 constexpr int kP13UnitElems = 2048, kP13UnitBytes = 3328, kP13Raw = 0xff;
+constexpr int kP12UnitBytes = 3072, kP12Raw = 0xff, kP12MaxExc = 16, kP12RecDwords = 1 + kP12MaxExc;
+constexpr int kP12MaxK = 65536 - kP13UnitElems;
+constexpr uint32_t kP12End = 0xffffffffu;
 struct PackedW {
   const uint8_t* planes;
   const uint8_t* hdr;
+  int wf = WF_P13;
 };
 struct P13Unit {
   u32x4 l0, l1, n;
@@ -51,18 +55,51 @@
   return w;
 }
 
+int launch_gemv_p12(int M, int NT, int RPW, int UNROLL, int pro, int epi, const void* x, int x_stride, const void* nw,
+                    float eps, const void* W, const PackedW& pw, void* out, int out_stride, int N, int K,
+                    const RopeEpi& rope, hipStream_t s);
+struct P12Unit {
+  u32x4 l0, l1, n;
+};
+template <int C>
+__device__ __forceinline__ u32x4 p12_chunk(const P12Unit& p, uint32_t base4) {
+  const uint32_t n = p.n[C];
+  const uint32_t h0 = ((n & 0x07070707u) + base4) | ((n << 4) & 0x80808080u);
+  const uint32_t h1 = (((n >> 4) & 0x07070707u) + base4) | (n & 0x80808080u);
+  const u32x4& L = C < 2 ? p.l0 : p.l1;
+  const uint32_t lw0 = L[(2 * C) & 3], lw1 = L[(2 * C + 1) & 3];
+  u32x4 w;
+  w[0] = __builtin_amdgcn_perm(h0, lw0, 0x05010400u);
+  w[1] = __builtin_amdgcn_perm(h0, lw0, 0x07030602u);
+  w[2] = __builtin_amdgcn_perm(h1, lw1, 0x05010400u);
+  w[3] = __builtin_amdgcn_perm(h1, lw1, 0x07030602u);
+  return w;
+}
+__device__ __forceinline__ void p12_patch(u32x4& w, uint32_t ent, int lane) {
+  const bool mine = lane == static_cast<int>((ent >> 3) & 63u);
+  const uint32_t e = ent & 7u, val = ent >> 16;
+  const uint32_t keep = (e & 1u) ? 0x0000ffffu : 0xffff0000u, ins = (e & 1u) ? val << 16 : val;
+#pragma unroll
+  for (int d = 0; d < 4; ++d)
+    if (mine && (e >> 1) == static_cast<uint32_t>(d)) w[d] = (w[d] & keep) | ins;
+}
+
 constexpr int kGemvMaxM = 2, kGemvmMaxM = 32, kMoeGemvmMaxTokens = 16;
 int gemvm_dispatch(int M, const void* x, int x_stride, const void* norm_w, float eps, const void* W, void* out,
                    int out_stride, int N, int K, int epi, const RopeEpi& rope, hipStream_t st, int form = 0);
 
-template <int M, int NT, int RPW, int UNROLL, int PRO, int EPI, bool EXPERT = false, int WF = WF_BF16>
+template <int M, int NT, int RPW, int UNROLL, int PRO, int EPI, bool EXPERT = false, int WF = WF_BF16, int DEPTH = 1>
 __device__ __forceinline__ void gemv_block(const int bx, const int by, char* smem, const bf16_t* __restrict__ x,
                                            int x_stride, const bf16_t* __restrict__ norm_w, float eps,
                                            const bf16_t* __restrict__ W, void* __restrict__ out, int out_stride, int N,
                                            int K, const int32_t* __restrict__ expert_ids, int x_div, const RopeEpi& rope,
                                            const CarArgs& ar, const PackedW& pw = PackedW{}) {
   constexpr int WAVES = NT / kWave;
-  constexpr bool P13 = WF == WF_P13;
+  constexpr bool P12 = WF == WF_P12;
+  constexpr bool P13 = WF == WF_P13 || P12;
+  using PUnit = std::conditional_t<P12, P12Unit, P13Unit>;
+  constexpr int kUnitBytes = P12 ? kP12UnitBytes : kP13UnitBytes;
+  static_assert(DEPTH == 1 || (DEPTH == 2 && P13), "prefetch depth: the packed loop, 1 or 2 batches ahead");
   static_assert(!P13 || (!EXPERT && EPI != EPI_AR && EPI != EPI_COMBINE && UNROLL % 4 == 0 && M <= 2),
                 "packed weights: the dense one- and two-row decode forms");
   constexpr bool PAIR_LDS = (EPI == EPI_SILU || EPI == EPI_ROPE) && RPW == 1;
@@ -127,20 +164,24 @@
   }
   constexpr int UB = P13 ? UNROLL / 4 : 1;
   const int units = K / kP13UnitElems;
-  P13Unit cur13[P13 ? RPW : 1][UB];
+  PUnit cur13[P13 ? RPW : 1][UB];
+  PUnit nx13[P13 && DEPTH == 2 ? RPW : 1][UB];
   const uint8_t* prow[RPW];
   uint32_t hdr_w[RPW];
-  auto issue13 = [&](P13Unit (&dst)[P13 ? RPW : 1][UB], int ubase) {
+  const uint32_t* rec12[RPW];
+  uint32_t nxt12[RPW], idx12[RPW];
+  auto issue13 = [&](PUnit (&dst)[P13 ? RPW : 1][UB], int ubase) {
 #pragma unroll
     for (int j = 0; j < UB; ++j) {
       const int u = min(ubase + j, units - 1);
 #pragma unroll
       for (int r = 0; r < (P13 ? RPW : 1); ++r) {
-        const uint8_t* p = prow[r] + static_cast<int64_t>(u) * kP13UnitBytes + lane * 16;
+        const uint8_t* p = prow[r] + static_cast<int64_t>(u) * kUnitBytes + lane * 16;
         dst[r][j].l0 = load16<true>(p);
         dst[r][j].l1 = load16<true>(p + 1024);
         dst[r][j].n = load16<true>(p + 2048);
-        dst[r][j].s = __builtin_nontemporal_load(reinterpret_cast<const uint32_t*>(p + 3072 - lane * 12));
+        if constexpr (!P12)
+          dst[r][j].s = __builtin_nontemporal_load(reinterpret_cast<const uint32_t*>(p + 3072 - lane * 12));
       }
     }
   };
@@ -150,10 +191,19 @@
 #pragma unroll
     for (int r = 0; r < RPW; ++r) {
       const int n_u = min((bx * WAVES + w_u) * RPW + r, N - 1);
-      hdr_w[r] = ld_scalar(reinterpret_cast<const uint32_t*>(pw.hdr + (n_u & ~3))) >> ((n_u & 3) * 8) & 0xffu;
-      prow[r] = pw.planes + static_cast<int64_t>(n_u) * units * kP13UnitBytes;
+      if constexpr (P12) {
+        rec12[r] = reinterpret_cast<const uint32_t*>(pw.hdr) + static_cast<int64_t>(n_u) * kP12RecDwords;
+        hdr_w[r] = ld_scalar(rec12[r]);
+        nxt12[r] = ld_scalar(rec12[r] + 1);
+      } else {
+        hdr_w[r] = ld_scalar(reinterpret_cast<const uint32_t*>(pw.hdr + (n_u & ~3))) >> ((n_u & 3) * 8) & 0xffu;
+      }
+      prow[r] = pw.planes + static_cast<int64_t>(n_u) * units * kUnitBytes;
     }
     issue13(cur13, 0);
+    if constexpr (DEPTH == 2) {
+      if (UB < units) issue13(nx13, UB);
+    }
   } else {
     issue(cur, lane);
   }
@@ -359,14 +409,18 @@
     uint32_t base4[RPW];
 #pragma unroll
     for (int r = 0; r < RPW; ++r) {
-      raw |= hdr_w[r] == kP13Raw;
-      base4[r] = hdr_w[r] * 0x01010101u;
+      raw |= (hdr_w[r] & 0xffu) == kP13Raw;
+      base4[r] = (hdr_w[r] & 0xffu) * 0x01010101u;
+      if constexpr (P12) {
+        idx12[r] = 0;
+        if ((hdr_w[r] >> 8 & 0xffu) == 0) nxt12[r] = kP12End;
+      }
     }
     if (raw) {
       issue(cur, lane);
       stream_bf16();
     } else {
-      auto consume13 = [&](const P13Unit (&wv)[RPW][UB], int ubase, auto masked) {
+      auto consume13 = [&](const PUnit (&wv)[RPW][UB], int ubase, auto masked) {
 #pragma unroll
         for (int j = 0; j < UB; ++j) {
           if (!decltype(masked)::value || ubase + j < units) {
@@ -375,7 +429,20 @@
               constexpr int C = decltype(cc)::value;
               u32x4 w[RPW];
 #pragma unroll
-              for (int r = 0; r < RPW; ++r) w[r] = p13_chunk<C>(wv[r][j], base4[r]);
+              for (int r = 0; r < RPW; ++r) {
+                if constexpr (P12) {
+                  w[r] = p12_chunk<C>(wv[r][j], base4[r]);
+                  const uint32_t q = 4u * static_cast<uint32_t>(ubase + j) + C;
+                  while ((nxt12[r] >> 9 & 0x7fu) == q) {
+                    p12_patch(w[r], nxt12[r], lane);
+                    ++idx12[r];
+                    const uint32_t e = ld_scalar(rec12[r] + 1 + min(idx12[r], static_cast<uint32_t>(kP12MaxExc - 1)));
+                    nxt12[r] = idx12[r] < (hdr_w[r] >> 8 & 0xffu) ? e : kP12End;
+                  }
+                } else {
+                  w[r] = p13_chunk<C>(wv[r][j], base4[r]);
+                }
+              }
 #pragma unroll
               for (int m = 0; m < M; ++m) {
                 const u32x4 xx = xv[m * nchunk + cb + C * kWave];
@@ -393,13 +460,26 @@
       const int it13 = (units + UB - 1) / UB;
       int u0 = 0;
       for (int it = 0; it + 1 < it13; ++it, u0 += UB) {
-        P13Unit nxt[RPW][UB];
-        issue13(nxt, u0 + UB);
-        consume13(cur13, u0, Full{});
-#pragma unroll
-        for (int j = 0; j < UB; ++j)
-#pragma unroll
-          for (int r = 0; r < RPW; ++r) cur13[r][j] = nxt[r][j];
+        PUnit nxt[RPW][UB];
+        if constexpr (DEPTH == 2) {
+          const bool more = u0 + 2 * UB < units;
+          if (more) issue13(nxt, u0 + 2 * UB);
+          consume13(cur13, u0, Full{});
+#pragma unroll
+          for (int j = 0; j < UB; ++j)
+#pragma unroll
+            for (int r = 0; r < RPW; ++r) {
+              cur13[r][j] = nx13[r][j];
+              if (more) nx13[r][j] = nxt[r][j];
+            }
+        } else {
+          issue13(nxt, u0 + UB);
+          consume13(cur13, u0, Full{});
+#pragma unroll
+          for (int j = 0; j < UB; ++j)
+#pragma unroll
+            for (int r = 0; r < RPW; ++r) cur13[r][j] = nxt[r][j];
+        }
       }
       if (units % UB == 0) {
         consume13(cur13, u0, Full{});
@@ -607,4 +687,16 @@
                                                           out, out_stride, N, K, nullptr, 1, rope, CarArgs{}, pw);
 }
 
+
+template <int M, int NT, int RPW, int UNROLL, int PRO, int EPI, int DEPTH = 1>
+__global__ __launch_bounds__(NT) void gemv_p12_kernel(const bf16_t* __restrict__ x, int x_stride,
+                                                      const bf16_t* __restrict__ norm_w, float eps,
+                                                      const bf16_t* __restrict__ W, PackedW pw,
+                                                      void* __restrict__ out, int out_stride, int N, int K,
+                                                      RopeEpi rope) {
+  extern __shared__ __attribute__((aligned(16))) char smem[];
+  gemv_block<M, NT, RPW, UNROLL, PRO, EPI, false, WF_P12, DEPTH>(blockIdx.x, blockIdx.y, smem, x, x_stride, norm_w, eps, W,
+                                                          out, out_stride, N, K, nullptr, 1, rope, CarArgs{}, pw);
 }
+
+}
diff --git a/csrc/kernels/gemv_p12.hip b/csrc/kernels/gemv_p12.hip
--- /dev/null
+++ b/csrc/kernels/gemv_p12.hip
@@ -0,0 +1,79 @@
+#include "gemv_core.h"
+
+namespace llmc {
+
+#define LLMC_P12_ARGS                                                                                             \
+  const void *x, int x_stride, const void *nw, float eps, const void *W, const PackedW &pw, void *out, int out_stride, \
+      int N, int K, const RopeEpi &rope, hipStream_t s
+#define LLMC_P12_PASS x, x_stride, nw, eps, W, pw, out, out_stride, N, K, rope, s
+
+template <int M, int NT, int RPW, int UNROLL, int PRO, int EPI, int DEPTH = 1>
+static int launch_p12(LLMC_P12_ARGS) {
+  constexpr int WAVES = NT / kWave;
+  auto kern = gemv_p12_kernel<M, NT, RPW, UNROLL, PRO, EPI, DEPTH>;
+  const size_t lds = static_cast<size_t>(M) * K * sizeof(bf16_t) + 2 * M * WAVES * sizeof(float);
+  if (lds > 160 * 1024) return -2;
+  static bool attr_set = false;
+  if (lds > 64 * 1024 && !attr_set) {
+    (void)hipFuncSetAttribute(reinterpret_cast<const void*>(kern), hipFuncAttributeMaxDynamicSharedMemorySize,
+                              160 * 1024);
+    attr_set = true;
+  }
+  const int rows_per_block = WAVES * RPW;
+  const int grid = (N + rows_per_block - 1) / rows_per_block;
+  kern<<<grid, NT, lds, s>>>((const bf16_t*)x, x_stride, (const bf16_t*)nw, eps, (const bf16_t*)W, pw, out, out_stride,
+                             N, K, rope);
+  return static_cast<int>(hipGetLastError());
+}
+
+template <int M, int PRO, int EPI>
+static int p12_geom(int NT, int RPW, int UNROLL, LLMC_P12_ARGS) {
+  if (M == 2 && NT == 1024 && RPW == 1 && UNROLL == 8 && EPI == EPI_ROPE) UNROLL = 4;
+#define LLMC_P12_GEOM(nt, rpw, un) \
+  if (NT == nt && RPW == rpw && UNROLL == un) return launch_p12<M, nt, rpw, un, PRO, EPI>(LLMC_P12_PASS);
+  LLMC_P12_GEOM(1024, 1, 4)
+  LLMC_P12_GEOM(896, 1, 4)
+  LLMC_P12_GEOM(768, 1, 4)
+  LLMC_P12_GEOM(640, 1, 4)
+  LLMC_P12_GEOM(512, 1, 4)
+  LLMC_P12_GEOM(1024, 2, 4)
+  LLMC_P12_GEOM(896, 2, 4)
+  LLMC_P12_GEOM(768, 2, 4)
+  LLMC_P12_GEOM(256, 2, 4)
+  LLMC_P12_GEOM(640, 1, 8)
+  LLMC_P12_GEOM(256, 1, 8)
+  if constexpr (!(M == 2 && EPI == EPI_ROPE)) {
+    LLMC_P12_GEOM(1024, 1, 8)
+  }
+#undef LLMC_P12_GEOM
+  return -8;
+}
+
+template <int PRO, int EPI>
+static int p12_rows(int M, int NT, int RPW, int UNROLL, LLMC_P12_ARGS) {
+  switch (M) {
+    case 1: return p12_geom<1, PRO, EPI>(NT, RPW, UNROLL, LLMC_P12_PASS);
+    case 2: return p12_geom<2, PRO, EPI>(NT, RPW, UNROLL, LLMC_P12_PASS);
+    default: return -3;
+  }
+}
+
+int launch_gemv_p12(int M, int NT, int RPW, int UNROLL, int pro, int epi, LLMC_P12_ARGS) {
+#define LLMC_P12_CASE(E)                                                                  \
+  case E:                                                                                 \
+    return pro == PRO_NORM ? p12_rows<PRO_NORM, E>(M, NT, RPW, UNROLL, LLMC_P12_PASS)     \
+                           : p12_rows<PRO_NONE, E>(M, NT, RPW, UNROLL, LLMC_P12_PASS);
+  switch (epi) {
+    LLMC_P12_CASE(EPI_BF16)
+    LLMC_P12_CASE(EPI_F32)
+    LLMC_P12_CASE(EPI_RESADD)
+    LLMC_P12_CASE(EPI_SILU)
+    case EPI_ROPE:
+      if (pro != PRO_NORM) return -5;
+      return p12_rows<PRO_NORM, EPI_ROPE>(M, NT, RPW, UNROLL, LLMC_P12_PASS);
+    default: return -4;
+  }
+#undef LLMC_P12_CASE
+}
+
+}
diff --git a/csrc/kernels/wpack.hip b/csrc/kernels/wpack.hip
--- a/csrc/kernels/wpack.hip
+++ b/csrc/kernels/wpack.hip
@@ -74,9 +74,139 @@
   *reinterpret_cast<uint32_t*>(p + 3072 + lane * 4) = S;
 }
 
+constexpr int kP12WindowSteps = 4;
+
+__global__ __launch_bounds__(256) void wpack12_record_kernel(const bf16_t* __restrict__ W, uint32_t* __restrict__ recs,
+                                                             int32_t* __restrict__ counts, int N, int K) {
+  __shared__ uint32_t slots[4][kP12MaxExc];
+  const int lane = threadIdx.x % kWave, wv = threadIdx.x / kWave;
+  const int row = blockIdx.x * 4 + wv;
+  const bool live = row < N;
+  const u32x4* w = reinterpret_cast<const u32x4*>(W + static_cast<int64_t>(live ? row : 0) * K);
+  const int nchunk = live ? K / 8 : 0;
+  int hi = 0;
+  for (int c = lane; c < nchunk; c += kWave) {
+    const u32x4 v = w[c];
+#pragma unroll
+    for (int i = 0; i < 4; ++i) hi = max(hi, max(static_cast<int>((v[i] >> 8) & 0x7f), static_cast<int>((v[i] >> 24) & 0x7f)));
+  }
+  for (int o = 32; o; o >>= 1) hi = max(hi, __shfl_xor(hi, o, kWave));
+  int cand[kP12WindowSteps], cnt[kP12WindowSteps];
+#pragma unroll
+  for (int d = 0; d < kP12WindowSteps; ++d) {
+    cand[d] = max(hi - 7 - d, 0);
+    cnt[d] = 0;
+  }
+  for (int c = lane; c < nchunk; c += kWave) {
+    const u32x4 v = w[c];
+#pragma unroll
+    for (int i = 0; i < 8; ++i) {
+      const int h = (v[i / 2] >> (16 * (i & 1) + 8)) & 0x7f;
+#pragma unroll
+      for (int d = 0; d < kP12WindowSteps; ++d) cnt[d] += (h < cand[d] || h > cand[d] + 7) ? 1 : 0;
+    }
+  }
+#pragma unroll
+  for (int d = 0; d < kP12WindowSteps; ++d)
+    for (int o = 32; o; o >>= 1) cnt[d] += __shfl_xor(cnt[d], o, kWave);
+  int base = cand[0], best = cnt[0];
+#pragma unroll
+  for (int d = 1; d < kP12WindowSteps; ++d)
+    if (cnt[d] < best) {
+      best = cnt[d];
+      base = cand[d];
+    }
+  if (lane < kP12MaxExc) slots[wv][lane] = 0;
+  __syncthreads();
+  if (live && best <= kP12MaxExc) {
+    int done = 0;
+    for (int c0 = 0; c0 < nchunk; c0 += kWave) {
+      const u32x4 v = w[c0 + lane];
+      uint32_t m = 0;
+#pragma unroll
+      for (int i = 0; i < 8; ++i) {
+        const int h = (v[i / 2] >> (16 * (i & 1) + 8)) & 0x7f;
+        m |= (h < base || h > base + 7) ? 1u << i : 0u;
+      }
+      const uint64_t any = __ballot(m != 0);
+      if (any == 0) continue;
+      int mine = __popc(m), pre = mine;
+      for (int o = 1; o < kWave; o <<= 1) {
+        const int t = __shfl_up(pre, o, kWave);
+        if (lane >= o) pre += t;
+      }
+      int at = done + pre - mine;
+#pragma unroll
+      for (int i = 0; i < 8; ++i) {
+        if (m >> i & 1u) {
+          const uint32_t b = (v[i / 2] >> (16 * (i & 1))) & 0xffffu;
+          if (at < kP12MaxExc) slots[wv][at] = b << 16 | static_cast<uint32_t>(8 * (c0 + lane) + i);
+          ++at;
+        }
+      }
+      done += __shfl(pre, kWave - 1, kWave);
+    }
+  }
+  __syncthreads();
+  if (!live) return;
+  const bool raw = best > kP12MaxExc;
+  uint32_t* rec = recs + static_cast<int64_t>(row) * kP12RecDwords;
+  if (lane == 0) {
+    rec[0] = raw ? static_cast<uint32_t>(kP12Raw) : static_cast<uint32_t>(base) | static_cast<uint32_t>(best) << 8;
+    atomicAdd(counts + (raw ? 0 : 1), raw ? 1 : best);
+  }
+  if (lane < kP12MaxExc) rec[1 + lane] = slots[wv][lane];
+}
+
+__global__ __launch_bounds__(256) void wpack12_planes_kernel(const bf16_t* __restrict__ W,
+                                                             const uint32_t* __restrict__ recs, uint8_t* __restrict__ P,
+                                                             int N, int K) {
+  const int units = K / kP13UnitElems;
+  const int64_t gid = static_cast<int64_t>(blockIdx.x) * blockDim.x + threadIdx.x;
+  if (gid >= static_cast<int64_t>(N) * units * kWave) return;
+  const int lane = static_cast<int>(gid % kWave);
+  const int u = static_cast<int>((gid / kWave) % units);
+  const int64_t row = gid / kWave / units;
+  const u32x4* w = reinterpret_cast<const u32x4*>(W + row * K);
+  const uint32_t hb = recs[row * kP12RecDwords] & 0xffu;
+  const uint32_t base = hb == kP12Raw ? 0u : hb;
+  uint32_t lowb[8], nib[4];
+#pragma unroll
+  for (int c = 0; c < 4; ++c) {
+    const u32x4 v = w[lane + kWave * (4 * u + c)];
+    uint32_t code[2];
+#pragma unroll
+    for (int h = 0; h < 2; ++h) {
+      uint32_t lb = 0, cd = 0;
+#pragma unroll
+      for (int j = 0; j < 4; ++j) {
+        const uint32_t b = (v[2 * h + j / 2] >> (16 * (j & 1))) & 0xffffu;
+        lb |= (b & 0xffu) << (8 * j);
+        cd |= (((((b >> 8) & 0x7fu) - base) & 0x7u) | (b >> 15) << 3) << (8 * j);
+      }
+      lowb[2 * c + h] = lb;
+      code[h] = cd;
+    }
+    nib[c] = code[0] | (code[1] << 4);
+  }
+  uint8_t* p = P + (row * units + u) * kP12UnitBytes;
+  *reinterpret_cast<u32x4*>(p + lane * 16) = u32x4{lowb[0], lowb[1], lowb[2], lowb[3]};
+  *reinterpret_cast<u32x4*>(p + 1024 + lane * 16) = u32x4{lowb[4], lowb[5], lowb[6], lowb[7]};
+  *reinterpret_cast<u32x4*>(p + 2048 + lane * 16) = u32x4{nib[0], nib[1], nib[2], nib[3]};
+}
+
 }
 
 using namespace llmc;
+
+extern "C" int llmc_wpack12(const void* W, void* planes, void* recs, void* counts, int N, int K, hipStream_t s) {
+  if (N <= 0 || K <= 0 || K % kP13UnitElems != 0 || K > kP12MaxK) return -1;
+  wpack12_record_kernel<<<(N + 3) / 4, 256, 0, s>>>((const bf16_t*)W, (uint32_t*)recs, (int32_t*)counts, N, K);
+  const int64_t threads = static_cast<int64_t>(N) * (K / kP13UnitElems) * kWave;
+  wpack12_planes_kernel<<<static_cast<unsigned>((threads + 255) / 256), 256, 0, s>>>(
+      (const bf16_t*)W, (const uint32_t*)recs, (uint8_t*)planes, N, K);
+  return static_cast<int>(hipGetLastError());
+}
 
 extern "C" int llmc_wpack13(const void* W, void* planes, void* hdr, void* raw_count, int N, int K, hipStream_t s) {
   if (N <= 0 || K <= 0 || K % kP13UnitElems != 0) return -1;
diff --git a/llm_consensus_amd/engine/engine.py b/llm_consensus_amd/engine/engine.py
--- a/llm_consensus_amd/engine/engine.py
+++ b/llm_consensus_amd/engine/engine.py
@@ -228,9 +228,10 @@
                 why = f"the twin ({need / 2**30:.2f} GiB) does not fit in {free / 2**30:.2f} GiB free"
             else:
                 st = self.w.pack_decode_weights(with_o)
-                log.info("%s: packed weights on: %d of %d tensors, %.2f GiB beside %.2f GiB bf16, raw rows <= %.3f %%",
-                         self.name, st["packed"], st["tensors"], st["bytes"] / 2**30, self.w.nbytes() / 2**30,
-                         100 * st["raw_share"])
+                log.info("%s: packed weights on: %d of %d tensors (%d at 12 bits, %d at 13), %.2f GiB beside %.2f GiB "
+                         "bf16, exceptions %.4f %% of the 12-bit weights, raw rows <= %.3f %%",
+                         self.name, st["packed"], st["tensors"], st["p12"], st["p13"], st["bytes"] / 2**30,
+                         self.w.nbytes() / 2**30, 100 * st["exception_share"], 100 * st["raw_share"])
         if why is not None:
             log.info("%s: packed weights off: %s", self.name, why)
             return
diff --git a/llm_consensus_amd/models/transformer.py b/llm_consensus_amd/models/transformer.py
--- a/llm_consensus_amd/models/transformer.py
+++ b/llm_consensus_amd/models/transformer.py
@@ -159,28 +159,42 @@
         ts = [self.lm_head]
         for L in self.layers:
             ts += [L.w_qkv, L.w_gu, L.w_down] + ([L.w_o] if with_o else [])
-        return sum(wpack.packed_nbytes(*t.shape) for t in ts if t.dim() == 2 and wpack.packable_shape(*t.shape))
+        fmt = wpack.packed_format()
+
+        def size(N, K):
+            return wpack.packed12_nbytes(N, K) if fmt == 12 and wpack.packable12_shape(N, K) else wpack.packed_nbytes(N, K)
+
+        return sum(size(*t.shape) for t in ts if t.dim() == 2 and wpack.packable_shape(*t.shape))
 
     def pack_decode_weights(self, with_o: bool = True) -> dict:
         from ..ops import wpack
 
         if self.cfg.is_moe:
             raise ValueError("packed weights: dense models only")
-        st = {"tensors": 0, "packed": 0, "bytes": 0, "raw_share": 0.0}
+        st = {"tensors": 0, "packed": 0, "p12": 0, "p13": 0, "bytes": 0, "raw_share": 0.0, "exception_share": 0.0}
+        exc = w12 = 0
 
         def twin(W):
+            nonlocal exc, w12
             st["tensors"] += 1
-            pw, share = wpack.pack_if_worthwhile(W)
-            st["raw_share"] = max(st["raw_share"], share)
+            pw = wpack.pack_best(W)
             if pw is not None:
                 st["packed"] += 1
                 st["bytes"] += pw.nbytes()
+                st["raw_share"] = max(st["raw_share"], pw.raw_share)
+                if isinstance(pw, wpack.PackedWeight12):
+                    st["p12"] += 1
+                    exc += pw.exceptions
+                    w12 += pw.N * pw.K
+                else:
+                    st["p13"] += 1
             return pw
 
         self.p_lm_head = twin(self.lm_head)
         for L in self.layers:
             L.p_qkv, L.p_gu, L.p_down = twin(L.w_qkv), twin(L.w_gu), twin(L.w_down)
             L.p_o = twin(L.w_o) if with_o else None
+        st["exception_share"] = exc / max(1, w12)
         return st
 
     def packed_nbytes(self) -> int:
diff --git a/llm_consensus_amd/ops/__init__.py b/llm_consensus_amd/ops/__init__.py
--- a/llm_consensus_amd/ops/__init__.py
+++ b/llm_consensus_amd/ops/__init__.py
@@ -95,8 +95,9 @@
         n_out = N // 2 if epi == EPI_SILU else N
         out = torch.empty(M, n_out, dtype=torch.float32 if epi == EPI_F32 else torch.bfloat16, device=x.device)
     if _use_packed(Wp, M, N, K, mfma):
-        kernels().gemv_p13(M, _p(x), x.stride(0), _p(norm_w), float(eps), _p(W), _p(Wp.planes), _p(Wp.hdr), _p(out),
-                           out.stride(0), N, K, epi, _s(x))
+        gemv_packed = kernels().gemv_p12 if isinstance(Wp, wpack.PackedWeight12) else kernels().gemv_p13
+        gemv_packed(M, _p(x), x.stride(0), _p(norm_w), float(eps), _p(W), _p(Wp.planes), _p(Wp.hdr), _p(out),
+                    out.stride(0), N, K, epi, _s(x))
         return out
     if M <= 4 or (M <= GEMV_MAX_M and K % 128 == 0 and x.stride(0) % 8 == 0):
         kernels().gemv(M, _p(x), x.stride(0), _p(norm_w), float(eps), _p(W), _p(out), out.stride(0), N, K, epi,
@@ -212,9 +213,11 @@
     M, K = x.shape
     bias = _qkv_bias(bias, W.shape[0], "qkv_rope")
     if _use_packed(Wp, M, W.shape[0], K, mfma):
-        kernels().gemv_qkv_rope_p13(M, _p(x), x.stride(0), _p(norm_w), float(eps), _p(W), _p(Wp.planes), _p(Wp.hdr),
-                                    W.shape[0], K, _p(q_out), q_out.stride(0), _p(k_cache), _p(v_cache),
-                                    _p(positions), _p(slots), _p(cos_t), _p(sin_t), nh, nkv, D, bs, _s(x), _p(bias))
+        qkv_packed = (kernels().gemv_qkv_rope_p12 if isinstance(Wp, wpack.PackedWeight12)
+                      else kernels().gemv_qkv_rope_p13)
+        qkv_packed(M, _p(x), x.stride(0), _p(norm_w), float(eps), _p(W), _p(Wp.planes), _p(Wp.hdr),
+                   W.shape[0], K, _p(q_out), q_out.stride(0), _p(k_cache), _p(v_cache),
+                   _p(positions), _p(slots), _p(cos_t), _p(sin_t), nh, nkv, D, bs, _s(x), _p(bias))
         return
     if M > 4 and (K % 128 != 0 or x.stride(0) % 8 != 0):
         qkv = linear(x, W, EPI_BF16, norm_w=norm_w, eps=eps)
diff --git a/llm_consensus_amd/ops/wpack.py b/llm_consensus_amd/ops/wpack.py
--- a/llm_consensus_amd/ops/wpack.py
+++ b/llm_consensus_amd/ops/wpack.py
@@ -116,3 +116,147 @@
         return None, 0.0
     pw = pack(W)
     return (pw if pw.raw_share <= MAX_RAW_SHARE else None), pw.raw_share
+
+
+
+UNIT12_BYTES = 3072
+MAX_EXC = 16
+REC12_DWORDS = 1 + MAX_EXC
+WINDOW_STEPS = 4
+MAX_K12 = 65536 - UNIT_ELEMS
+
+
+class PackedWeight12:
+
+    __slots__ = ("planes", "hdr", "raw_rows", "exceptions", "N", "K")
+
+    def __init__(self, planes: torch.Tensor, hdr: torch.Tensor, raw_rows: int, exceptions: int, N: int, K: int):
+        self.planes, self.hdr, self.raw_rows, self.exceptions, self.N, self.K = \
+            planes, hdr, int(raw_rows), int(exceptions), N, K
+
+    @property
+    def raw_share(self) -> float:
+        return self.raw_rows / max(1, self.N)
+
+    @property
+    def exception_share(self) -> float:
+        return self.exceptions / max(1, self.N * self.K)
+
+    def records(self) -> torch.Tensor:
+        return self.hdr.view(torch.int32).view(self.N, REC12_DWORDS)
+
+    def nbytes(self) -> int:
+        return self.planes.numel() + self.hdr.numel()
+
+
+def packable12_shape(N: int, K: int) -> bool:
+    return packable_shape(N, K) and K <= MAX_K12
+
+
+def packed12_nbytes(N: int, K: int) -> int:
+    return N * (K // UNIT_ELEMS) * UNIT12_BYTES + N * REC12_DWORDS * 4
+
+
+def window_candidates(W: torch.Tensor) -> Tuple[torch.Tensor, torch.Tensor]:
+    hi7 = (_bits(W) >> 8) & 0x7F
+    top = hi7.max(dim=1).values - 7
+    bases = torch.stack([(top - d).clamp(min=0) for d in range(WINDOW_STEPS)], dim=1)
+    counts = torch.stack([((hi7 < bases[:, d:d + 1]) | (hi7 > bases[:, d:d + 1] + 7)).sum(dim=1)
+                          for d in range(WINDOW_STEPS)], dim=1)
+    return bases.to(torch.int32), counts.to(torch.int32)
+
+
+def pack12_reference(W: torch.Tensor) -> PackedWeight12:
+    N, K = W.shape
+    if not packable12_shape(N, K):
+        raise ValueError(f"wpack12: K = {K} is not a multiple of {UNIT_ELEMS} up to {MAX_K12}")
+    U = K // UNIT_ELEMS
+    bits = _bits(W)
+    hi7 = (bits >> 8) & 0x7F
+    bases, counts = window_candidates(W)
+    base, cnt = bases[:, 0].clone(), counts[:, 0].clone()
+    for d in range(1, WINDOW_STEPS):
+        better = counts[:, d] < cnt
+        base = torch.where(better, bases[:, d], base)
+        cnt = torch.where(better, counts[:, d], cnt)
+    raw = cnt > MAX_EXC
+    rec = torch.zeros(N, REC12_DWORDS, dtype=torch.int64, device=W.device)
+    rec[:, 0] = torch.where(raw, torch.full_like(cnt, RAW), base | (cnt << 8))
+    exc = ((hi7 < base.view(N, 1)) | (hi7 > base.view(N, 1) + 7)) & ~raw.view(N, 1)
+    rows, ks = exc.nonzero(as_tuple=True)
+    if rows.numel():
+        first = torch.zeros(N + 1, dtype=torch.int64, device=W.device)
+        first[1:] = exc.sum(dim=1).cumsum(0)
+        rank = torch.arange(rows.numel(), device=W.device) - first[rows]
+        rec[rows, 1 + rank] = (bits[rows, ks].to(torch.int64) << 16) | ks
+    rec = (rec - ((rec & 0x80000000) << 1)).to(torch.int32)
+    pbase = torch.where(raw, torch.zeros_like(base), base)
+    b = _lane_order(bits, U)
+    low = (b & 0xFF).to(torch.uint8)
+    code = ((((b >> 8) & 0x7F) - pbase.view(N, 1, 1, 1)) & 0x7) | ((b >> 15) << 3)
+    code = code.view(N, U, 64, 4, 2, 4)
+    nib = (code[..., 0, :] | (code[..., 1, :] << 4)).to(torch.uint8)
+    planes = torch.cat([low[..., :16].reshape(N, U, 1024), low[..., 16:].reshape(N, U, 1024),
+                        nib.reshape(N, U, 1024)], dim=2).contiguous()
+    hdr = rec.contiguous().view(torch.uint8).view(N, REC12_DWORDS * 4)
+    return PackedWeight12(planes, hdr, int(raw.sum()), int(cnt[~raw].sum()), N, K)
+
+
+def unpack12_reference(pw: PackedWeight12, W: Optional[torch.Tensor] = None) -> torch.Tensor:
+    N, K = pw.N, pw.K
+    U = K // UNIT_ELEMS
+    p = pw.planes.view(N, U, UNIT12_BYTES).to(torch.int32)
+    rec = pw.records().to(torch.int64) & 0xFFFFFFFF
+    hb = rec[:, 0] & 0xFF
+    raw = hb == RAW
+    base = torch.where(raw, torch.zeros_like(hb), hb).view(N, 1, 1, 1).to(torch.int32)
+    low = torch.cat([p[..., :1024].reshape(N, U, 64, 16), p[..., 1024:2048].reshape(N, U, 64, 16)], dim=3)
+    nib = p[..., 2048:].reshape(N, U, 64, 4, 4)
+    code = torch.stack([nib & 0xF, nib >> 4], dim=4).reshape(N, U, 64, 32)
+    b = ((code >> 3) << 15) | (((code & 7) + base) << 8) | low
+    bits = b.view(N, U, 64, 4, 8).permute(0, 1, 3, 2, 4).reshape(N, K).contiguous()
+    cnt = torch.where(raw, torch.zeros_like(hb), (rec[:, 0] >> 8) & 0xFF)
+    live = torch.arange(MAX_EXC, device=rec.device).view(1, MAX_EXC) < cnt.view(N, 1)
+    rows, slot = live.nonzero(as_tuple=True)
+    ent = rec[rows, 1 + slot]
+    bits[rows, ent & 0xFFFF] = (ent >> 16).to(torch.int32)
+    out = (bits - ((bits & 0x8000) << 1)).to(torch.int16).view(torch.bfloat16)
+    if W is not None:
+        out[raw] = W[raw].to(out.device)
+    return out
+
+
+def pack12(W: torch.Tensor) -> PackedWeight12:
+    if not W.is_cuda:
+        return pack12_reference(W)
+    from ..utils.native import kernels
+
+    N, K = W.shape
+    if W.dtype != torch.bfloat16 or not packable12_shape(N, K):
+        raise ValueError(f"wpack12: bf16 [N, K] with K a multiple of {UNIT_ELEMS} up to {MAX_K12}, "
+                         f"got {W.dtype} {tuple(W.shape)}")
+    W = W.contiguous()
+    planes = torch.empty(N, K // UNIT_ELEMS, UNIT12_BYTES, dtype=torch.uint8, device=W.device)
+    hdr = torch.empty(N, REC12_DWORDS * 4, dtype=torch.uint8, device=W.device)
+    counts = torch.zeros(2, dtype=torch.int32, device=W.device)
+    kernels().wpack12(W.data_ptr(), planes.data_ptr(), hdr.data_ptr(), counts.data_ptr(), N, K,
+                      torch.cuda.current_stream(W.device).cuda_stream)
+    raw_rows, exceptions = counts.tolist()
+    return PackedWeight12(planes, hdr, raw_rows, exceptions, N, K)
+
+
+def packed_format() -> int:
+    from ..parallel.placement import packed_format as fmt
+
+    return fmt()
+
+
+def pack_best(W: torch.Tensor, fmt: Optional[int] = None):
+    if W.dim() != 2 or not packable_shape(*W.shape):
+        return None
+    if (packed_format() if fmt is None else fmt) == 12 and packable12_shape(*W.shape):
+        pw12 = pack12(W)
+        if pw12.raw_share <= MAX_RAW_SHARE:
+            return pw12
+    pw = pack(W)
+    return pw if pw.raw_share <= MAX_RAW_SHARE else None
diff --git a/llm_consensus_amd/parallel/placement.py b/llm_consensus_amd/parallel/placement.py
--- a/llm_consensus_amd/parallel/placement.py
+++ b/llm_consensus_amd/parallel/placement.py
@@ -12,6 +12,13 @@
 def packed_weights_mode() -> str:
     v = os.environ.get("LLMC_PACKED_WEIGHTS", "auto").strip().lower()
     return {"1": "on", "true": "on", "0": "off", "false": "off"}.get(v, v if v in ("auto", "on", "off") else "auto")
+
+
+def packed_format() -> int:
+    v = os.environ.get("LLMC_PACKED_FORMAT", "12").strip()
+    if v not in ("12", "13"):
+        raise ValueError(f"LLMC_PACKED_FORMAT: 12 or 13, got {v!r}")
+    return int(v)
 
 
 @dataclasses.dataclass
```

New measurement: 516.8 (median of 6 runs). +6.9%, better.
